# mantasu/face-crop-plus

Measured on AMD Instinct MI355X. Metric: faces/sec end-to-end (detect+align+crop), higher is better.
Workload: dtype f16x3; 1 GPU; RetinaFace detect + 5-pt align/crop, batch=32/GPU synthetic 1024x1024 RGB, strategy=largest, det_threshold=0.6, output 256x256, detector on 2 HIP streams x 16 images; global_batch=32, image_size=1024, parallelism=dp1

## Files before the change

face-crop-plus_amd/_native.py:

```python
from __future__ import annotations

import ctypes as C
import os

_HERE = os.path.dirname(os.path.abspath(__file__))
LIB_PATH = os.path.join(_HERE, "csrc", "libfcp_hip.so")
ABI_VERSION = 15

c_f32p = C.c_void_p
_lib = None


class ConvDesc(C.Structure):
    _fields_ = [
        ("in_", C.c_void_p), ("w", C.c_void_p), ("bias", C.c_void_p), ("out", C.c_void_p),
        ("res1", C.c_void_p), ("res2", C.c_void_p), ("wscale", C.c_void_p), ("in2", C.c_void_p),
        ("n", C.c_int32), ("in_h", C.c_int32), ("in_w", C.c_int32),
        ("cin", C.c_int32), ("in_ld", C.c_int32), ("in_up2", C.c_int32),
        ("cout", C.c_int32), ("kh", C.c_int32), ("kw", C.c_int32),
        ("stride", C.c_int32), ("pad", C.c_int32),
        ("out_h", C.c_int32), ("out_w", C.c_int32), ("out_ld", C.c_int32),
        ("tile_n", C.c_int32), ("cin4", C.c_int32),
        ("act_slope", C.c_float), ("alpha", C.c_float), ("alpha2", C.c_float),
        ("res1_pre", C.c_int32), ("res1_ld", C.c_int32), ("res1_h", C.c_int32),
        ("res1_w", C.c_int32), ("res2_ld", C.c_int32), ("precision", C.c_int32),
        ("in_fmt", C.c_int32), ("out_fmt", C.c_int32), ("res1_fmt", C.c_int32), ("res2_fmt", C.c_int32),
        ("tile_m", C.c_int32), ("cin2", C.c_int32), ("in2_ld", C.c_int32), ("in2_h", C.c_int32),
        ("in2_w", C.c_int32), ("in2_stride", C.c_int32), ("flags", C.c_int32), ("cu_budget", C.c_int32),
        ("band_top", C.c_int32), ("band_bottom", C.c_int32),
    ]


CONV_FLAT_ADDR = 1
CONV_BALANCE_TAIL = 2
CHAIN_OUT_EVEN_ONLY = 1


class ChainDesc(C.Structure):
    _fields_ = [(k, C.c_void_p) for k in ("t1", "w2", "ws2", "b2", "w3", "ws3", "b3", "res", "out", "w1n", "ws1n",
                                          "b1n", "t1n", "t1b")] + \
               [(k, C.c_int32) for k in ("n", "h", "w", "c", "cn", "t1_ld", "res_ld", "out_ld", "t1n_ld", "nout", "tile_m", "flags",
                                         "cb", "t1b_ld", "t1b_h", "t1b_w", "t1b_stride")]


_P, _I, _F, _L = C.c_void_p, C.c_int, C.c_float, C.c_int64
SIGNATURES = {
    "fcp_conv2d_nhwc_f32": [C.POINTER(ConvDesc), _P],
    "fcp_bottleneck_chain_f16x3": [C.POINTER(ChainDesc), _P],
    "fcp_u8_to_nhwc4_f32": [_P, _P, _L, C.POINTER(C.c_float), _F, _P],
    "fcp_f32nchw_to_nhwc4_f32": [_P, _P, _I, _I, _I, C.POINTER(C.c_float), _F, _P],
    "fcp_maxpool3x3s2_nhwc_f32": [_P, _P, _I, _I, _I, _I, _I, _I, _I, _P],
    "fcp_maxpool3x3s2_split32": [_P, _P, _I, _I, _I, _I, _I, _I, _I, _P],
    "fcp_stem7x7s2_relu_pool_u8": [_P, _I, _I, _I, C.POINTER(C.c_int32), _P, _P, _P, _P, _I, _I, _P],
    "fcp_stem7x7s2_relu_pool_conv1_u8": [_P, _I, _I, _I, C.POINTER(C.c_int32), _P, _P, _P, _P, _I, _I, _P, _P, _P, _P, _I, _P],
    "fcp_stem7x7s2_relu_pool_f32": [_P, _I, _I, _I, _P, _P, _P, _P, _I, _I, _P],
    "fcp_f32_to_split32": [_P, _P, _L, _I, _P],
    "fcp_split32_to_f32": [_P, _P, _L, _I, _P],
    "fcp_absmax_nhwc": [_P, _L, _I, _I, _I, _P, _P],
    "fcp_retina_decode": [_P, _P, _P, _I, _I, _I, _F, _F, _F, _P, _P, _P, _P, _P, _P, _P, _P, _P],
    "fcp_retina_nms_select": [_P, _P, _P, _I, _I, _F, _I, _P, _P, _P, _P, _P, _P],
    "fcp_retina_gather_faces": [_P, _P, _P, _I, _I, _P, _I, _P, _P, _P, _P],
    "fcp_estimate_transform": [_P, _P, _I, _I, _I, _P, _P, _P],
    "fcp_estimate_transform_counted": [_P, _P, _I, _I, _I, _P, _P, _P, _P, _P],
    "fcp_bise_preprocess_u8": [_P, _I, _I, _I, _P, _I, _I, C.POINTER(C.c_float), C.POINTER(C.c_float), _P],
    "fcp_avgpool_nhwc_f32": [_P, _I, _I, _I, _I, _P, _P],
    "fcp_fc_f32": [_P, _P, _P, _P, _I, _I, _I, _I, _P, _P],
    "fcp_scale_add_nhwc_f32": [_P, _I, _P, _P, _P, _I, _I, _I, _I, _P, _I, _P],
    "fcp_parse_tail": [_P, _I, _I, _I, _I, _I, _I, _I, _I, _I, _P, _P, _P],
    "fcp_label_mask_u8": [_P, _L, C.c_uint32, _P, _P],
    "fcp_bicubic_down4_u8": [_P, _I, _I, _I, _P, _P],
    "fcp_warp_affine_u8": [_P, _I, _I, _I, _P, _P, _P, _P, _I, _I, _I, _I, _P, _P],
    "fcp_warp_affine_u8_float": [_P, _I, _I, _I, _P, _P, _P, _P, _I, _I, _I, _I, _P, _P],
    "fcp_build_batch_u8": [_P, _L, _P, _P, _I, _I, _I, _I, _P, _P],
    "fcp_warp_affine_u8_ragged": [_P, _L, _P, _P, _P, _P, _I, _I, _I, _I, _P, _P],
    "fcp_warp_affine_u8_float_ragged": [_P, _L, _P, _P, _P, _P, _I, _I, _I, _I, _P, _P],
    "fcp_resize_area_ragged_u8": [_P, _L, _P, _P, _I, _P, _L, _P],
    "fcp_warp_affine_u8_interp": [_P, _I, _I, _I, _P, _P, _P, _P, _I, _I, _I, _I, _I, _P, _P],
    "fcp_warp_affine_u8_interp_ragged": [_P, _L, _P, _P, _P, _P, _I, _I, _I, _I, _I, _P, _P],
    "fcp_warp_interp_weights": [_I, _P],
    "fcp_crop_sharpness_u8": [_P, _I, _I, _I, _P, _P, _P],
    "fcp_jpeg_encode_u8": [_P, _I, _I, _I, _I, _I, _I, _P, _L, _L, _P, _P, _L, _P],
    "fcp_jpeg_encode_ex_u8": [_P, _I, _I, _I, _I, _I, _I, _I, _P, _L, _L, _P, _P, _P, _L, _P],
    "fcp_jpeg_huffman_tables": [_P, _I, _P, _P, _P],
    "fcp_png_encode_u8": [_P, _I, _I, _I, _I, _P, _L, _L, _P, _P, _L, _P],
    "fcp_png_huffman_lengths": [_P, _I, _P, _P, _P],
    "fcp_matte_u8": [_P, _P, _I, _I, _I, C.c_uint32, _I, _I, _I, _I, _P, _P, _P],
    "fcp_clahe_u8": [_P, _I, _I, _I, _I, C.c_double, _P, _P, _P],
    "fcp_matte_blur_u8": [_P, _P, _I, _I, _I, C.c_uint32, _I, _P, _I, _P, _P, _P, _L, _P],
    "fcp_matte_refine_u8": [_P, _P, _I, _I, _I, C.c_uint32, _I, _I, _P, _P, _L, _P],
    "fcp_matte_alpha_u8": [_P, _P, _I, _I, _I, _I, _I, _I, _P, _P],
    "fcp_matte_blur_alpha_u8": [_P, _P, _P, _I, _I, _I, C.c_uint32, _P, _I, _P, _P, _L, _P],
    "fcp_subject_mask_u8": [_P, _I, _I, _I, C.c_uint32, _I, _I, _P, _P, _L, _P],
    "fcp_feather_alpha_u8": [_P, _I, _I, _I, C.c_uint32, _I, _P, _P],
    "fcp_cutout_u8": [_P, _P, _I, _I, _I, _I, _I, _I, _I, _P, _I, _P, _P, _L, _P],
    "fcp_mask_shift_u8": [_P, _I, _I, _I, C.c_uint32, _I, _P, _P],
    "fcp_nlm_denoise_u8": [_P, _I, _I, _I, _P, _I, _I, _P, _P],
}
EXPORTS = ["fcp_abi_version", "fcp_last_error", "fcp_retina_nms_workspace_bytes", "fcp_jpeg_workspace_bytes",
           "fcp_jpeg_workspace_bytes_ex", "fcp_matte_blur_workspace_bytes", "fcp_matte_refine_workspace_bytes",
           "fcp_subject_mask_workspace_bytes", "fcp_png_workspace_bytes", "fcp_cutout_workspace_bytes"] + list(SIGNATURES)


def lib():
    global _lib
    if _lib is not None:
        return _lib
    if not os.path.isfile(LIB_PATH):
        raise RuntimeError(
            f"HIP extension not built: {LIB_PATH} is missing. Run "
            f"`python face-crop-plus_amd/build_native.py` (needs hipcc). There is no CPU fallback.")
    l = C.CDLL(LIB_PATH)
    l.fcp_abi_version.restype = C.c_int
    l.fcp_last_error.restype = C.c_char_p
    if l.fcp_abi_version() != ABI_VERSION:
        raise RuntimeError(f"libfcp_hip.so ABI {l.fcp_abi_version()} != expected {ABI_VERSION}; rebuild")
    l.fcp_retina_nms_workspace_bytes.argtypes = [C.c_int, C.c_int]
    l.fcp_retina_nms_workspace_bytes.restype = C.c_int64
    l.fcp_jpeg_workspace_bytes.argtypes = [C.c_int, C.c_int, C.c_int, C.c_int]
    l.fcp_jpeg_workspace_bytes.restype = C.c_int64
    l.fcp_jpeg_workspace_bytes_ex.argtypes = [C.c_int] * 6
    l.fcp_jpeg_workspace_bytes_ex.restype = C.c_int64
    l.fcp_png_workspace_bytes.argtypes = [C.c_int, C.c_int, C.c_int, C.c_int]
    l.fcp_png_workspace_bytes.restype = C.c_int64
    l.fcp_matte_blur_workspace_bytes.argtypes = [C.c_int, C.c_int, C.c_int]
    l.fcp_matte_blur_workspace_bytes.restype = C.c_int64
    l.fcp_matte_refine_workspace_bytes.argtypes = [C.c_int, C.c_int, C.c_int]
    l.fcp_matte_refine_workspace_bytes.restype = C.c_int64
    l.fcp_subject_mask_workspace_bytes.argtypes = [C.c_int, C.c_int, C.c_int]
    l.fcp_subject_mask_workspace_bytes.restype = C.c_int64
    l.fcp_cutout_workspace_bytes.argtypes = [C.c_int, C.c_int, C.c_int]
    l.fcp_cutout_workspace_bytes.restype = C.c_int64
    for name, args in SIGNATURES.items():
        fn = getattr(l, name)
        fn.argtypes = args
        fn.restype = C.c_int
    _lib = l
    return l


def check(rc: int, what: str = ""):
    if rc != 0:
        msg = lib().fcp_last_error().decode(errors="replace")
        raise RuntimeError(f"{what or 'fcp_hip'} failed ({rc}): {msg}")


def stream_ptr():
    import torch
    return C.c_void_p(torch.cuda.current_stream().cuda_stream)


def ptr(t, byte_offset: int = 0):
    if t is None:
        return C.c_void_p(0)
    return C.c_void_p(t.data_ptr() + byte_offset)


def encode_slots(who: str, entry: str, pixels_dev, out, op, workspace_bytes, call):
    import torch
    assert pixels_dev.dtype == torch.uint8 and pixels_dev.is_contiguous() and pixels_dev.dim() in (3, 4)
    assert out.dtype == torch.uint8 and out.dim() == 2 and out.shape[0] == pixels_dev.shape[0]
    if op is not None:
        return op()
    f, h, w = pixels_dev.shape[:3]
    c = pixels_dev.shape[3] if pixels_dev.dim() == 4 else 1
    capacity = out.shape[1]
    if capacity and out.stride(1) != 1:
        raise RuntimeError(f"{who}: the bytes of a row of out must be contiguous")
    lengths = torch.empty((f,), dtype=torch.int32, device=pixels_dev.device)
    need = workspace_bytes(f, h, w, c)
    check(-1 if need < 0 else 0, entry)
    work = torch.empty((need,), dtype=torch.uint8, device=pixels_dev.device)
    check(call((f, h, w, c), (ptr(out) if capacity else None, out.stride(0) if f > 1 else capacity, capacity, ptr(lengths)),
               (ptr(work), need, stream_ptr())), entry)
    return lengths
```

face-crop-plus_amd/csrc/fcp_conv.hip:

```cpp
#include "fcp_conv_common.h"

#include <cstdlib>

using namespace fcp_conv;

namespace {

constexpr int LDK = 32;


template <int BN, bool CIN4, bool BUF>
__global__ void __launch_bounds__(256, (BN == 128 ? 2 : (BN == 64 ? 3 : 4))) conv_igemm_f32(const ConvK p) {
  constexpr int WAVES_N = (BN == 32) ? 1 : 2;
  constexpr int WAVES_M = 4 / WAVES_N;
  constexpr int WTM = BM / WAVES_M;
  constexpr int WTN = BN / WAVES_N;
  constexpr int TM = WTM / 32, TN = WTN / 32;
  constexpr int A_LD = BM / 32;
  constexpr int B_LD = BN / 32;

  extern __shared__ __attribute__((aligned(16))) float smem[];
  float* As = smem;
  float* Bs = smem + 2 * BM * LDK;

  const int logical = xcd_tile_order(gridDim.x, blockIdx.x);
  const int tile_n = logical % p.grid_n;
  const int tile_m = logical / p.grid_n;

  const int tid = threadIdx.x;
  const int lane = tid & 63;
  const int wave = tid >> 6;
  const int wm = wave / WAVES_N, wn = wave % WAVES_N;
  const int chunk = tid & 7;
  const int lrow = tid >> 3;

  long nbase[A_LD];
  RowPiece pc[A_LD];
  const int hw = p.out_h * p.out_w;
#pragma unroll
  for (int i = 0; i < A_LD; ++i) {
    const ConvRow r = conv_row(p, tile_m * BM + lrow + 32 * i, p.M, hw, 0u);
    nbase[i] = (long)r.ni * p.ph * p.pw;
    pc[i] = make_row_piece<CIN4>(p, r, chunk, (unsigned)(chunk * 4));
  }
  const float* wbase = p.w + (long)(tile_n * BN + lrow) * p.wrow + chunk * 4;

  __amdgpu_buffer_rsrc_t rs_in, rs_w;
  unsigned rowoff[A_LD];
  unsigned woff[B_LD];
  if (BUF) {
    rs_in = __builtin_amdgcn_make_buffer_rsrc(const_cast<float*>(p.in), 0, p.in_bytes, 0x00020000);
    rs_w = __builtin_amdgcn_make_buffer_rsrc(const_cast<float*>(p.w), 0, p.w_bytes, 0x00020000);
#pragma unroll
    for (int i = 0; i < B_LD; ++i)
      woff[i] = (unsigned)(((tile_n * BN + lrow + 32 * i) * p.wrow + chunk * 4) * 4);
  }

  f32x4 ra0[A_LD], rb0[B_LD], ra1[A_LD], rb1[B_LD];

  auto load_slice = [&](f32x4 (&ra)[A_LD], f32x4 (&rb)[B_LD], int kt, int kh_i, int kw_i, int c0) {
    if (BUF) {
#pragma unroll
      for (int i = 0; i < A_LD; ++i) {
        const unsigned vo = rowoff[i] == 0xFFFFFFFFu ? 0xFFFFFFFFu : rowoff[i] + (unsigned)(c0 * 4);
        ra[i] = buf_load16(rs_in, vo);
      }
#pragma unroll
      for (int i = 0; i < B_LD; ++i) rb[i] = buf_load16(rs_w, woff[i] + (unsigned)(kt * BK * 4));
    } else {
#pragma unroll
      for (int i = 0; i < A_LD; ++i) {
        int hi = pc[i].hi0 + kh_i;
        int wi = pc[i].wi0 + (CIN4 ? chunk : kw_i);
        const bool ok = (unsigned)hi < (unsigned)p.in_h && (unsigned)wi < (unsigned)p.in_w;
        if (p.in_up2) { hi >>= 1; wi >>= 1; }
        const long pix = nbase[i] + (long)hi * p.pw + wi;
        const float* src = CIN4 ? p.in + pix * p.in_ld : p.in + pix * p.in_ld + c0 + chunk * 4;
        ra[i] = ok ? *reinterpret_cast<const f32x4*>(src) : f32x4{0.f, 0.f, 0.f, 0.f};
      }
#pragma unroll
      for (int i = 0; i < B_LD; ++i)
        rb[i] = *reinterpret_cast<const f32x4*>(wbase + (long)(32 * i) * p.wrow + kt * BK);
    }
  };
  const int schunk = chunk ^ ((lrow >> 1) & 7);
  auto store_slice = [&](const f32x4 (&ra)[A_LD], const f32x4 (&rb)[B_LD], int buf) {
    float* a = As + buf * BM * LDK + lrow * LDK + schunk * 4;
    float* b = Bs + buf * BN * LDK + lrow * LDK + schunk * 4;
#pragma unroll
    for (int i = 0; i < A_LD; ++i) *reinterpret_cast<f32x4*>(a + 32 * i * LDK) = ra[i];
#pragma unroll
    for (int i = 0; i < B_LD; ++i) *reinterpret_cast<f32x4*>(b + 32 * i * LDK) = rb[i];
  };

  f32x16 acc[TM][TN];
  clear_acc(acc);

  TapWalk tw;
  auto advance = [&]() {
    if (BUF) next_tap<CIN4, true>(p, tw, pc, rowoff);
    else tw.advance<CIN4>(p);
  };

  const int aoff = (wm * WTM + (lane & 31)) * LDK;
  const int boff = (wn * WTN + (lane & 31)) * LDK;
  const int rsw = ((lane & 31) >> 1) & 7;
  int koff[4];
#pragma unroll
  for (int pp = 0; pp < 4; ++pp) koff[pp] = (((2 * pp + (lane >> 5)) ^ rsw)) * 4;

  auto compute = [&](int buf) {
    const float* Ab = As + buf * BM * LDK + aoff;
    const float* Bb = Bs + buf * BN * LDK + boff;
#pragma unroll
    for (int pp = 0; pp < 4; ++pp) {
      f32x4 a[TM], b[TN];
#pragma unroll
      for (int i = 0; i < TM; ++i) a[i] = *reinterpret_cast<const f32x4*>(Ab + (i * 32 * LDK + koff[pp]));
#pragma unroll
      for (int j = 0; j < TN; ++j) b[j] = *reinterpret_cast<const f32x4*>(Bb + (j * 32 * LDK + koff[pp]));
#pragma unroll
      for (int e = 0; e < 4; ++e)
#pragma unroll
        for (int i = 0; i < TM; ++i)
#pragma unroll
          for (int j = 0; j < TN; ++j)
            acc[i][j] = __builtin_amdgcn_mfma_f32_32x32x2f32(a[i][e], b[j][e], acc[i][j], 0, 0, 0);
    }
  };
  auto step = [&](int kt, f32x4 (&ra_ld)[A_LD], f32x4 (&rb_ld)[B_LD], const f32x4 (&ra_st)[A_LD],
                  const f32x4 (&rb_st)[B_LD]) {
    if (kt + 2 < p.ktiles) {
      advance();
      load_slice(ra_ld, rb_ld, kt + 2, tw.kh_i, tw.kw_i, tw.c0);
    }
    compute(kt & 1);
    if (kt + 1 < p.ktiles) store_slice(ra_st, rb_st, (kt + 1) & 1);
    __syncthreads();
  };

  if (BUF) set_tap<CIN4, true>(p, tw, pc, rowoff);
  load_slice(ra0, rb0, 0, tw.kh_i, tw.kw_i, tw.c0);
  store_slice(ra0, rb0, 0);
  if (p.ktiles > 1) {
    advance();
    load_slice(ra1, rb1, 1, tw.kh_i, tw.kw_i, tw.c0);
  }
  __syncthreads();
  for (int kt = 0; kt < p.ktiles; kt += 2) {
    step(kt, ra0, rb0, ra1, rb1);
    if (kt + 1 < p.ktiles) step(kt + 1, ra1, rb1, ra0, rb0);
  }

  conv_epilogue<BN, TM, TN, WTM, WTN>(p, acc, smem, tile_m, tile_n, tid, lane, wm, wn, hw);
}

template <int BN, bool CIN4, bool BUF>
int launch(const ConvK& k, hipStream_t s) {
  const size_t lds = (size_t)2 * (BM + BN) * LDK * sizeof(float);
  FCP_LDS_OPT_IN((&conv_igemm_f32<BN, CIN4, BUF>), lds);
  const int blocks = k.grid_m * k.grid_n;
  hipLaunchKernelGGL((conv_igemm_f32<BN, CIN4, BUF>), dim3(blocks), dim3(256), lds, s, k);
  FCP_LAUNCH_OK();
  return 0;
}

}

extern "C" int fcp_conv2d_nhwc_f32(const fcp_conv_desc* d, fcp_stream_t stream) {
  FCP_REQUIRE(d != nullptr, "conv: null descriptor");
  FCP_REQUIRE(d->in && d->w && d->out, "conv: null tensor pointer");
  FCP_REQUIRE(d->n > 0 && d->in_h > 0 && d->in_w > 0 && d->cout > 0, "conv: bad sizes");
  const bool big = d->tile_m == 256, halo = d->tile_m == 1;
  FCP_REQUIRE(d->tile_m == 0 || d->tile_m == 128 || big || halo, "conv: tile_m must be 0/128/256 (or 1: halo-tile 3x3)");
  const bool halo_wide = halo && d->tile_n != 32;
  if (halo)
    FCP_REQUIRE(d->precision == 1 && d->in_fmt == 1 && !d->cin4 && d->kh == 3 && d->kw == 3 && d->stride == 1 &&
                d->pad == 1 && d->cout <= 64 && d->cout % 8 == 0 && d->cin >= 64 && !d->in2 &&
                (!d->res1 || (d->res1_h == d->out_h && d->res1_w == d->out_w)) || halo_wide,
                "conv: the halo-tile kernel needs a 3x3 / stride 1 / pad 1 conv with cin >= 64, cout <= 64 (cout %% 8 == 0) on the "
                "fp16x3 path with a split32 input, no second source, no resized residual");
  if (halo_wide)
    FCP_REQUIRE(d->precision == 1 && d->in_fmt == 1 && !d->cin4 && d->kh == 3 && d->kw == 3 && d->stride == 1 &&
                d->pad == 1 && d->cout % 8 == 0 && d->cin >= 64 && d->cin % 64 == 0 && !d->in2 &&
                ((d->tile_n == 64 && d->cout <= 64 && (!d->res1 || (d->res1_h == d->out_h && d->res1_w == d->out_w))) ||
                 (d->tile_n == 128 && d->cout <= 128 && !d->res1 && !d->res2)),
                "conv: the wide halo-tile kernel (tile_m 1, tile_n 64 / 128) needs a 3x3 / stride 1 / pad 1 conv with cin %% 64 == 0, "
                "cout <= tile_n (cout %% 8 == 0; no residuals above 64 filters) on the fp16x3 path with a split32 input");
  FCP_REQUIRE(d->tile_n == 32 || d->tile_n == 64 || d->tile_n == 128 || (big && (d->tile_n == 256 || d->tile_n == 192)),
              "conv: tile_n must be 32/64/128 (or 192 / 256 with tile_m 256)");
  if (big)
    FCP_REQUIRE(d->precision == 1 && d->in_fmt == 1 && !d->cin4 && !d->in_up2 && d->cout % 8 == 0 && d->tile_n >= 128,
                "conv: 256-row tiles need the fp16x3 path on a split32 input (no cin4 / in_up2), cout %% 8 == 0, tile_n 128/256");
  FCP_REQUIRE(d->kh >= 1 && d->kw >= 1 && d->stride >= 1 && d->pad >= 0, "conv: bad filter geometry");
  FCP_REQUIRE(d->kh * d->kw <= 32 || d->cin4, "conv: at most 32 filter taps (kh*kw) outside cin4 mode");
  FCP_REQUIRE(d->in_ld % 4 == 0 && ((uintptr_t)d->in & 15) == 0, "conv: input must be 16-byte aligned, in_ld %% 4 == 0");
  FCP_REQUIRE(((uintptr_t)d->w & 15) == 0, "conv: filter must be 16-byte aligned");
  if (d->cin4) {
    FCP_REQUIRE(d->cin <= 4 && d->in_ld == 4 && d->kw <= 8, "conv: cin4 mode needs cin<=4, in_ld==4, kw<=8");
  } else {
    FCP_REQUIRE(d->cin % 32 == 0 && d->cin > 0, "conv: cin must be a multiple of 32 (got %d)", d->cin);
  }
  FCP_REQUIRE(d->band_top >= 0 && d->band_bottom >= 0 && d->band_top <= d->pad && d->band_bottom <= d->pad &&
              ((d->band_top | d->band_bottom) == 0 || (d->stride == 1 && !d->in2)),
              "conv: band_top / band_bottom must lie in 0..pad (stride-1 convs without a second source only)");
  const int eh = (d->in_h - d->band_top - d->band_bottom + 2 * d->pad - d->kh) / d->stride + 1;
  const int ew = (d->in_w + 2 * d->pad - d->kw) / d->stride + 1;
  FCP_REQUIRE(eh == d->out_h && ew == d->out_w, "conv: output size %dx%d does not match geometry %dx%d",
              d->out_h, d->out_w, eh, ew);
  if (d->in_up2) FCP_REQUIRE(d->in_h % 2 == 0 && d->in_w % 2 == 0, "conv: in_up2 needs even logical size");
  const long M = (long)d->n * d->out_h * d->out_w;
  FCP_REQUIRE(M < (1L << 31), "conv: too many output pixels");

  ConvK k;
  k.in = d->in; k.w = reinterpret_cast<const float*>(d->w); k.bias = d->bias; k.wscale = d->wscale; k.out = d->out; k.res1 = d->res1; k.res2 = d->res2;
  k.n = d->n; k.in_h = d->in_h; k.in_w = d->in_w;
  k.ph = d->in_up2 ? d->in_h / 2 : d->in_h;
  k.pw = d->in_up2 ? d->in_w / 2 : d->in_w;
  k.cin = d->cin; k.in_ld = d->in_ld; k.in_up2 = d->in_up2;
  k.cout = d->cout; k.kh = d->kh; k.kw = d->kw; k.stride = d->stride; k.pad = d->pad; k.pad_h = d->pad - d->band_top;
  k.out_h = d->out_h; k.out_w = d->out_w; k.out_ld = d->out_ld;
  k.M = (int)M;
  if (d->cin4) {
    k.ktiles = d->kh; k.ctiles = 1; k.wrow = d->kh * 32;
  } else {
    k.ctiles = d->cin / 32; k.ktiles = d->kh * d->kw * k.ctiles; k.wrow = d->kh * d->kw * d->cin;
  }
  k.act_slope = d->act_slope; k.alpha = d->alpha; k.alpha2 = d->alpha2;
  k.res1_pre = d->res1_pre; k.res1_ld = d->res1_ld; k.res2_ld = d->res2_ld;
  k.res1_h = d->res1_h; k.res1_w = d->res1_w;
  k.res1_resize = 0; k.res1_sh = 1.f; k.res1_sw = 1.f;
  k.in_fmt = d->in_fmt; k.out_fmt = d->out_fmt; k.res1_fmt = d->res1 ? d->res1_fmt : 0; k.res2_fmt = d->res2 ? d->res2_fmt : 0;
  const int any_split = k.in_fmt | k.out_fmt | k.res1_fmt | k.res2_fmt;
  FCP_REQUIRE((unsigned)any_split <= 1u, "conv: tensor formats must be 0 (fp32) or 1 (split32)");
  if (any_split) {
    FCP_REQUIRE(d->precision == 1, "conv: split32 tensors need precision 1 (fp16x3 kernel)");
    FCP_REQUIRE(d->cout % 8 == 0, "conv: split32 epilogue needs cout %% 8 == 0");
    FCP_REQUIRE(!k.in_fmt || (!d->cin4 && d->in_ld % 32 == 0 && ((uintptr_t)d->in & 127) == 0),
                "conv: split32 input must be a 32-channel-group aligned view (in_ld %% 32 == 0), not cin4");
    FCP_REQUIRE(!k.out_fmt || (d->out_ld % 32 == 0 && ((uintptr_t)d->out & 127) == 0 && d->cout % 32 == 0),
                "conv: split32 output must be a 32-channel-group aligned view with cout %% 32 == 0");
    FCP_REQUIRE(!k.res1_fmt || (d->res1_ld % 32 == 0 && ((uintptr_t)d->res1 & 127) == 0), "conv: misaligned split32 res1");
    FCP_REQUIRE(!k.res2_fmt || (d->res2_ld % 32 == 0 && ((uintptr_t)d->res2 & 127) == 0), "conv: misaligned split32 res2");
    FCP_REQUIRE(((uintptr_t)d->out & 15) == 0 && d->out_ld % 4 == 0 && (!d->res1 || (((uintptr_t)d->res1 & 15) == 0 && d->res1_ld % 4 == 0)) &&
                (!d->res2 || (((uintptr_t)d->res2 & 15) == 0 && d->res2_ld % 4 == 0)), "conv: 8-channel epilogue needs 16-byte aligned tensors");
  }
  if (d->res1) {
    FCP_REQUIRE(d->res1_h > 0 && d->res1_w > 0 && d->res1_ld > 0, "conv: res1 geometry missing");
    if (d->res1_h != d->out_h || d->res1_w != d->out_w) {
      k.res1_resize = 1;
      k.res1_sh = (float)d->res1_h / (float)d->out_h;
      k.res1_sw = (float)d->res1_w / (float)d->out_w;
    }
  }
  if (d->res2) FCP_REQUIRE(d->res2_ld > 0, "conv: res2_ld missing");
  k.vec_ok = (d->out_ld % 4 == 0) && (((uintptr_t)d->out & 15) == 0);
  if (d->res1) k.vec_ok = k.vec_ok && (d->res1_ld % 4 == 0) && (((uintptr_t)d->res1 & 15) == 0);
  if (d->res2) k.vec_ok = k.vec_ok && (d->res2_ld % 4 == 0) && (((uintptr_t)d->res2 & 15) == 0);
  static const int nt_env = getenv("FCP_NT_STORE") ? atoi(getenv("FCP_NT_STORE")) : 1;
  k.nt_store = nt_env;
  k.balance = (d->flags & FCP_CONV_BALANCE_TAIL) ? 1 : 0;
  k.cu_budget = d->cu_budget;
  k.mfull = 0; k.tail_rows = 0; k.round_size = 0;
  k.in2 = nullptr; k.in2_bytes = 0; k.csplit = d->cin; k.in2_ld = 0; k.ph2 = 0; k.pw2 = 0; k.stride2 = 1;
  if (d->in2) {
    FCP_REQUIRE(d->precision == 1 && d->in_fmt == 1 && !d->cin4 && !d->in_up2 && d->kh == 1 && d->kw == 1 && d->pad == 0,
                "conv: a second source needs a 1x1 / pad 0 conv on the fp16x3 path with split32 inputs");
    FCP_REQUIRE(d->cin2 > 0 && d->cin2 < d->cin && d->cin2 % 32 == 0 && d->in2_ld % 32 == 0 && d->in2_ld >= d->cin2 &&
                ((uintptr_t)d->in2 & 127) == 0, "conv: in2 must be a 32-channel-group aligned split32 view, 0 < cin2 < cin");
    FCP_REQUIRE(d->in2_stride >= 1 && d->in2_h > 0 && d->in2_w > 0 && (long)(d->out_h - 1) * d->in2_stride < d->in2_h &&
                (long)(d->out_w - 1) * d->in2_stride < d->in2_w, "conv: in2 geometry does not cover the output grid");
    const unsigned long in2_bytes = (unsigned long)d->n * d->in2_h * d->in2_w * d->in2_ld * 4ul;
    FCP_REQUIRE(in2_bytes < 0xFFFFFFF0ul, "conv: in2 must be below 4 GiB");
    k.in2 = d->in2; k.in2_bytes = (unsigned)in2_bytes; k.csplit = d->cin - d->cin2; k.in2_ld = d->in2_ld;
    k.ph2 = d->in2_h; k.pw2 = d->in2_w; k.stride2 = d->in2_stride;
  }
  k.grid_m = fcp_cdiv(M, BM);
  k.grid_n = fcp_cdiv(d->cout, d->tile_n);
  hipStream_t s = (hipStream_t)stream;
  const unsigned long in_bytes = (unsigned long)d->n * k.ph * k.pw * d->in_ld * 4ul;
  const unsigned long w_bytes = (unsigned long)(k.grid_n * d->tile_n) * k.wrow * 4ul;
  FCP_REQUIRE(!(d->flags & FCP_CONV_FLAT_ADDR) || d->precision == 0, "conv: FCP_CONV_FLAT_ADDR is a precision-0 (fp32 kernel) option");
  const bool buf = in_bytes < 0xFFFFFFF0ul && w_bytes < 0xFFFFFFF0ul && !(d->flags & FCP_CONV_FLAT_ADDR);
  FCP_REQUIRE(d->precision == 0 || d->precision == 1, "conv: precision must be 0 (fp32) or 1 (fp16x3)");
  if (d->precision == 1) {
    FCP_REQUIRE(buf, "conv: the fp16x3 path needs tensors below 4 GiB (pack this layer with precision 0)");
    FCP_REQUIRE(d->wscale != nullptr, "conv: precision 1 needs wscale");
    k.in_bytes = (unsigned)in_bytes;
    k.w_bytes = (unsigned)w_bytes;
    if (halo) {
      k.grid_n = 1;
      const unsigned long out_bytes = (unsigned long)M * d->out_ld * 4ul;
      FCP_REQUIRE(out_bytes < 0xFFFFFFF0ul, "conv(halo): the output view must span less than 4 GiB");
      FCP_REQUIRE(d->wscale != nullptr && ((uintptr_t)d->wscale & 15) == 0 && ((uintptr_t)d->bias & 15) == 0,
                  "conv(halo): wscale / bias must be 16-byte aligned");
      k.in2_bytes = (unsigned)out_bytes;
      k.w_bytes = (unsigned)((unsigned long)fcp_cdiv(d->cout, 128) * 128ul * k.wrow * 4ul);
      return halo_wide ? launch_f16x3_halo_wide(k, s) : launch_f16x3_halo(k, s);
    }
    if (big) {
      k.w_bytes = (unsigned)((unsigned long)fcp_cdiv(d->cout, 128) * 128ul * k.wrow * 4ul);
      return launch_f16x3_big(k, d->tile_n, s);
    }
    if (k.in_fmt == 1 && !d->cin4) return launch_f16x3_dma(k, d->tile_n, s);
    return launch_f16x3(k, d->tile_n, d->cin4 != 0, s);
  }
  k.in_bytes = buf ? (unsigned)in_bytes : 0u;
  k.w_bytes = buf ? (unsigned)w_bytes : 0u;
#define FCP_DISPATCH(BN_)                                                             \
  do {                                                                                \
    if (d->cin4) return buf ? launch<BN_, true, true>(k, s) : launch<BN_, true, false>(k, s); \
    return buf ? launch<BN_, false, true>(k, s) : launch<BN_, false, false>(k, s);   \
  } while (0)
  switch (d->tile_n) {
    case 32: FCP_DISPATCH(32);
    case 64: FCP_DISPATCH(64);
    default: FCP_DISPATCH(128);
  }
#undef FCP_DISPATCH
}
```

face-crop-plus_amd/csrc/fcp_conv_common.h:

```cpp
#pragma once
#include <type_traits>
#include "fcp_common.h"
#include "fcp_hip.h"

typedef float f32x16 __attribute__((ext_vector_type(16)));
typedef float f32x4 __attribute__((ext_vector_type(4)));


constexpr int FCP_AUX_A = 0;
constexpr int FCP_AUX_B = 0;

namespace fcp_conv {

constexpr int BM = 128;
constexpr int BK = 32;

struct ConvK {
  const float* in;
  const float* w;
  const float* bias;
  float* out;
  const float* res1;
  const float* res2;
  int n, in_h, in_w, ph, pw, cin, in_ld, in_up2;
// ... 271 lines not shown
  if (fmt == 1) {
    pack8(v, 1, a, b);
    store8(base, pix, ld, c, 1, nt, a, b);
  } else {
    pack8(v, 0, a, b);
    store8(base, pix, ld, c, 0, 0, a, b);
  }
}

__device__ __forceinline__ float conv_scale_bias(float acc, float ws, float b) { return acc * ws + b; }

struct ConvEpi {
  bool res1, res1_pre, res2;
  float act_slope, alpha, alpha2;
};
template <typename E>
__device__ __forceinline__ float conv_finish(const E e, float x, float r1, float r2) {
  if (e.res1 && e.res1_pre) x += r1;
  x = x >= 0.f ? x : x * e.act_slope;
  x = x * e.alpha;
  if (e.res1 && !e.res1_pre) x += r1;
  if (e.res2) x = x * e.alpha2 + r2;
  return x;
}
template <typename E>
__device__ __forceinline__ float conv_value(const E& e, float acc, float ws, float b, float r1, float r2) {
  return conv_finish(e, conv_scale_bias(acc, ws, b), r1, r2);
}
__device__ __forceinline__ float conv_finish_relu(float x) { return conv_finish(ConvEpi{false, false, false, 0.f, 1.f, 1.f}, x, 0.f, 0.f); }
__device__ __forceinline__ float conv_finish_relu(float x, float r1) { return conv_finish(ConvEpi{true, true, false, 0.f, 1.f, 1.f}, x, r1, 0.f); }
__device__ __forceinline__ float conv_value_relu(float acc, float ws, float b) { return conv_finish_relu(conv_scale_bias(acc, ws, b)); }

__device__ __forceinline__ long res1_pixel(const ConvK& p, long m, int hw) {
  int ni, ho, wo;
  conv_out_pixel(p, m, hw, ni, ho, wo);
  int sh = (int)floorf(ho * p.res1_sh);
  int sw = (int)floorf(wo * p.res1_sw);
  sh = sh < p.res1_h - 1 ? sh : p.res1_h - 1;
  sw = sw < p.res1_w - 1 ? sw : p.res1_w - 1;
  return ((long)ni * p.res1_h + sh) * p.res1_w + sw;
}

__device__ __forceinline__ constexpr int mfma_c_row(int rr, int half) { return (rr & 3) + 8 * (rr >> 2) + 4 * half; }

template <int BN, int TM, int TN, int WTM, int WTN>
__device__ __forceinline__ void stage_acc_tile(const f32x16 (&acc)[TM][TN], float* Cs, int lane, int wm, int wn) {
  const int half = lane >> 5;
#pragma unroll
  for (int i = 0; i < TM; ++i)
#pragma unroll
    for (int j = 0; j < TN; ++j)
#pragma unroll
      for (int rr = 0; rr < 16; ++rr) {
        const int row = wm * WTM + i * 32 + mfma_c_row(rr, half);
        Cs[row * BN + wn * WTN + j * 32 + (lane & 31)] = acc[i][j][rr];
      }
  __syncthreads();
}

template <int BN, int TM, int TN, int WTM, int WTN>
__device__ __forceinline__ void conv_epilogue(const ConvK& p, f32x16 (&acc)[TM][TN], float* smem, int tile_m,
                                              int tile_n, int tid, int lane, int wm, int wn, int hw) {
  constexpr int CPR = BN / 4;
  constexpr int RPP = 256 / CPR;
  constexpr int PASSES = BM / RPP;
  float* Cs = smem;
  const int ccol = (tid % CPR) * 4;
  const int crow = tid / CPR;
  const int co = tile_n * BN + ccol;
  const bool vec = p.vec_ok && (co + 3 < p.cout);
  const long m0 = (long)tile_m * BM + crow;

  const bool pre1 = p.res1 != nullptr && !p.res1_resize && vec;
  const bool pre2 = p.res2 != nullptr && vec;
  stage_acc_tile<BN, TM, TN, WTM, WTN>(acc, Cs, lane, wm, wn);

  f32x4 bias4 = {0.f, 0.f, 0.f, 0.f}, ws4 = {1.f, 1.f, 1.f, 1.f};
  if (p.bias != nullptr) {
#pragma unroll
    for (int e = 0; e < 4; ++e)
      if (co + e < p.cout) bias4[e] = p.bias[co + e];
  }
  if (p.wscale != nullptr) {
#pragma unroll
    for (int e = 0; e < 4; ++e)
      if (co + e < p.cout) ws4[e] = p.wscale[co + e];
  }
  constexpr int EPC = PASSES < 4 ? PASSES : 4;
#pragma unroll 1
  for (int g = 0; g < PASSES; g += EPC) {
    f32x4 r1v[EPC], r2v[EPC];
    if (pre1) {
#pragma unroll
      for (int i = 0; i < EPC; ++i) {
        const long m = m0 + (long)(g + i) * RPP;
        r1v[i] = m < p.M ? *reinterpret_cast<const f32x4*>(p.res1 + m * p.res1_ld + co) : f32x4{0.f, 0.f, 0.f, 0.f};
      }
    }
    if (pre2) {
#pragma unroll
      for (int i = 0; i < EPC; ++i) {
        const long m = m0 + (long)(g + i) * RPP;
        r2v[i] = m < p.M ? *reinterpret_cast<const f32x4*>(p.res2 + m * p.res2_ld + co) : f32x4{0.f, 0.f, 0.f, 0.f};
      }
    }
#pragma unroll
    for (int i = 0; i < EPC; ++i) {
      const int row = crow + (g + i) * RPP;
      const long m = m0 + (long)(g + i) * RPP;
      if (m >= p.M || co >= p.cout) continue;
      f32x4 v = *reinterpret_cast<const f32x4*>(Cs + row * BN + ccol);
      f32x4 r1 = {0.f, 0.f, 0.f, 0.f}, r2 = {0.f, 0.f, 0.f, 0.f};
      if (pre1) {
        r1 = r1v[i];
      } else if (p.res1 != nullptr) {
        const long roff = (p.res1_resize ? res1_pixel(p, m, hw) : m) * p.res1_ld + co;
        if (vec) {
          r1 = *reinterpret_cast<const f32x4*>(p.res1 + roff);
        } else {
#pragma unroll
          for (int e = 0; e < 4; ++e)
            if (co + e < p.cout) r1[e] = p.res1[roff + e];
        }
      }
      if (pre2) {
        r2 = r2v[i];
      } else if (p.res2 != nullptr) {
#pragma unroll
        for (int e = 0; e < 4; ++e)
          if (co + e < p.cout) r2[e] = p.res2[m * p.res2_ld + co + e];
      }
#pragma unroll
      for (int e = 0; e < 4; ++e) v[e] = conv_value(p, v[e], ws4[e], bias4[e], r1[e], r2[e]);
      float* dst = p.out + m * p.out_ld + co;
      if (vec) {
        *reinterpret_cast<f32x4*>(dst) = v;
      } else {
#pragma unroll
        for (int e = 0; e < 4; ++e)
          if (co + e < p.cout) dst[e] = v[e];
      }
    }
  }
}


template <int I, int N, typename F>
__device__ __forceinline__ void fcp_static_for(F&& f) {
  if constexpr (I < N) {
    f(std::integral_constant<int, I>{});
    fcp_static_for<I + 1, N>(f);
  }
}

template <int TM, int TN, int WTM, int WTN>
__device__ __forceinline__ void conv_epilogue_regs(const ConvK& p, f32x16 (&acc)[TM][TN], int m_start, int m_end, int tm_act, int co_tile,
                                                   int co_end, int wm, int wn, int lane, int hw) {
    const int lp = lane & 15, lg = lane >> 4;
  auto swap32 = [](float& x, float& y) {
    const auto r = __builtin_amdgcn_permlane32_swap(__float_as_uint(x), __float_as_uint(y), false, false);
    const unsigned r0 = r[0], r1 = r[1];
    x = __uint_as_float(r0); y = __uint_as_float(r1);
  };
  auto swap16 = [](float& x, float& y) {
    const auto r = __builtin_amdgcn_permlane16_swap(__float_as_uint(x), __float_as_uint(y), false, false);
    const unsigned r0 = r[0], r1 = r[1];
    x = __uint_as_float(r0); y = __uint_as_float(r1);
  };
  constexpr int GI = TM < 2 ? TM : 2;
  constexpr int NGI = (TM + GI - 1) / GI;
  constexpr int NG = TN * NGI;
  u32x4_t pend_a[GI][2], pend_b[GI][2];
  auto row_of = [&](int i, int set) { return m_start + wm * WTM + i * 32 + 16 * set + lp; };
  auto chan_of = [&](int jj) { return co_tile + wn * WTN + jj * 32 + 8 * lg; };
  auto flush = [&](auto gc) {
    constexpr int g = decltype(gc)::value, jj = g / NGI, i0 = (g % NGI) * GI;
    const int co = chan_of(jj);
    fcp_static_for<0, GI>([&](auto ic) {
      constexpr int i = i0 + decltype(ic)::value;
      if constexpr (i < TM) {
        fcp_static_for<0, 2>([&](auto sc) {
          constexpr int set = decltype(sc)::value;
          const int mi = row_of(i, set);
          if (i < tm_act && mi < m_end && co < co_end) store8(p.out, mi, p.out_ld, co, p.out_fmt, 0, pend_a[i - i0][set], pend_b[i - i0][set]);
        });
      }
    });
  };
  fcp_static_for<0, NG>([&](auto gc) {
    constexpr int g = decltype(gc)::value, j = g / NGI, i0 = (g % NGI) * GI;
    const int co = chan_of(j);
    const bool cok = co < co_end;
    const int cc = cok ? co : co_tile;
    u32x4_t r1a[GI][2], r1b[GI][2];
    if (p.res1 != nullptr) {
      fcp_static_for<0, GI>([&](auto ic) {
        constexpr int i = i0 + decltype(ic)::value;
        if constexpr (i < TM) {
          fcp_static_for<0, 2>([&](auto sc) {
            constexpr int set = decltype(sc)::value;
            const int mi = row_of(i, set);
            const long m = (i < tm_act && mi < m_end && cok) ? (long)mi : (long)m_start;
            const long rpix = p.res1_resize ? res1_pixel(p, m, hw) : m;
            if (p.res1_fmt == 1) {
              const char* pb = reinterpret_cast<const char*>(p.res1) + rpix * p.res1_ld * 4 + split_chan_off(cc);
              r1a[i - i0][set] = *reinterpret_cast<const u32x4_t*>(pb);
              r1b[i - i0][set] = *reinterpret_cast<const u32x4_t*>(pb + 64);
            } else {
              r1a[i - i0][set] = *reinterpret_cast<const u32x4_t*>(p.res1 + rpix * p.res1_ld + cc);
              r1b[i - i0][set] = *reinterpret_cast<const u32x4_t*>(p.res1 + rpix * p.res1_ld + cc + 4);
            }
          });
        }
      });
    }
    __builtin_amdgcn_sched_barrier(0);
    if constexpr (g > 0) flush(std::integral_constant<int, g - 1>{});
    __builtin_amdgcn_sched_barrier(0);
    float bias8[8], ws8[8];
    {
      const f32x4 w0 = *reinterpret_cast<const f32x4*>(p.wscale + cc), w1 = *reinterpret_cast<const f32x4*>(p.wscale + cc + 4);
      f32x4 b0 = {0.f, 0.f, 0.f, 0.f}, b1 = b0;
      if (p.bias != nullptr) { b0 = *reinterpret_cast<const f32x4*>(p.bias + cc); b1 = *reinterpret_cast<const f32x4*>(p.bias + cc + 4); }
#pragma unroll
      for (int e = 0; e < 4; ++e) { ws8[e] = w0[e]; ws8[4 + e] = w1[e]; bias8[e] = b0[e]; bias8[4 + e] = b1[e]; }
    }
    fcp_static_for<0, GI>([&](auto ic) {
      constexpr int i = i0 + decltype(ic)::value;
      if constexpr (i < TM) {
        float va[8], vb[8];
        fcp_static_for<0, 4>([&](auto ec) {
          constexpr int e = decltype(ec)::value;
          float q0 = acc[i][j][e], q1 = acc[i][j][4 + e], q2 = acc[i][j][8 + e], q3 = acc[i][j][12 + e];
          swap32(q0, q1);
          swap32(q2, q3);
          swap32(q0, q2); swap16(q0, q2);
          swap32(q1, q3); swap16(q1, q3);
          va[e] = q0; va[4 + e] = q1; vb[e] = q2; vb[4 + e] = q3;
        });
        fcp_static_for<0, 2>([&](auto sc) {
          constexpr int set = decltype(sc)::value;
          float (&v)[8] = set == 0 ? va : vb;
          float r1[8], r2[8];
          if (p.res1 != nullptr) {
            if (p.res1_fmt == 1) {
              join8(r1a[i - i0][set], r1b[i - i0][set], r1);
            } else {
              const f32x4 fa = __builtin_bit_cast(f32x4, r1a[i - i0][set]), fb = __builtin_bit_cast(f32x4, r1b[i - i0][set]);
              r1[0] = fa[0]; r1[1] = fa[1]; r1[2] = fa[2]; r1[3] = fa[3]; r1[4] = fb[0]; r1[5] = fb[1]; r1[6] = fb[2]; r1[7] = fb[3];
            }
          }
          if (p.res2 != nullptr) {
            const int mi = row_of(i, set);
            load8(p.res2, (i < tm_act && mi < m_end && cok) ? (long)mi : (long)m_start, p.res2_ld, cc, p.res2_fmt, r2);
          }
#pragma unroll
          for (int e = 0; e < 8; ++e) v[e] = conv_value(p, v[e], ws8[e], bias8[e], r1[e], r2[e]);
          pack8(v, p.out_fmt, pend_a[i - i0][set], pend_b[i - i0][set]);
        });
      }
    });
  });
  flush(std::integral_constant<int, NG - 1>{});
}

template <int BN, int TM, int TN, int WTM, int WTN>
__device__ __forceinline__ void conv_epilogue8(const ConvK& p, f32x16 (&acc)[TM][TN], float* smem, int tile_m,
                                               int tile_n, int tid, int lane, int wm, int wn, int hw) {
  constexpr int CPR = BN / 8;
  constexpr int RPP = 256 / CPR;
  constexpr int PASSES = BM / RPP;
  float* Cs = smem;
  const int ccol = (tid % CPR) * 8;
  const int crow = tid / CPR;
  const int co = tile_n * BN + ccol;
  const long m0 = (long)tile_m * BM + crow;
  stage_acc_tile<BN, TM, TN, WTM, WTN>(acc, Cs, lane, wm, wn);
  if (co >= p.cout) return;
  float bias8[8], ws8[8];
#pragma unroll
  for (int e = 0; e < 8; ++e) {
    bias8[e] = p.bias != nullptr ? p.bias[co + e] : 0.f;
    ws8[e] = p.wscale != nullptr ? p.wscale[co + e] : 1.f;
  }
#pragma unroll
  for (int g = 0; g < PASSES; ++g) {
    const int row = crow + g * RPP;
    const long m = m0 + (long)g * RPP;
    if (m >= p.M) continue;
    float v[8], r1[8], r2[8];
    {
      const f32x4 a = *reinterpret_cast<const f32x4*>(Cs + row * BN + ccol);
      const f32x4 b = *reinterpret_cast<const f32x4*>(Cs + row * BN + ccol + 4);
      v[0] = a[0]; v[1] = a[1]; v[2] = a[2]; v[3] = a[3]; v[4] = b[0]; v[5] = b[1]; v[6] = b[2]; v[7] = b[3];
    }
    if (p.res1 != nullptr) load8(p.res1, p.res1_resize ? res1_pixel(p, m, hw) : m, p.res1_ld, co, p.res1_fmt, r1);
    if (p.res2 != nullptr) load8(p.res2, m, p.res2_ld, co, p.res2_fmt, r2);
#pragma unroll
    for (int e = 0; e < 8; ++e) v[e] = conv_value(p, v[e], ws8[e], bias8[e], r1[e], r2[e]);
    pack_store8(p.out, m, p.out_ld, co, p.out_fmt, p.nt_store, v);
  }
}

int launch_f16x3(const ConvK& k, int tile_n, bool cin4, hipStream_t s);
int launch_f16x3_dma(const ConvK& k, int tile_n, hipStream_t s);
int launch_f16x3_halo(const ConvK& k, hipStream_t s);
int launch_f16x3_halo_wide(const ConvK& k, hipStream_t s);
int launch_f16x3_big(const ConvK& k, int tile_n, hipStream_t s);

}
```

face-crop-plus_amd/csrc/fcp_conv_f16x3_big.hip:

```cpp
#include "fcp_conv_common.h"

#include <type_traits>

using namespace fcp_conv;

namespace {

constexpr int BMB = 256;
constexpr int NT = 512;
constexpr int ROWB = 128;
constexpr int STAGE = 1 << 16;

template <int BN>
__global__ void __launch_bounds__(NT, 1) conv_igemm_f16x3_big(const ConvK p) {
  constexpr int WAVES_N = BN == 256 ? 4 : 2;
  constexpr int WAVES_M = 8 / WAVES_N;
  constexpr int WTM = BMB / WAVES_M, WTN = BN / WAVES_N;
  constexpr int TM = WTM / 32, TN = WTN / 32;
  constexpr int A_LD = BMB / 64, B_LD = BN / 64;

  extern __shared__ __attribute__((aligned(16))) float smem[];
  char* lds = reinterpret_cast<char*>(smem);

  const int nb = p.big_tiles;
  int vb = blockIdx.x;
  int tile_n = 0, m_start = 0, m_end = 0;
  auto decode = [&](int bid) {
    const int rbase = (bid / p.round_size) * p.round_size;
    const int nr = nb - rbase < p.round_size ? nb - rbase : p.round_size;
    const int bi = bid - rbase;
    const int logical = rbase + xcd_tile_order(nr, bi);
    tile_n = logical % p.grid_n;
    const int tile_m = logical / p.grid_n;
    m_start = tile_m < p.mfull ? tile_m * BMB : p.mfull * BMB + (tile_m - p.mfull) * p.tail_rows;
    const int m_rows = tile_m < p.mfull ? BMB : p.tail_rows;
    m_end = m_start + m_rows < p.M ? m_start + m_rows : p.M;
  };
  decode(vb);

  const int tid = threadIdx.x;
  const int lane = tid & 63;
  const int wave_u = __builtin_amdgcn_readfirstlane(tid >> 6);
  const int wm = wave_u / WAVES_N, wn = wave_u % WAVES_N;
  const int lrow = tid >> 3;
  const int csrc = (tid & 7) ^ (((lrow >> 1) & 7) ^ ((lrow & 1) << 2));

  const int hw = p.out_h * p.out_w;
  RowPiece pc[A_LD];
  unsigned base2[A_LD];
  unsigned rowoff[A_LD], woff[B_LD];
  auto setup_tile = [&]() {
#pragma unroll
    for (int i = 0; i < A_LD; ++i) {
      const int m = m_start + lrow + 64 * i;
      unsigned pbase = 0;
      int hi0 = -(1 << 28), wi0 = 0;
      base2[i] = 0xFFFFFFFFu;
      if (m < m_end) {
        int ni, ho, wo;
        conv_out_pixel(p, m, hw, ni, ho, wo);
        pbase = (unsigned)(ni * p.ph * p.pw);
        hi0 = ho * p.stride - p.pad_h;
        wi0 = wo * p.stride - p.pad;
        if (p.in2 != nullptr)
          base2[i] = (((unsigned)(ni * p.ph2 + ho * p.stride2) * (unsigned)p.pw2 + (unsigned)(wo * p.stride2)) * (unsigned)p.in2_ld +
                      (unsigned)(csrc * 4)) * 4u;
      }
      pc[i].tp = make_tap_piece<false>(p, pbase, hi0, wi0, (unsigned)(csrc * 4));
    }
#pragma unroll
    for (int i = 0; i < B_LD; ++i) woff[i] = (unsigned)(((tile_n * BN + lrow + 64 * i) * p.wrow + csrc * 4) * 4);
  };
  setup_tile();
  __amdgpu_buffer_rsrc_t rs_in2 = __builtin_amdgcn_make_buffer_rsrc(const_cast<float*>(p.in2 ? p.in2 : p.in), 0, p.in2_bytes, 0x00020000);
  __amdgpu_buffer_rsrc_t rs_in = __builtin_amdgcn_make_buffer_rsrc(const_cast<float*>(p.in), 0, p.in_bytes, 0x00020000);
  __amdgpu_buffer_rsrc_t rs_w = __builtin_amdgcn_make_buffer_rsrc(const_cast<float*>(p.w), 0, p.w_bytes, 0x00020000);
  TapWalk tw;
  auto advance = [&]() { next_tap<false, false>(p, tw, pc, rowoff); };
  auto dma = [&](int kt, int stage) {
    char* a = lds + stage * STAGE + wave_u * 8 * ROWB;
    dma_slice<64>(p, rs_in, rs_in2, rs_w, a, a + BMB * ROWB, rowoff, base2, woff, tw.c0, kt);
  };

  f32x16 acc[TM][TN];

  const unsigned lds0 = (unsigned)(size_t)(__attribute__((address_space(3))) char*)lds;
  int offH[2], offL[2];
  frag_offsets(lane, offH, offL);
  const unsigned arow = lds0 + (unsigned)((wm * WTM + (lane & 31)) * ROWB);
  const unsigned brow = lds0 + (unsigned)((BMB + wn * WTN + (lane & 31)) * ROWB);
  unsigned aH[2], aL[2], bH[2], bL[2];
#pragma unroll
  for (int s = 0; s < 2; ++s) {
    aH[s] = arow + (unsigned)offH[s]; aL[s] = arow + (unsigned)offL[s];
    bH[s] = brow + (unsigned)offH[s]; bL[s] = brow + (unsigned)offL[s];
  }

  auto prefetch_tile = [&]() {
    tw = TapWalk();
    set_tap<false, false>(p, tw, pc, rowoff);
    dma(0, 0);
    if (p.ktiles > 1) {
      advance();
      dma(1, 1);
    }
  };
  prefetch_tile();
  int tm_act = 0;
  auto main_loop = [&](auto tma_c) {
    constexpr int TMA = decltype(tma_c)::value;
    f16x8 fah[2][TMA > 0 ? TMA : 1], fal[2][TMA > 0 ? TMA : 1], fbh[2][TN], fbl[2][TN];
  auto read_frags = [&](auto set_c, unsigned stage_xor) {
    constexpr int set = decltype(set_c)::value;
    fcp_static_for<0, TMA>([&](auto ic) {
      constexpr int i = decltype(ic)::value;
      fah[set][i] = lds_read128i<i * 32 * ROWB>(aH[set] ^ stage_xor);
      fal[set][i] = lds_read128i<i * 32 * ROWB>(aL[set] ^ stage_xor);
    });
    fcp_static_for<0, TN>([&](auto jc) {
      constexpr int j = decltype(jc)::value;
      fbh[set][j] = lds_read128i<j * 32 * ROWB>(bH[set] ^ stage_xor);
      fbl[set][j] = lds_read128i<j * 32 * ROWB>(bL[set] ^ stage_xor);
    });
  };
  constexpr std::integral_constant<int, 0> SET0{};
  constexpr std::integral_constant<int, 1> SET1{};
  auto mfmas_reads = [&](auto cs_c, auto ls_c, unsigned stage_xor) {
    constexpr int cs = decltype(cs_c)::value, ls = decltype(ls_c)::value;
    constexpr int NM = 3 * TMA * TN, NR = 2 * TMA + 2 * TN;
    fcp_static_for<0, NM>([&](auto mc) {
      constexpr int m = decltype(mc)::value;
      constexpr int g = m / (TMA * TN), i = (m % (TMA * TN)) / TN, j = m % TN;
      if constexpr (g == 0) acc[i][j] = __builtin_amdgcn_mfma_f32_32x32x16_f16(fbh[cs][j], fal[cs][i], acc[i][j], 0, 0, 0);
      else if constexpr (g == 1) acc[i][j] = __builtin_amdgcn_mfma_f32_32x32x16_f16(fbl[cs][j], fah[cs][i], acc[i][j], 0, 0, 0);
      else acc[i][j] = __builtin_amdgcn_mfma_f32_32x32x16_f16(fbh[cs][j], fah[cs][i], acc[i][j], 0, 0, 0);
      __builtin_amdgcn_sched_barrier(0);
      fcp_static_for<0, NR>([&](auto rc) {
        constexpr int r = decltype(rc)::value;
        if constexpr (((r + 1) * NM) / NR - 1 == m
        ) {
          if constexpr (r < 2 * TMA) {
            constexpr int ii = r / 2;
            if constexpr (r % 2 == 0) fah[ls][ii] = lds_read128i<ii * 32 * ROWB>(aH[ls] ^ stage_xor);
            else fal[ls][ii] = lds_read128i<ii * 32 * ROWB>(aL[ls] ^ stage_xor);
          } else {
            constexpr int jj = (r - 2 * TMA) / 2;
            if constexpr (r % 2 == 0) fbh[ls][jj] = lds_read128i<jj * 32 * ROWB>(bH[ls] ^ stage_xor);
            else fbl[ls][jj] = lds_read128i<jj * 32 * ROWB>(bL[ls] ^ stage_xor);
          }
          __builtin_amdgcn_sched_barrier(0);
        }
      });
    });
  };

  read_frags(SET0, 0u);
  asm volatile("s_waitcnt lgkmcnt(0)" ::: "memory");
  __builtin_amdgcn_sched_barrier(0);

  unsigned sx = 0u;
  for (int kt = 0; kt < p.ktiles; ++kt) {
    mfmas_reads(SET0, SET1, sx);
    __builtin_amdgcn_sched_barrier(0);
    asm volatile("s_waitcnt lgkmcnt(0)" ::: "memory");
    asm volatile("s_waitcnt vmcnt(0)" ::: "memory");
    __builtin_amdgcn_s_barrier();
    __builtin_amdgcn_sched_barrier(0);
    const bool dma_first = wave_u >= 4;
    if (dma_first && kt + 2 < p.ktiles) {
      advance();
      dma(kt + 2, kt & 1);
    }
    __builtin_amdgcn_sched_barrier(0);
    mfmas_reads(SET1, SET0, sx ^ (unsigned)STAGE);
    __builtin_amdgcn_sched_barrier(0);
    if (!dma_first && kt + 2 < p.ktiles) {
      advance();
      dma(kt + 2, kt & 1);
    }
    __builtin_amdgcn_sched_barrier(0);
    asm volatile("s_waitcnt lgkmcnt(0)" ::: "memory");
    __builtin_amdgcn_sched_barrier(0);
    sx ^= (unsigned)STAGE;
  }
  };
  for (;;) {
  asm volatile("s_waitcnt vmcnt(0)" ::: "memory");
  __builtin_amdgcn_s_barrier();
  __builtin_amdgcn_sched_barrier(0);
  tm_act = (m_end - m_start - wm * WTM + 31) >> 5;
  tm_act = __builtin_amdgcn_readfirstlane(tm_act < 0 ? 0 : (tm_act > TM ? TM : tm_act));
  clear_acc(acc);
  fcp_static_for<0, TM + 1>([&](auto tc) {
    if (tm_act == decltype(tc)::value) main_loop(tc);
  });
  asm volatile("s_waitcnt vmcnt(0)" ::: "memory");
  __builtin_amdgcn_s_barrier();

  const int e_tile_n = tile_n, e_m_start = m_start, e_m_end = m_end, e_tm_act = tm_act;
  const bool more = p.big_persist && vb + p.round_size < nb;
  if (more) {
    vb += p.round_size;
    decode(vb);
    setup_tile();
    prefetch_tile();
  }
  conv_epilogue_regs<TM, TN, WTM, WTN>(p, acc, e_m_start, e_m_end, e_tm_act, e_tile_n * BN,
                                       (e_tile_n + 1) * BN < p.cout ? (e_tile_n + 1) * BN : p.cout, wm, wn, lane, hw);
  if (!more) break;
  }
}

template <int BN>
int launch(ConvK k, hipStream_t s) {
  const size_t lds = 2 * (size_t)STAGE;
  FCP_LDS_OPT_IN((&conv_igemm_f16x3_big<BN>), lds);
  k.grid_n = fcp_cdiv(k.cout, BN);
  int cus = k.cu_budget > 0 ? k.cu_budget : fcp_cu_count();
  cus = cus < 8 ? 8 : (cus & ~7);
  k.round_size = cus;
  const int mt = fcp_cdiv(k.M, BMB);
  k.mfull = mt;
  k.tail_rows = BMB;
  k.grid_m = mt;
  if (k.balance) {
    const long tiles = (long)mt * k.grid_n;
    const long full_rounds = tiles / cus;
    const int mfull = (int)((full_rounds * cus) / k.grid_n);
    const long rem = (long)k.M - (long)mfull * BMB;
    if (rem > 0) {
      const long slots = cus / k.grid_n > 0 ? cus / k.grid_n : 1;
      long r = ((rem + slots - 1) / slots + 31) / 32 * 32;
      r = r < 32 ? 32 : r;
      if (r < BMB) {
        k.mfull = mfull;
        k.tail_rows = (int)r;
        k.grid_m = mfull + (int)((rem + r - 1) / r);
      }
    }
  }
  k.big_tiles = k.grid_m * k.grid_n;
  static const int persist_env = getenv("FCP_BIG_PERSIST") ? atoi(getenv("FCP_BIG_PERSIST")) : -1;
  k.big_persist = persist_env < 0 ? (k.cu_budget == 0) : (persist_env != 0);
  hipLaunchKernelGGL((conv_igemm_f16x3_big<BN>), dim3(k.big_persist && k.big_tiles > k.round_size ? k.round_size : k.big_tiles), dim3(NT), lds, s, k);
  FCP_LAUNCH_OK();
  return 0;
}

}

namespace fcp_conv {

int launch_f16x3_big(const ConvK& k, int tile_n, hipStream_t s) {
  return tile_n == 256 ? launch<256>(k, s) : tile_n == 192 ? launch<192>(k, s) : launch<128>(k, s);
}

}
```

face-crop-plus_amd/csrc/fcp_conv_f16x3_dma.hip:

```cpp
#include "fcp_conv_common.h"

using namespace fcp_conv;

namespace {

constexpr int NST = 2;

template <int BN, bool EP8>
__global__ void __launch_bounds__(256, (BN == 128 ? 2 : 3)) conv_igemm_f16x3_dma(const ConvK p) {
  constexpr int WAVES_N = (BN == 32) ? 1 : 2;
  constexpr int WAVES_M = 4 / WAVES_N;
  constexpr int WTM = BM / WAVES_M;
  constexpr int WTN = BN / WAVES_N;
  constexpr int TM = WTM / 32, TN = WTN / 32;
  constexpr int A_LD = BM / 32;
  constexpr int B_LD = BN / 32;
  constexpr int ROWB = 128;
  constexpr int STAGE = (BM + BN) * ROWB;

  extern __shared__ __attribute__((aligned(16))) float smem[];
  char* lds = reinterpret_cast<char*>(smem);

  const int logical = xcd_tile_order(gridDim.x, blockIdx.x);
  const int tile_n = logical % p.grid_n;
  const int tile_m = logical / p.grid_n;

  const int tid = threadIdx.x;
  const int lane = tid & 63;
  const int wave = tid >> 6;
  const int wave_u = __builtin_amdgcn_readfirstlane(wave);
  const int wm = wave / WAVES_N, wn = wave % WAVES_N;
  const int lrow = tid >> 3;
  const int csrc = (tid & 7) ^ (((lrow >> 1) & 7) ^ ((lrow & 1) << 2));

  const int hw = p.out_h * p.out_w;
  __amdgpu_buffer_rsrc_t rs_in = __builtin_amdgcn_make_buffer_rsrc(const_cast<float*>(p.in), 0, p.in_bytes, 0x00020000);
  __amdgpu_buffer_rsrc_t rs_w = __builtin_amdgcn_make_buffer_rsrc(const_cast<float*>(p.w), 0, p.w_bytes, 0x00020000);
  __amdgpu_buffer_rsrc_t rs_in2 = __builtin_amdgcn_make_buffer_rsrc(const_cast<float*>(p.in2 ? p.in2 : p.in), 0, p.in2_bytes, 0x00020000);
  RowPiece pc[A_LD];
  unsigned base2[A_LD], rowoff[A_LD], woff[B_LD];
#pragma unroll
  for (int i = 0; i < A_LD; ++i) {
    const ConvRow r = conv_row(p, tile_m * BM + lrow + 32 * i, p.M, hw, (unsigned)(csrc * 4));
    pc[i] = make_row_piece<false>(p, r, 0, (unsigned)(csrc * 4));
    base2[i] = r.base2;
  }
#pragma unroll
  for (int i = 0; i < B_LD; ++i) woff[i] = (unsigned)(((tile_n * BN + lrow + 32 * i) * p.wrow + csrc * 4) * 4);
  TapWalk tw;
  auto dma = [&](int kt, int stage) {
    char* a = lds + stage * STAGE + wave_u * 8 * ROWB;
    dma_slice<32>(p, rs_in, rs_in2, rs_w, a, a + BM * ROWB, rowoff, base2, woff, tw.c0, kt);
  };

  f32x16 acc[TM][TN];
  clear_acc(acc);

  const int aoff = (wm * WTM + (lane & 31)) * ROWB;
  const int boff = BM * ROWB + (wn * WTN + (lane & 31)) * ROWB;
  int offH[2], offL[2];
  frag_offsets(lane, offH, offL);

  set_tap<false, true>(p, tw, pc, rowoff);
  dma(0, 0);
  asm volatile("s_waitcnt vmcnt(0)" ::: "memory");
  __builtin_amdgcn_s_barrier();

  int stage = 0;
  const int kt_end = p.ktiles;
  for (int kt = 0; kt < kt_end; ++kt) {
    const char* Ab = lds + stage * STAGE + aoff;
    const char* Bb = lds + stage * STAGE + boff;
    f16x8 ah[2][TM], al[2][TM], bh[2][TN], bl[2][TN];
#pragma unroll
    for (int s = 0; s < 2; ++s) {
#pragma unroll
      for (int i = 0; i < TM; ++i) {
        ah[s][i] = *reinterpret_cast<const f16x8*>(Ab + i * 32 * ROWB + offH[s]);
        al[s][i] = *reinterpret_cast<const f16x8*>(Ab + i * 32 * ROWB + offL[s]);
      }
#pragma unroll
      for (int j = 0; j < TN; ++j) {
        bh[s][j] = *reinterpret_cast<const f16x8*>(Bb + j * 32 * ROWB + offH[s]);
        bl[s][j] = *reinterpret_cast<const f16x8*>(Bb + j * 32 * ROWB + offL[s]);
      }
    }
    asm volatile("s_waitcnt lgkmcnt(0)" ::: "memory");
    __builtin_amdgcn_sched_barrier(0);
    const int ahead = kt + NST - 1;
    const bool issue = ahead < p.ktiles;
    if (issue) {
      next_tap<false, true>(p, tw, pc, rowoff);
      int st = stage + NST - 1;
      if (st >= NST) st -= NST;
      dma(ahead, st);
    }
    __builtin_amdgcn_sched_barrier(0);
#pragma unroll
    for (int s = 0; s < 2; ++s)
#pragma unroll
      for (int i = 0; i < TM; ++i)
#pragma unroll
        for (int j = 0; j < TN; ++j) {
          if constexpr (EP8) {
            acc[i][j] = __builtin_amdgcn_mfma_f32_32x32x16_f16(bh[s][j], al[s][i], acc[i][j], 0, 0, 0);
            acc[i][j] = __builtin_amdgcn_mfma_f32_32x32x16_f16(bl[s][j], ah[s][i], acc[i][j], 0, 0, 0);
            acc[i][j] = __builtin_amdgcn_mfma_f32_32x32x16_f16(bh[s][j], ah[s][i], acc[i][j], 0, 0, 0);
          } else {
            acc[i][j] = __builtin_amdgcn_mfma_f32_32x32x16_f16(al[s][i], bh[s][j], acc[i][j], 0, 0, 0);
            acc[i][j] = __builtin_amdgcn_mfma_f32_32x32x16_f16(ah[s][i], bl[s][j], acc[i][j], 0, 0, 0);
            acc[i][j] = __builtin_amdgcn_mfma_f32_32x32x16_f16(ah[s][i], bh[s][j], acc[i][j], 0, 0, 0);
          }
        }
    __builtin_amdgcn_sched_barrier(0);
    asm volatile("s_waitcnt vmcnt(0)" ::: "memory");
    __builtin_amdgcn_s_barrier();
    __builtin_amdgcn_sched_barrier(0);
    if (++stage >= NST) stage = 0;
  }

  if constexpr (EP8) {
    const int m_end = (tile_m + 1) * BM < p.M ? (tile_m + 1) * BM : p.M;
    conv_epilogue_regs<TM, TN, WTM, WTN>(p, acc, tile_m * BM, m_end, TM, tile_n * BN, (tile_n + 1) * BN < p.cout ? (tile_n + 1) * BN : p.cout,
                                         wm, wn, lane, hw);
  } else {
    conv_epilogue<BN, TM, TN, WTM, WTN>(p, acc, smem, tile_m, tile_n, tid, lane, wm, wn, hw);
  }
}

template <int BN, bool EP8>
int launch_ep(const ConvK& k, hipStream_t s) {
  size_t lds = (size_t)NST * (BM + BN) * 128;
  const size_t epi = EP8 ? 0 : (size_t)BM * BN * 4;
  if (lds < epi) lds = epi;
  FCP_LDS_OPT_IN((&conv_igemm_f16x3_dma<BN, EP8>), lds);
  hipLaunchKernelGGL((conv_igemm_f16x3_dma<BN, EP8>), dim3(k.grid_m * k.grid_n), dim3(256), lds, s, k);
  FCP_LAUNCH_OK();
  return 0;
}
template <int BN>
int launch(const ConvK& k, hipStream_t s) {
  const bool ep8 = (k.out_fmt | k.res1_fmt | k.res2_fmt) != 0;
  return ep8 ? launch_ep<BN, true>(k, s) : launch_ep<BN, false>(k, s);
}

}

namespace fcp_conv {

int launch_f16x3_dma(const ConvK& k, int tile_n, hipStream_t s) {
  switch (tile_n) {
    case 32: return launch<32>(k, s);
    case 64: return launch<64>(k, s);
    default: return launch<128>(k, s);
  }
}

}
```

face-crop-plus_amd/csrc/fcp_conv_f16x3_halo.hip:

```cpp
#include "fcp_conv_common.h"

#include <type_traits>

using namespace fcp_conv;

namespace {

constexpr int TH = 8, TW = 32;
constexpr int HW_ = TW + 2;
constexpr int HROWS = 344;
constexpr int ROWB = 128;
constexpr int A_BYTES = HROWS * ROWB;
constexpr int B_BYTES = 9 * 32 * ROWB;
constexpr int B_OFF = 2 * A_BYTES;
constexpr int LDS_TOTAL = 2 * A_BYTES + 2 * B_BYTES;
constexpr int A_LD = 11;
constexpr int HALO_I = A_LD - 1;

__device__ __forceinline__ void lds_write32(unsigned addr, float v) { asm volatile("ds_write_b32 %0, %1" ::"v"(addr), "v"(v) : "memory"); }
__device__ __forceinline__ f32x4 lds_read128f(unsigned addr) {
  f32x4 v;
  asm volatile("ds_read_b128 %0, %1" : "=v"(v) : "v"(addr));
  return v;
}


struct HaloTiles {
  int tiles_x, tiles_y, ntiles, per_x, xcd, slot, slots;
  struct Next { int nit, ntile; bool more; };
  __device__ __forceinline__ HaloTiles(const ConvK& p, int nb, int bid)
      : tiles_x((p.out_w + TW - 1) / TW), tiles_y((p.out_h + TH - 1) / TH), ntiles(p.n * tiles_x * tiles_y), per_x((ntiles + 7) / 8),
        xcd(bid & 7), slot(bid >> 3), slots((nb + 7 - xcd) / 8) {}
  __device__ __forceinline__ int tile(int it) const { return xcd * per_x + it; }
  __device__ __forceinline__ bool has(int it) const { return it < per_x && tile(it) < ntiles; }
  __device__ __forceinline__ Next next(int it) const { return {it + slots, tile(it + slots), has(it + slots)}; }
  __device__ __forceinline__ void coords(int tile, int& ni, int& y0, int& x0) const {
    const int tx = tile % tiles_x;
    const int ty = (tile / tiles_x) % tiles_y;
    ni = tile / (tiles_x * tiles_y);
    y0 = ty * TH; x0 = tx * TW;
  }
};

__device__ __forceinline__ void halo_frag_addrs(unsigned (&aaddr)[4][3], unsigned lds0, int wave_u, int xl, int half) {
#pragma unroll
  for (int d = 0; d < 4; ++d)
#pragma unroll
    for (int kw = 0; kw < 3; ++kw) {
      const int hr = (2 * wave_u + d) * HW_ + xl + kw;
      aaddr[d][kw] = lds0 + (unsigned)(hr * ROWB + ((half ^ swz(hr)) << 4));
    }
}

__device__ __forceinline__ void halo_epi_consts(const ConvK& p, int ccol, bool cvalid, f32x4 (&b8)[2], f32x4 (&w8)[2]) {
  b8[0] = b8[1] = w8[0] = w8[1] = f32x4{0.f, 0.f, 0.f, 0.f};
  if (cvalid) {
    if (p.bias != nullptr) { b8[0] = *reinterpret_cast<const f32x4*>(p.bias + ccol); b8[1] = *reinterpret_cast<const f32x4*>(p.bias + ccol + 4); }
    w8[0] = *reinterpret_cast<const f32x4*>(p.wscale + ccol); w8[1] = *reinterpret_cast<const f32x4*>(p.wscale + ccol + 4);
  }
}

template <int TN>
__global__ void __launch_bounds__(512, 1) conv3x3_halo_f16x3(const ConvK p) {
  extern __shared__ __attribute__((aligned(16))) float smem[];
  char* lds = reinterpret_cast<char*>(smem);
  const unsigned lds0 = (unsigned)(size_t)(__attribute__((address_space(3))) char*)lds;

  const HaloTiles ts(p, gridDim.x, blockIdx.x);

  const int lane = threadIdx.x & 63;
  const int wave8 = __builtin_amdgcn_readfirstlane(threadIdx.x >> 6);
  const bool loader = wave8 >= 4;
  const int wave_u = wave8 & 3;
  const int tid = threadIdx.x & 255;
  const int nslices = p.ctiles;
  const int nblocks = nslices * TN;

  int it = ts.slot;
  if (!ts.has(it)) return;

  if (loader) {
    const int lrow = tid >> 3;
    const int csrc = (tid & 7) ^ swz(lrow);
    __amdgpu_buffer_rsrc_t rs_in = __builtin_amdgcn_make_buffer_rsrc(const_cast<float*>(p.in), 0, p.in_bytes, 0x00020000);
    __amdgpu_buffer_rsrc_t rs_w = __builtin_amdgcn_make_buffer_rsrc(const_cast<float*>(p.w), 0, p.w_bytes, 0x00020000);
    const unsigned wbase = (unsigned)((lrow * p.wrow) * 4 + csrc * 16);
    unsigned abase[A_LD];
    int hyx[A_LD];
#pragma unroll
    for (int i = 0; i < A_LD; ++i) {
      const int hr = lrow + 32 * i;
      const int hy = hr / HW_, hx = hr - hy * HW_;
      hyx[i] = hr < (TH + 2) * HW_ ? (hy << 8 | hx) : -1;
    }
    auto tile_setup = [&](int tile) {
      int ni, y0, x0;
      ts.coords(tile, ni, y0, x0);
#pragma unroll
      for (int i = 0; i < A_LD; ++i) {
        const int y = y0 - p.pad_h + (hyx[i] >> 8), x = x0 - 1 + (hyx[i] & 255);
        const bool ok = hyx[i] >= 0 && (unsigned)y < (unsigned)p.in_h && (unsigned)x < (unsigned)p.in_w;
        const int yp = p.in_up2 ? y >> 1 : y, xp = p.in_up2 ? x >> 1 : x;
        abase[i] = ok ? ((unsigned)((ni * p.ph + yp) * p.pw + xp) * (unsigned)p.in_ld + (unsigned)(csrc * 4)) * 4u : 0xFFFFFFFFu;
      }
    };
    auto dma_halo = [&](int cs, int stage) {
      char* a = lds + stage * A_BYTES + wave_u * 8 * ROWB;
#pragma unroll
      for (int i = 0; i < A_LD - 1; ++i) {
        const unsigned ro = abase[i];
        __builtin_amdgcn_raw_ptr_buffer_load_lds(rs_in, (__attribute__((address_space(3))) void*)(a + 32 * i * ROWB), 16,
                                                 (int)(ro == 0xFFFFFFFFu ? 0xFFFFFFFFu : ro + (unsigned)(cs * 128)), 0, 0, 0);
      }
      if (wave_u < 3) {
        const unsigned ro = abase[A_LD - 1];
        __builtin_amdgcn_raw_ptr_buffer_load_lds(rs_in, (__attribute__((address_space(3))) void*)(a + 32 * (A_LD - 1) * ROWB), 16,
                                                 (int)(ro == 0xFFFFFFFFu ? 0xFFFFFFFFu : ro + (unsigned)(cs * 128)), 0, 0, 0);
      }
    };
    auto dma_filter = [&](int blk, int buf) {
      const int cs = blk / TN, pass = blk - cs * TN;
      char* b = (lds + wave_u * 8 * ROWB) + B_OFF + buf * B_BYTES;
      const unsigned wo = wbase + (unsigned)(pass * 32 * p.wrow * 4 + cs * 9 * 128);
#pragma unroll
      for (int t = 0; t < 9; ++t)
        __builtin_amdgcn_raw_ptr_buffer_load_lds(rs_w, (__attribute__((address_space(3))) void*)(b + 32 * t * ROWB), 16,
                                                 (int)(wo + (unsigned)(t * 128)), 0, 0, 0);
    };

    tile_setup(ts.tile(it));
    dma_halo(0, 0);
    dma_filter(0, 0);
    dma_halo(1, 1);
    dma_filter(1, 1);
    int blk = 0;
    unsigned bbuf = 0, astage = 0;
    asm volatile("s_waitcnt vmcnt(0)" ::: "memory");
    __builtin_amdgcn_s_barrier();
    for (;;) {
      const bool new_slice = TN == 1 || (blk & 1) != 0;
      const int cs = blk / TN;
      const bool last_of_tile = blk == nblocks - 1;
      const HaloTiles::Next nx = ts.next(it);
      asm volatile("s_waitcnt vmcnt(0)" ::: "memory");
      __builtin_amdgcn_s_barrier();
      bool halo_delayed = false;
      const int b2 = blk + 2;
      if (b2 < nblocks) dma_filter(b2, (int)bbuf);
      else if (nx.more) dma_filter(b2 - nblocks, (int)bbuf);
      if (new_slice) {
        const int s2 = cs + 2;
        if (s2 < nslices) dma_halo(s2, (int)astage);
        else if (nx.more) {
          if (s2 == nslices) {
            tile_setup(nx.ntile);
            dma_halo(0, (int)astage);
          } else {
            halo_delayed = true;
          }
        }
      }
      const unsigned freed = astage;
      bbuf ^= 1u;
      if (new_slice) astage ^= 1u;
      ++blk;
      if (new_slice && last_of_tile) {
        __builtin_amdgcn_s_barrier();
        if (!nx.more) return;
        if (halo_delayed) dma_halo(1, (int)freed);
        it = nx.nit;
        blk = 0;
      }
    }
  }

  const int xl = lane & 31, half = lane >> 5;
  unsigned aaddr[4][3];
  halo_frag_addrs(aaddr, lds0, wave_u, xl, half);
  const unsigned baddr0 = lds0 + (unsigned)(B_OFF + xl * ROWB + ((half ^ swz(xl)) << 4));

  f16x8 fah[2][2], fal[2][2], fbh[2], fbl[2];

  auto read_one = [&](auto tap_c, auto idx_c, unsigned aoff, unsigned boff) {
    constexpr int tap = decltype(tap_c)::value, idx = decltype(idx_c)::value;
    constexpr int kh = tap / 3, kw = tap % 3;
    constexpr int s = idx / 6, r = idx % 6;
    if constexpr (r == 0) fbh[s] = lds_read128i<tap * 4096>((baddr0 + boff) ^ (unsigned)(s ? 0x20 : 0));
    else if constexpr (r == 3) fbl[s] = lds_read128i<tap * 4096>((baddr0 + boff) ^ (unsigned)(s ? 0x60 : 0x40));
    else {
      constexpr int i = (r == 1 || r == 4) ? 0 : 1;
      constexpr bool lo = r < 3;
      const unsigned a = (aaddr[i + kh][kw] + aoff) ^ (unsigned)((lo ? 0x40 : 0) | (s ? 0x20 : 0));
      if constexpr (lo) fal[i][s] = lds_read128i<0>(a);
      else fah[i][s] = lds_read128i<0>(a);
    }
  };

  __amdgpu_buffer_rsrc_t rs_out = __builtin_amdgcn_make_buffer_rsrc(p.out, 0, p.in2_bytes, 0x00020000);

  int e_ni = 0, e_y0 = 0, e_x0 = 0;
  ts.coords(ts.tile(it), e_ni, e_y0, e_x0);

  f32x16 acc[TN][2];
  clear_acc(acc);

  __builtin_amdgcn_s_barrier();
  __builtin_amdgcn_sched_barrier(0);

  fcp_static_for<0, 12>([&](auto ic) { read_one(std::integral_constant<int, 0>{}, ic, 0u, 0u); });

  auto tap_step = [&](auto tap_c, auto pass_c, unsigned aoff_n, unsigned boff_n) {
    constexpr int tap = decltype(tap_c)::value, pass = decltype(pass_c)::value;
    constexpr int ntap = (tap + 1) % 9;
    fcp_static_for<0, 2>([&](auto sc) {
      constexpr int s = decltype(sc)::value;
      asm volatile("s_waitcnt lgkmcnt(6)" ::: "memory");
      __builtin_amdgcn_sched_barrier(0);
      auto rd = [&](auto rc) {
        read_one(std::integral_constant<int, ntap>{}, std::integral_constant<int, 6 * s + decltype(rc)::value>{}, aoff_n, boff_n);
        __builtin_amdgcn_sched_barrier(0);
      };
      auto mm = [&](int i, const f16x8& a, const f16x8& b) {
        acc[pass][i] = __builtin_amdgcn_mfma_f32_32x32x16_f16(a, b, acc[pass][i], 0, 0, 0);
        __builtin_amdgcn_sched_barrier(0);
      };
      mm(0, fal[0][s], fbh[s]); rd(std::integral_constant<int, 1>{});
      mm(1, fal[1][s], fbh[s]); rd(std::integral_constant<int, 2>{});
      mm(0, fah[0][s], fbl[s]);
      mm(1, fah[1][s], fbl[s]); rd(std::integral_constant<int, 3>{});
      mm(0, fah[0][s], fbh[s]); rd(std::integral_constant<int, 4>{});
      mm(1, fah[1][s], fbh[s]); rd(std::integral_constant<int, 5>{}); rd(std::integral_constant<int, 0>{});
    });
  };

  auto epilogue = [&](int stage) {
    const unsigned cs0 = lds0 + (unsigned)(stage * A_BYTES + wave_u * 64 * 128);
    const int eq = lane & 3, er = lane >> 2;
#pragma unroll
    for (int n = 0; n < TN; ++n) {
      const int ccol = n * 32 + eq * 8;
      const bool cvalid = ccol < p.cout;
      f32x4 b8[2], w8[2];
      halo_epi_consts(p, ccol, cvalid, b8, w8);
#pragma unroll
      for (int i = 0; i < 2; ++i)
#pragma unroll
        for (int rr = 0; rr < 16; ++rr) {
          const int row = i * 32 + mfma_c_row(rr, half);
          lds_write32(cs0 + (unsigned)((row * 32 + xl) * 4), acc[n][i][rr]);
        }
      __builtin_amdgcn_sched_barrier(0);
#pragma unroll
      for (int gp = 0; gp < 2; ++gp) {
        f32x4 va[2], vb[2];
#pragma unroll
        for (int g = 0; g < 2; ++g) {
          const unsigned ra = cs0 + (unsigned)(((er + 16 * (2 * gp + g)) * 32 + eq * 8) * 4);
          va[g] = lds_read128f(ra);
          vb[g] = lds_read128f(ra + 16);
        }
        asm volatile("s_waitcnt lgkmcnt(0)" ::: "memory");
        __builtin_amdgcn_sched_barrier(0);
#pragma unroll
        for (int g = 0; g < 2; ++g) {
          const int row = wave_u * 64 + er + 16 * (2 * gp + g);
          const int y = e_y0 + (row >> 5), x = e_x0 + (row & 31);
          const bool ok = cvalid && y < p.out_h && x < p.out_w;
          const long m = ok ? ((long)e_ni * p.out_h + y) * p.out_w + x : 0;
          float v[8] = {va[g][0], va[g][1], va[g][2], va[g][3], vb[g][0], vb[g][1], vb[g][2], vb[g][3]};
          float r1[8], r2[8];
          if (p.res1 != nullptr) load8(p.res1, m, p.res1_ld, cvalid ? ccol : 0, p.res1_fmt, r1);
          if (p.res2 != nullptr) load8(p.res2, m, p.res2_ld, cvalid ? ccol : 0, p.res2_fmt, r2);
#pragma unroll
          for (int e = 0; e < 8; ++e) v[e] = conv_value(p, v[e], w8[e >> 2][e & 3], b8[e >> 2][e & 3], r1[e], r2[e]);
          u32x4_t s0, s1;
          unsigned o0, o1;
          if (p.out_fmt == 1) {
            pack8(v, 1, s0, s1);
            o0 = (unsigned)(m * p.out_ld * 4 + split_chan_off(ccol));
            o1 = o0 + 64u;
          } else {
            pack8(v, 0, s0, s1);
            o0 = (unsigned)((m * p.out_ld + ccol) * 4);
            o1 = o0 + 16u;
          }
          __builtin_amdgcn_raw_buffer_store_b128(s0, rs_out, ok ? o0 : 0xFFFFFFFFu, 0, 0);
          __builtin_amdgcn_raw_buffer_store_b128(s1, rs_out, ok ? o1 : 0xFFFFFFFFu, 0, 0);
        }
      }
      __builtin_amdgcn_sched_barrier(0);
    }
    __builtin_amdgcn_s_barrier();
    __builtin_amdgcn_sched_barrier(0);
  };

  int blk = 0;
  unsigned bbuf = 0, astage = 0;
  auto run_block = [&](auto pass_c) -> bool {
    constexpr int pass = decltype(pass_c)::value;
    constexpr bool new_slice = pass == TN - 1;
    const unsigned aoff = astage * (unsigned)A_BYTES, boff = bbuf * (unsigned)B_BYTES;
    const bool last_of_tile = blk == nblocks - 1;
    const HaloTiles::Next nx = ts.next(it);
    fcp_static_for<0, 8>([&](auto tc) { tap_step(tc, pass_c, aoff, boff); });
    asm volatile("s_waitcnt lgkmcnt(0)" ::: "memory");
    __builtin_amdgcn_s_barrier();
    __builtin_amdgcn_sched_barrier(0);
    const unsigned aoff_next = new_slice ? (astage ^ 1u) * (unsigned)A_BYTES : aoff;
    const unsigned boff_next = (bbuf ^ 1u) * (unsigned)B_BYTES;
    tap_step(std::integral_constant<int, 8>{}, pass_c, aoff_next, boff_next);
    const unsigned freed = astage;
    bbuf ^= 1u;
    if constexpr (new_slice) astage ^= 1u;
    ++blk;
    if constexpr (new_slice) {
      if (last_of_tile) {
        __builtin_amdgcn_sched_barrier(0);
        epilogue((int)freed);
        if (!nx.more) return true;
        it = nx.nit;
        blk = 0;
        ts.coords(nx.ntile, e_ni, e_y0, e_x0);
        clear_acc(acc);
      }
    }
    return false;
  };
  for (;;) {
    if constexpr (TN == 2) {
      if (run_block(std::integral_constant<int, 0>{})) break;
      if (run_block(std::integral_constant<int, 1>{})) break;
    } else {
      if (run_block(std::integral_constant<int, 0>{})) break;
    }
  }
}


template <int TN, bool RES, int BT, int RS>
__global__ void __launch_bounds__(512, 1) conv3x3_halo_wide_f16x3(const ConvK p) {
  constexpr int TAPB = TN * 32 * ROWB;
  constexpr int PRE = RS - BT;
  constexpr bool SLACK2 = (RS - BT - 1) / BT >= 2;
  static_assert(18 % BT == 0 && 18 % RS == 2 && (RS & (RS - 1)) == 0 && PRE >= BT + 1, "block / ring geometry");
  extern __shared__ __attribute__((aligned(16))) float smem[];
  char* lds = reinterpret_cast<char*>(smem);
  const unsigned lds0 = (unsigned)(size_t)(__attribute__((address_space(3))) char*)lds;

  const HaloTiles ts(p, gridDim.x, blockIdx.x);

  const int lane = threadIdx.x & 63;
  const int wave8 = __builtin_amdgcn_readfirstlane(threadIdx.x >> 6);
  const bool loader = wave8 >= 4;
  const int wave_u = wave8 & 3;
  const int tid = threadIdx.x & 255;
  const int nslices = p.ctiles;
  const int T = 9 * nslices;

  int it = ts.slot;
  if (!ts.has(it)) return;

  if (loader) {
    const int lrow = tid >> 3;
    const int csrc = (tid & 7) ^ swz(lrow);
    __amdgpu_buffer_rsrc_t rs_in = __builtin_amdgcn_make_buffer_rsrc(const_cast<float*>(p.in), 0, p.in_bytes, 0x00020000);
    __amdgpu_buffer_rsrc_t rs_w = __builtin_amdgcn_make_buffer_rsrc(const_cast<float*>(p.w), 0, p.w_bytes, 0x00020000);
    const unsigned wbase = (unsigned)((lrow * p.wrow) * 4 + csrc * 16);
    unsigned abase[A_LD];
    int hyx[A_LD];
#pragma unroll
    for (int i = 0; i < A_LD; ++i) {
      const int hr = lrow + 32 * i;
      const int hy = hr / HW_, hx = hr - hy * HW_;
      hyx[i] = hr < (TH + 2) * HW_ ? (hy << 8 | hx) : -1;
    }
    auto tile_setup = [&](int tile) {
      int ni, y0, x0;
      ts.coords(tile, ni, y0, x0);
#pragma unroll
      for (int i = 0; i < A_LD; ++i) {
        const int y = y0 - p.pad_h + (hyx[i] >> 8), x = x0 - 1 + (hyx[i] & 255);
        const bool ok = hyx[i] >= 0 && (unsigned)y < (unsigned)p.in_h && (unsigned)x < (unsigned)p.in_w;
        const int yp = p.in_up2 ? y >> 1 : y, xp = p.in_up2 ? x >> 1 : x;
        abase[i] = ok ? ((unsigned)((ni * p.ph + yp) * p.pw + xp) * (unsigned)p.in_ld + (unsigned)(csrc * 4)) * 4u : 0xFFFFFFFFu;
      }
    };
    auto dma_halo = [&](int cs, int stage) {
      char* a = lds + stage * A_BYTES + wave_u * 8 * ROWB;
#pragma unroll
      for (int i = 0; i < A_LD - 1; ++i) {
        const unsigned ro = abase[i];
        __builtin_amdgcn_raw_ptr_buffer_load_lds(rs_in, (__attribute__((address_space(3))) void*)(a + 32 * i * ROWB), 16,
                                                 (int)(ro == 0xFFFFFFFFu ? 0xFFFFFFFFu : ro + (unsigned)(cs * 128)), 0, 0, 0);
      }
      if (wave_u < 3) {
        const unsigned ro = abase[A_LD - 1];
        __builtin_amdgcn_raw_ptr_buffer_load_lds(rs_in, (__attribute__((address_space(3))) void*)(a + 32 * (A_LD - 1) * ROWB), 16,
                                                 (int)(ro == 0xFFFFFFFFu ? 0xFFFFFFFFu : ro + (unsigned)(cs * 128)), 0, 0, 0);
      }
    };
    auto dma_tap = [&](int gt, int rs) {
      const int cs = gt / 9, tap = gt - cs * 9;
      char* b = (lds + wave_u * 8 * ROWB) + B_OFF + rs * TAPB;
      const unsigned wo = wbase + (unsigned)(cs * 9 * 128 + tap * 128);
#pragma unroll
      for (int k = 0; k < TN; ++k)
        __builtin_amdgcn_raw_ptr_buffer_load_lds(rs_w, (__attribute__((address_space(3))) void*)(b + 32 * k * ROWB), 16,
                                                 (int)(wo + (unsigned)(k * 32 * p.wrow * 4)), 0, 0, 0);
    };

    tile_setup(ts.tile(it));
    dma_halo(0, 0);
    dma_halo(1, 1);
#pragma unroll
    for (int e = 0; e < PRE; ++e) dma_tap(e, e);
    int g = 0;
    unsigned G = 0;
    int pend = 0;
    asm volatile("s_waitcnt vmcnt(0)" ::: "memory");
    __builtin_amdgcn_s_barrier();
    for (;;) {
      const HaloTiles::Next nx = ts.next(it);
      if constexpr (SLACK2) {
        if (pend >= BT * TN + HALO_I) asm volatile("s_waitcnt vmcnt(%0)" ::"n"(BT * TN + HALO_I) : "memory");
        else if (pend >= BT * TN) asm volatile("s_waitcnt vmcnt(%0)" ::"n"(BT * TN) : "memory");
        else asm volatile("s_waitcnt vmcnt(0)" ::: "memory");
      } else {
        asm volatile("s_waitcnt vmcnt(0)" ::: "memory");
      }
      __builtin_amdgcn_s_barrier();
      pend = 0;
#pragma unroll
      for (int e = 0; e < BT; ++e) {
        const int ta = g + PRE + e;
        if (ta < T) { dma_tap(ta, (int)((G + (unsigned)(PRE + e)) & (unsigned)(RS - 1))); pend += TN; }
        else if (nx.more) { dma_tap(ta - T, (int)((G + (unsigned)(PRE + e)) & (unsigned)(RS - 1))); pend += TN; }
      }
      const int t8 = (g / 9) * 9 - 1;
      if (t8 >= 0 && t8 >= g - BT) {
        const int died = t8 / 9, s2 = died + 2, stage = died & 1;
        if (s2 < nslices) { dma_halo(s2, stage); pend += HALO_I; }
        else if (nx.more) {
          tile_setup(nx.ntile);
          dma_halo(0, stage);
          pend += HALO_I;
        }
      }
      g += BT; G += (unsigned)BT;
      if (g == T) {
        __builtin_amdgcn_s_barrier();
        if (!nx.more) return;
        dma_halo(1, 1);
        pend += HALO_I;
        it = nx.nit;
        g = 0;
      }
    }
  }

  const int xl = lane & 31, half = lane >> 5;
  unsigned aaddr[4][3];
  auto make_aaddr = [&]() {
    int xo = xl;
    asm volatile("" : "+v"(xo));
    halo_frag_addrs(aaddr, lds0, wave_u, xo, half);
  };
  make_aaddr();
  unsigned bslot[RS];
#pragma unroll
  for (int k = 0; k < RS; ++k) bslot[k] = lds0 + (unsigned)(B_OFF + k * TAPB + xl * ROWB + ((half ^ swz(xl)) << 4));

  f16x8 fah[2][2], fal[2][2], fbh[2], fbl[2];

  auto read_a = [&](auto tap_c, auto s_c, auto i_c, auto lo_c, auto aoff_c) {
    constexpr int tap = decltype(tap_c)::value, sk = decltype(s_c)::value, i = decltype(i_c)::value;
    constexpr bool lo = decltype(lo_c)::value != 0;
    constexpr int kh = tap / 3, kw = tap % 3;
    const unsigned a = aaddr[i + kh][kw] ^ (unsigned)((lo ? 0x40 : 0) | (sk ? 0x20 : 0));
    if constexpr (lo) fal[sk][i] = lds_read128i<decltype(aoff_c)::value>(a);
    else fah[sk][i] = lds_read128i<decltype(aoff_c)::value>(a);
  };
  auto read_b = [&](unsigned base, auto j_c, auto s_c, auto lo_c, auto set_c) {
    constexpr int j = decltype(j_c)::value, sk = decltype(s_c)::value, set = decltype(set_c)::value;
    constexpr bool lo = decltype(lo_c)::value != 0;
    const unsigned b = base ^ (unsigned)((lo ? 0x40 : 0) | (sk ? 0x20 : 0));
    if constexpr (lo) fbl[set] = lds_read128i<j * 4096>(b);
    else fbh[set] = lds_read128i<j * 4096>(b);
  };

  __amdgpu_buffer_rsrc_t rs_out = __builtin_amdgcn_make_buffer_rsrc(p.out, 0, p.in2_bytes, 0x00020000);

  f32x16 acc[TN][2];
  clear_acc(acc);

  __builtin_amdgcn_s_barrier();
  __builtin_amdgcn_sched_barrier(0);

  using I0 = std::integral_constant<int, 0>;
  using I1 = std::integral_constant<int, 1>;
  auto first_frags = [&]() {
    read_a(I0{}, I0{}, I0{}, I1{}, I0{}); read_a(I0{}, I0{}, I1{}, I1{}, I0{});
    read_a(I0{}, I0{}, I0{}, I0{}, I0{}); read_a(I0{}, I0{}, I1{}, I0{}, I0{});
    read_b(bslot[0], I0{}, I0{}, I0{}, I0{}); read_b(bslot[0], I0{}, I0{}, I1{}, I0{});
  };
  first_frags();

  auto tap_step = [&](auto first_c, auto tap_c, auto aoff_x, unsigned bx, auto ntap_c, auto aoff_n, unsigned bn) {
    if constexpr (decltype(first_c)::value != 0) {
      __builtin_amdgcn_s_barrier();
      __builtin_amdgcn_sched_barrier(0);
    }
    fcp_static_for<0, 2>([&](auto sc) {
      constexpr int s = decltype(sc)::value;
      fcp_static_for<0, TN>([&](auto jc) {
        constexpr int j = decltype(jc)::value;
        constexpr int gi = s * TN + j, set = gi & 1, nset = set ^ 1;
        if constexpr (j == 1 || (j == 2 && TN == 4)) asm volatile("s_waitcnt lgkmcnt(2)" ::: "memory");
        else asm volatile("s_waitcnt lgkmcnt(0)" ::: "memory");
        __builtin_amdgcn_sched_barrier(0);
        auto mm = [&](int i, const f16x8& a, const f16x8& b) {
          acc[j][i] = __builtin_amdgcn_mfma_f32_32x32x16_f16(a, b, acc[j][i], 0, 0, 0);
          __builtin_amdgcn_sched_barrier(0);
        };
        auto rd_b = [&](auto lo_c) {
          if constexpr (j + 1 < TN) read_b(bx, std::integral_constant<int, j + 1>{}, sc, lo_c, std::integral_constant<int, nset>{});
          else if constexpr (s == 0) read_b(bx, I0{}, I1{}, lo_c, std::integral_constant<int, nset>{});
          else read_b(bn, I0{}, I0{}, lo_c, std::integral_constant<int, nset>{});
          __builtin_amdgcn_sched_barrier(0);
        };
        auto rd_a = [&](auto idx_c) {
          constexpr int idx = decltype(idx_c)::value;
          if constexpr (idx < 4) {
            using IC = std::integral_constant<int, idx & 1>;
            using LO = std::integral_constant<int, idx < 2 ? 1 : 0>;
            if constexpr (s == 0) read_a(tap_c, I1{}, IC{}, LO{}, aoff_x);
            else read_a(ntap_c, I0{}, IC{}, LO{}, aoff_n);
            __builtin_amdgcn_sched_barrier(0);
          }
        };
        mm(0, fal[s][0], fbh[set]); rd_b(I0{});
        mm(1, fal[s][1], fbh[set]); rd_b(I1{});
        mm(0, fah[s][0], fbl[set]); rd_a(std::integral_constant<int, j < 2 ? 2 * j : 4>{});
        mm(1, fah[s][1], fbl[set]); rd_a(std::integral_constant<int, j < 2 ? 2 * j + 1 : 4>{});
        mm(0, fah[s][0], fbh[set]);
        mm(1, fah[s][1], fbh[set]);
      });
    });
  };

  auto epilogue = [&]() {
    int e_ni, e_y0, e_x0;
    ts.coords(ts.tile(it), e_ni, e_y0, e_x0);
    const unsigned cs0 = lds0 + (unsigned)(A_BYTES + wave_u * 64 * 128);
    const int eq = lane & 3, er = lane >> 2;
    asm volatile("s_waitcnt lgkmcnt(0)" ::: "memory");
#pragma unroll
    for (int n = 0; n < TN; ++n) {
      asm volatile("" ::: "memory");
      __builtin_amdgcn_sched_barrier(0);
      const int ccol = n * 32 + eq * 8;
      const bool cvalid = ccol < p.cout;
      f32x4 b8[2], w8[2];
      halo_epi_consts(p, ccol, cvalid, b8, w8);
#pragma unroll
      for (int i = 0; i < 2; ++i)
#pragma unroll
        for (int rr = 0; rr < 16; ++rr) {
          const int row = i * 32 + mfma_c_row(rr, half);
          lds_write32(cs0 + (unsigned)((row * 32 + xl) * 4), acc[n][i][rr]);
        }
      __builtin_amdgcn_sched_barrier(0);
#pragma unroll
      for (int gp = 0; gp < (RES ? 2 : 4); ++gp) {
        constexpr int GN = RES ? 2 : 1;
        f32x4 va[GN], vb[GN];
#pragma unroll
        for (int g = 0; g < GN; ++g) {
          const unsigned ra = cs0 + (unsigned)(((er + 16 * (GN * gp + g)) * 32 + eq * 8) * 4);
          va[g] = lds_read128f(ra);
          vb[g] = lds_read128f(ra + 16);
        }
        asm volatile("s_waitcnt lgkmcnt(0)" ::: "memory");
        __builtin_amdgcn_sched_barrier(0);
#pragma unroll
        for (int g = 0; g < GN; ++g) {
          const int row = wave_u * 64 + er + 16 * (GN * gp + g);
          const int y = e_y0 + (row >> 5), x = e_x0 + (row & 31);
          const bool ok = cvalid && y < p.out_h && x < p.out_w;
          const long m = ok ? ((long)e_ni * p.out_h + y) * p.out_w + x : 0;
          float v[8] = {va[g][0], va[g][1], va[g][2], va[g][3], vb[g][0], vb[g][1], vb[g][2], vb[g][3]};
          if constexpr (RES) {
            float r1[8], r2[8];
            if (p.res1 != nullptr) load8(p.res1, m, p.res1_ld, cvalid ? ccol : 0, p.res1_fmt, r1);
            if (p.res2 != nullptr) load8(p.res2, m, p.res2_ld, cvalid ? ccol : 0, p.res2_fmt, r2);
#pragma unroll
            for (int e = 0; e < 8; ++e) v[e] = conv_value(p, v[e], w8[e >> 2][e & 3], b8[e >> 2][e & 3], r1[e], r2[e]);
          } else {
            const ConvEpi plain{false, false, false, p.act_slope, p.alpha, 1.f};
#pragma unroll
            for (int e = 0; e < 8; ++e) v[e] = conv_value(plain, v[e], w8[e >> 2][e & 3], b8[e >> 2][e & 3], 0.f, 0.f);
          }
          u32x4_t s0, s1;
          unsigned o0, o1;
          if (p.out_fmt == 1) {
            pack8(v, 1, s0, s1);
            o0 = (unsigned)(m * p.out_ld * 4 + split_chan_off(ccol));
            o1 = o0 + 64u;
          } else {
            pack8(v, 0, s0, s1);
            o0 = (unsigned)((m * p.out_ld + ccol) * 4);
            o1 = o0 + 16u;
          }
          __builtin_amdgcn_raw_buffer_store_b128(s0, rs_out, ok ? o0 : 0xFFFFFFFFu, 0, 0);
          __builtin_amdgcn_raw_buffer_store_b128(s1, rs_out, ok ? o1 : 0xFFFFFFFFu, 0, 0);
        }
      }
      __builtin_amdgcn_sched_barrier(0);
    }
    __builtin_amdgcn_s_barrier();
    __builtin_amdgcn_sched_barrier(0);
  };

  int unit = 0;
  const int nunits = nslices / 2;
  for (;;) {
    if (unit != 0 || it != ts.slot) make_aaddr();
    fcp_static_for<0, 18>([&](auto tc) {
      constexpr int t = decltype(tc)::value, tn = (t + 1) % 18;
      using OX = std::integral_constant<int, (t / 9) * A_BYTES>;
      using ON = std::integral_constant<int, (tn / 9) * A_BYTES>;
      tap_step(std::integral_constant<int, t % BT == 0 ? 1 : 0>{}, std::integral_constant<int, t % 9>{}, OX{}, bslot[t % RS],
               std::integral_constant<int, tn % 9>{}, ON{}, bslot[(t + 1) % RS]);
    });
    {
      const unsigned b0 = bslot[0], b1 = bslot[1];
      fcp_static_for<0, RS - 2>([&](auto kc) { bslot[decltype(kc)::value] = bslot[decltype(kc)::value + 2]; });
      bslot[RS - 2] = b0; bslot[RS - 1] = b1;
    }
    if (++unit == nunits) {
      const HaloTiles::Next nx = ts.next(it);
      __builtin_amdgcn_sched_barrier(0);
      epilogue();
      if (!nx.more) break;
      it = nx.nit;
      unit = 0;
      clear_acc(acc);
      first_frags();
    }
  }
}

}

namespace fcp_conv {

static int halo_grid(const ConvK& k, unsigned* grid) {
  const long tiles = (long)k.n * ((k.out_h + TH - 1) / TH) * ((k.out_w + TW - 1) / TW);
  FCP_REQUIRE(tiles < (1L << 31), "conv(halo): too many tiles");
  const int cus = fcp_cu_count();
  *grid = (unsigned)(tiles < cus ? tiles : cus);
  return 0;
}

int launch_f16x3_halo(const ConvK& k, hipStream_t s) {
  const size_t lds = (size_t)LDS_TOTAL;
  unsigned grid = 0;
  if (const int e = halo_grid(k, &grid)) return e;
  if (k.cout <= 32) {
    FCP_LDS_OPT_IN(&conv3x3_halo_f16x3<1>, lds);
    hipLaunchKernelGGL(conv3x3_halo_f16x3<1>, dim3(grid), dim3(512), lds, s, k);
  } else {
    FCP_LDS_OPT_IN(&conv3x3_halo_f16x3<2>, lds);
    hipLaunchKernelGGL(conv3x3_halo_f16x3<2>, dim3(grid), dim3(512), lds, s, k);
  }
  FCP_LAUNCH_OK();
  return 0;
}

constexpr int WIDE2_BT = 2;

int launch_f16x3_halo_wide(const ConvK& k, hipStream_t s) {
  const int tn = k.cout <= 64 ? 2 : 4;
  const size_t lds = (size_t)(2 * A_BYTES + (tn == 2 ? 8 : 4) * tn * 32 * ROWB);
  unsigned grid = 0;
  if (const int e = halo_grid(k, &grid)) return e;
  FCP_REQUIRE(k.ctiles >= 2 && k.ctiles % 2 == 0 && k.cout <= 128, "conv(halo, wide): cin must be a multiple of 64, cout <= 128");
  FCP_REQUIRE(tn == 2 || (k.res1 == nullptr && k.res2 == nullptr), "conv(halo, wide): no residual inputs with more than 64 filters");
  if (tn == 2) {
    FCP_LDS_OPT_IN((&conv3x3_halo_wide_f16x3<2, true, WIDE2_BT, 8>), lds);
    hipLaunchKernelGGL((conv3x3_halo_wide_f16x3<2, true, WIDE2_BT, 8>), dim3(grid), dim3(512), lds, s, k);
  } else {
    FCP_LDS_OPT_IN((&conv3x3_halo_wide_f16x3<4, false, 1, 4>), lds);
    hipLaunchKernelGGL((conv3x3_halo_wide_f16x3<4, false, 1, 4>), dim3(grid), dim3(512), lds, s, k);
  }
  FCP_LAUNCH_OK();
  return 0;
}

}
```

face-crop-plus_amd/engine.py:

```python
from __future__ import annotations

import contextlib
import ctypes as C
import os
import threading
from dataclasses import dataclass

import numpy as np
import torch

from . import _native as N
from . import torch_ops as T

BN_EPS = 1e-5
COUT_PAD = 128


class Act:
    __slots__ = ("buf", "c0", "c", "fmt")

    def __init__(self, buf: torch.Tensor, c0: int = 0, c: int | None = None, fmt: int = 0):
        assert buf.dim() == 4 and buf.dtype == torch.float32 and buf.is_contiguous()
        self.buf, self.c0, self.fmt = buf, c0, fmt
        self.c = buf.shape[3] - c0 if c is None else c
        assert 0 <= c0 and c0 + self.c <= buf.shape[3]
        if fmt == 1:
            assert c0 % 32 == 0 and self.c % 32 == 0 and buf.shape[3] % 32 == 0, "split32 views are 32-channel aligned"

    @staticmethod
    def empty(n, h, w, c, device, fmt: int = 0):
        return Act(torch.empty((n, h, w, c), dtype=torch.float32, device=device), fmt=fmt)

    @property
    def n(self): return self.buf.shape[0]
    @property
    def h(self): return self.buf.shape[1]
    @property
    def w(self): return self.buf.shape[2]
    @property
    def ld(self): return self.buf.shape[3]

    def slice(self, c0, c):
        return Act(self.buf, self.c0 + c0, c, self.fmt)

    def ptr(self):
        return N.ptr(self.buf, 4 * self.c0)

    def nchw(self) -> torch.Tensor:
        v = self.buf[..., self.c0:self.c0 + self.c].contiguous()
        if self.fmt == 1:
            v = split32_to_f32(Act(v, fmt=1)).buf
        return v.permute(0, 3, 1, 2).contiguous()


@dataclass
class PackedConv:
    w: torch.Tensor
    bias: torch.Tensor | None
    cin: int
    cout: int
    kh: int
    kw: int
    stride: int
    pad: int
    cin4: bool
    flops_per_pixel: int
    precision: int = 0
    wscale: torch.Tensor | None = None


def fold_bn(weight: np.ndarray, bn: dict | None, bias: np.ndarray | None):
    w = np.asarray(weight, dtype=np.float32)
    if bn is None:
        return w, (None if bias is None else np.asarray(bias, np.float32))
    f = np.float32
    alpha = (bn["weight"].astype(f) / np.sqrt(bn["running_var"].astype(f) + f(BN_EPS))).astype(f)
    beta = (bn["bias"].astype(f) - bn["running_mean"].astype(f) * alpha).astype(f)
    if bias is not None:
        beta = (beta + np.asarray(bias, f) * alpha).astype(f)
    return (w * alpha[:, None, None, None]).astype(f), beta


PRECISIONS = {"f32": 0, "fp32": 0, "exact": 0, 0: 0, "f16x3": 1, "fp16x3": 1, 1: 1}
DEFAULT_PRECISION = PRECISIONS[os.environ.get("FCP_PRECISION", "f16x3")]


def resolve_precision(p):
    if p is None:
        return DEFAULT_PRECISION
    if p not in PRECISIONS:
        raise ValueError(f"unknown precision {p!r}: use 'f32' (exact fp32 MFMA) or 'f16x3' (split fp16 MFMA)")
    return PRECISIONS[p]


@contextlib.contextmanager
def default_precision(p):
    global DEFAULT_PRECISION
    prev, DEFAULT_PRECISION = DEFAULT_PRECISION, resolve_precision(p)
    try:
        yield
    finally:
        DEFAULT_PRECISION = prev



def split_f16x3(packed: np.ndarray):
    rows = packed.reshape(packed.shape[0], -1).astype(np.float32)
    amax = np.abs(rows).max(1)
    e = np.where(amax > 0, np.floor(np.log2(np.maximum(amax, 1e-38))), 0.0)
    scale = np.exp2(e).astype(np.float32)
    ws = rows / scale[:, None]
    hi = ws.astype(np.float16)
    lo = (ws - hi.astype(np.float32)).astype(np.float16)
    k = rows.shape[1]
    assert k % 32 == 0
    img = np.empty((rows.shape[0], k // 32, 2, 32), np.float16)
    img[:, :, 0] = hi.reshape(rows.shape[0], k // 32, 32)
    img[:, :, 1] = lo.reshape(rows.shape[0], k // 32, 32)
    return img.reshape(rows.shape[0], k * 2).view(np.uint16), scale


def pack_conv(weight, bias=None, bn=None, stride=1, pad=0, device="cuda", cin_perm=None,
              precision: int | None = None) -> PackedConv:
    precision = resolve_precision(precision)
    if isinstance(weight, torch.Tensor):
        weight = weight.detach().cpu().numpy()
    if isinstance(bias, torch.Tensor):
        bias = bias.detach().cpu().numpy()
    if bn is not None:
        bn = {k: (v.detach().cpu().numpy() if isinstance(v, torch.Tensor) else np.asarray(v)) for k, v in bn.items()}
    w, b = fold_bn(weight, bn, bias)
    if cin_perm is not None:
        w = w[:, cin_perm]
    cout, cin, kh, kw = w.shape
    cout_pad = -(-cout // COUT_PAD) * COUT_PAD
    cin4 = cin <= 4
    if cin4:
        assert kw <= 8
        packed = np.zeros((cout_pad, kh, 8, 4), np.float32)
        packed[:cout, :, :kw, :cin] = w.transpose(0, 2, 3, 1)
    else:
        assert cin % 32 == 0, f"cin={cin} must be a multiple of 32"
        packed = np.zeros((cout_pad, cin // 32, kh, kw, 32), np.float32)
        packed[:cout] = w.transpose(0, 2, 3, 1).reshape(cout, kh, kw, cin // 32, 32).transpose(0, 3, 1, 2, 4)
    wsc = None
    if precision == 1:
        img, scale = split_f16x3(packed)
        wd = torch.from_numpy(np.ascontiguousarray(img.view(np.int16))).to(device)
        wsc = torch.from_numpy(scale).to(device)
    else:
        wd = torch.from_numpy(np.ascontiguousarray(packed)).to(device)
    bd = None if b is None else torch.from_numpy(np.ascontiguousarray(b)).to(device)
    return PackedConv(wd, bd, 4 if cin4 else cin, cout, kh, kw, stride, pad, cin4,
                      2 * cout * cin * kh * kw, precision, wsc)


def bn_of(sd, prefix):
    return {k: sd[f"{prefix}.{k}"] for k in ("weight", "bias", "running_mean", "running_var")}


def _pick_tile_n(cout: int, m: int) -> int:
    if cout <= 32:
        return 32
    gm = -(-m // 128)
    if cout % 128 == 0 and gm * (cout // 128) >= 512:
        return 128
    return 64


_props_lock = threading.Lock()
_props: dict = {}


def device_props(dev=None):
    idx = torch.cuda.current_device() if dev is None else (torch.device(dev).index if torch.device(dev).index is not None
                                                           else torch.cuda.current_device())
    got = _props.get(idx)
    if got is None:
        with _props_lock:
            got = _props.get(idx)
            if got is None:
                got = _props[idx] = torch.cuda.get_device_properties(idx)
    return got


class _StreamClaim:

    def __init__(self, dev_index, slot):
        self.dev_index, self.slot = dev_index, slot

    def __del__(self):
        try:
            with _stream_lock:
                _stream_free.setdefault(self.dev_index, set()).add(self.slot)
        except Exception:
            pass


_stream_lock = threading.RLock()
_stream_sets: dict = {}
_stream_free: dict = {}
_stream_tls = threading.local()


def thread_streams(dev) -> dict:
    dev = torch.device(dev)
    idx = dev.index if dev.index is not None else torch.cuda.current_device()
    claims = _stream_tls.__dict__.setdefault("claims", {})
    claim = claims.get(idx)
    with _stream_lock:
        sets = _stream_sets.setdefault(idx, [])
        if claim is None:
            free = _stream_free.setdefault(idx, set())
            slot = min(free) if free else len(sets)
            free.discard(slot)
            if slot == len(sets):
                sets.append({"main": None, "side": {}})
            claim = claims[idx] = _StreamClaim(idx, slot)
        return sets[claim.slot]


STREAM_PROBE = os.environ.get("FCP_STREAM_PROBE", "1") != "0"
_stream_rejects: list = []


def _streams_overlap(a, b, cycles: int = 1_500_000) -> bool:
    import time

    def timed(streams):
        for s_ in streams:
            s_.synchronize()
        t = time.perf_counter()
        for s_ in streams:
            with torch.cuda.stream(s_):
                torch.cuda._sleep(cycles)
        for s_ in streams:
            s_.synchronize()
        return time.perf_counter() - t
    timed([a])
    timed([b])
    one = min(timed([a]), timed([b]))
    return min(timed([a, b]), timed([a, b])) < 1.5 * one


def _new_stream_beside(dev, others, tries: int = 6):
    with torch.cuda.device(dev):
        cand = torch.cuda.Stream(device=dev)
        if not STREAM_PROBE or not others or not hasattr(torch.cuda, "_sleep") or torch.cuda.is_current_stream_capturing():
            return cand
        for _ in range(tries):
            try:
                if all(_streams_overlap(o, cand) for o in others):
                    return cand
            except Exception:
                return cand
            _stream_rejects.append(cand)
            cand = torch.cuda.Stream(device=dev)
        return cand


def thread_side_streams(dev, k: int, with_main: bool = False):
    st = thread_streams(dev)
    key = (k, bool(with_main))
    if key not in st["side"]:
        base = [thread_main_stream(dev)] if with_main else []
        with _stream_lock:
            side = list(base)
            while len(side) < k:
                side.append(_new_stream_beside(dev, side))
        st["side"][key] = side
    return st["side"][key]


def thread_main_stream(dev):
    st = thread_streams(dev)
    if st["main"] is None:
        with torch.cuda.device(dev):
            st["main"] = torch.cuda.Stream(device=dev)
    return st["main"]


_budget = threading.local()


@contextlib.contextmanager
def cu_budget(cus: int):
    prev = getattr(_budget, "cus", 0)
    _budget.cus = int(cus)
    try:
        yield
    finally:
        _budget.cus = prev


class Autotune:
    enabled = os.environ.get("FCP_AUTOTUNE", "1") != "0"
    use_tables = os.environ.get("FCP_TUNE_TABLES", "1") != "0"
    cache: dict = {}
    _lock = threading.Lock()
    TABLE_VERSION = 13
    _disk_loaded = False
    _disk_section = None
    _disk_dirty = False

    @classmethod
    def _user_path(cls):
        p = os.environ.get("FCP_TUNE_CACHE")
        if p == "0":
            return None
        return p or os.path.join(os.path.expanduser("~"), ".cache", "face_crop_plus_amd", "autotune.json")

    @classmethod
    def section(cls):
        if cls._disk_section is None:
            prop = device_props()
            arch = getattr(prop, "gcnArchName", prop.name).split(":")[0]
            cls._disk_section = f"{arch}|{prop.multi_processor_count}|abi{cls.TABLE_VERSION}"
        return cls._disk_section

    @classmethod
    def ensure_loaded(cls):
        if cls._disk_loaded or not cls.use_tables:
            return
        with cls._lock:
            if cls._disk_loaded:
                return
            cls._disk_loaded = True
            if os.environ.get("FCP_TUNE_CACHE") == "0":
                return
            import ast
            import json
            shipped = os.path.join(os.path.dirname(os.path.abspath(__file__)), "tuned")
            files = sorted(os.path.join(shipped, f) for f in os.listdir(shipped) if f.endswith(".json")) if os.path.isdir(shipped) else []
            if cls._user_path() and os.path.isfile(cls._user_path()):
                files.append(cls._user_path())
            try:
                sec = cls.section()
            except Exception:
                return
            for path in files:
                try:
                    with open(path) as f:
                        table = json.load(f).get(sec, {})
                    for k, v in table.items():
                        cls.cache.setdefault(ast.literal_eval(k), tuple(v))
                except Exception as e:
                    import warnings
                    warnings.warn(f"autotune table {path} ignored: {type(e).__name__}: {e}")

    @classmethod
    def save(cls, path: str | None = None):
        path = path or cls._user_path()
        if path is None:
            return None
        import json
        with cls._lock:
            table = {}
            try:
                with open(path) as f:
                    table = json.load(f)
            except Exception:
                pass
            sec = table.setdefault(cls.section(), {})
            for k, v in list(cls.cache.items()):
                sec[repr(k)] = list(v)
            os.makedirs(os.path.dirname(os.path.abspath(path)), exist_ok=True)
            tmp = f"{path}.{os.getpid()}.tmp"
            with open(tmp, "w") as f:
                json.dump(table, f, indent=0, sort_keys=True)
            os.replace(tmp, path)
            cls._disk_dirty = False
        return path

    @classmethod
    def choose(cls, key, candidates, trial_desc):
        cls.ensure_loaded()
        if not (cls.enabled or cls.cache):
            return None
        best = cls.cache.get(key)
        if best is not None and tuple(best) not in candidates:
            with cls._lock:
                cls.cache.pop(key, None)
            best = None
        if best is None and cls.enabled:
            d = trial_desc()
            base_flags = d.flags

            def trial(t):
                d.tile_m, d.tile_n, d.flags = t[0], t[1], base_flags | (t[2] if len(t) > 2 else 0)
                _c_launch("fcp_conv2d_nhwc_f32", C.byref(d))
            best = cls.pick(key, candidates, trial)
        return best

    @classmethod
    def pick(cls, key, candidates, launch):
        best = cls.cache.get(key)
        if best is not None:
            return best
        with cls._lock:
            best = cls.cache.get(key)
            if best is not None:
                return best
            times = []
            for t in candidates:
                launch(t)
                best_t = float("inf")
                for _ in range(3):
                    e0, e1 = torch.cuda.Event(enable_timing=True), torch.cuda.Event(enable_timing=True)
                    e0.record()
                    for _ in range(2):
                        launch(t)
                    e1.record()
                    e1.synchronize()
                    best_t = min(best_t, e0.elapsed_time(e1) / 2)
                times.append(best_t)
            tmin = min(times)
            best = next(c for c, t in zip(candidates, times) if t <= 1.02 * tmin)
            if os.environ.get("FCP_AUTOTUNE_LOG"):
                print("autotune", key, {str(c): round(t * 1e3, 1) for c, t in zip(candidates, times)}, "->", best, flush=True)
            cls.cache[key] = best
            cls._disk_dirty = True
        if os.environ.get("FCP_TUNE_CACHE") != "0":
            cls._save_soon()
        return best

    _last_save = 0.0
    _atexit = False

    @classmethod
    def _save_soon(cls):
        import time
        if not cls._atexit:
            import atexit
            cls._atexit = True
            atexit.register(cls._save_quietly)
        if time.monotonic() - cls._last_save >= 2.0:
            cls._save_quietly()

    @classmethod
    def _save_quietly(cls):
        import time
        if not cls._disk_dirty or os.environ.get("FCP_TUNE_CACHE") == "0":
            return
        try:
            cls.save()
        except Exception:
            pass
        cls._last_save = time.monotonic()


class ConvStats:
    timing = None
    replay = None


class RangeMonitor:
    active = None
    LIMIT = 32768.0

    def __init__(self):
        self.rows = []

    def __enter__(self):
        assert RangeMonitor.active is None, "RangeMonitor is not re-entrant"
        RangeMonitor.active = self
        return self

    def __exit__(self, *exc):
        RangeMonitor.active = None

    def see(self, label: str, t: Act):
        m = torch.zeros((), dtype=torch.float32, device=t.buf.device)
        N.check(N.lib().fcp_absmax_nhwc(t.ptr(), t.n * t.h * t.w, t.c, t.ld, t.fmt, N.ptr(m), N.stream_ptr()), "fcp_absmax_nhwc")
        self.rows.append((label, m))

    def report(self):
        return [(label, float(m.item())) for label, m in self.rows]

    def check(self, what: str):
        rep = self.report()
        bad = [(label, v) for label, v in rep if not v < self.LIMIT]
        if bad:
            worst = max(bad, key=lambda r: r[1])
            raise FloatingPointError(
                f"{what}: activations leave the range of the fp16x3 (split binary16) conv path: |x| reaches {worst[1]:.4g} "
                f"after '{worst[0]}' ({len(bad)} of {len(rep)} launches at or above 2^15 = {self.LIMIT:.0f}; binary16 "
                f"saturates at 65504).  Load the model with precision='f32' (exact fp32 MFMA path) for these weights.")
        return rep


def selfcheck_mode(weights) -> bool:
    mode = os.environ.get("FCP_SELFCHECK", "auto")
    from_checkpoint = weights is None or (isinstance(weights, str) and weights != "generated")
    return mode == "1" or (mode == "auto" and from_checkpoint)


SELFCHECK_HARD_TOL = 1e-2


def selfcheck_compare(what: str, got: torch.Tensor, ref: torch.Tensor, rel_tol: float) -> float:
    scale = float(ref.abs().max().item())
    diff = float((got - ref).abs().max().item()) / max(scale, 1e-30)
    if not diff <= rel_tol:
        msg = (f"{what}: the fp16x3 path and the exact-fp32 path disagree by {diff:.3g} of the output's "
               f"largest value (tolerance {rel_tol:g}, hard limit {SELFCHECK_HARD_TOL:g}) with these weights; load with precision='f32'.")
        if os.environ.get("FCP_SELFCHECK", "auto") == "1" or not diff <= SELFCHECK_HARD_TOL:
            raise FloatingPointError(msg)
        import warnings
        warnings.warn(msg)
    return diff


def selfcheck_at_load(model, sd, weights, precision, repack_f32):
    if model.precision != 1 or not selfcheck_mode(weights):
        return
    try:
        model.selfcheck(sd)
    except FloatingPointError as e:
        if precision is not None or os.environ.get("FCP_SELFCHECK", "auto") == "1":
            raise
        import warnings
        warnings.warn(f"{e}  Falling back to precision='f32' for this model.", RuntimeWarning)
        repack_f32()
        model.selfcheck_report = {"fallback": "f32", "reason": str(e)}


def _c_launch(fn: str, *args):
    N.check(getattr(N.lib(), fn)(*args, N.stream_ptr()), fn)


def _filter(pc: PackedConv | None):
    return (None, None, None) if pc is None else (pc.w, pc.wscale, pc.bias)


def _alias_safe_out(out: Act, *ins: Act | None) -> Act:
    st = out.buf.untyped_storage().data_ptr()
    if any(t is not None and t.buf.untyped_storage().data_ptr() == st and t.c0 < out.c0 + out.c and out.c0 < t.c0 + t.c
           for t in ins):
        return Act.empty(out.n, out.h, out.w, out.c, out.buf.device, out.fmt)
    return out


def _accounted(go, describe, relaunch):
    timing, replay = ConvStats.timing, ConvStats.replay
    if timing is not None:
        e0, e1 = torch.cuda.Event(enable_timing=True), torch.cuda.Event(enable_timing=True)
        e0.record()
    outs = go()
    if timing is None and replay is None and RangeMonitor.active is None:
        return outs
    label, mon_label, flops, byts = describe()
    if timing is not None:
        e1.record()
        timing.append((e0, e1, flops, label, byts))
    if replay is not None:
        fn, args, keep = relaunch(*outs)
        replay.append((label, flops, byts, lambda keep=keep: _c_launch(fn, *args)))
    mon = RangeMonitor.active
    if mon is not None:
        for i, t in enumerate(outs):
            if t is not None and t.c % 8 == 0:
                mon.see(mon_label if i == 0 else f"{mon_label} [output {i}]", t)
    return outs


def _conv_desc(pc: PackedConv, x: Act, out: Act, x2, x2_stride, res1, res1_pre, res2, alpha, alpha2, act_slope, in_up2, band,
               tile_m, tile_n, flags, cu_budget) -> N.ConvDesc:
    in_h, in_w = (x.h * 2, x.w * 2) if in_up2 else (x.h, x.w)
    d = N.ConvDesc()
    d.in_, d.w, d.out = x.ptr(), N.ptr(pc.w), out.ptr()
    if x2 is not None:
        d.in2, d.cin2, d.in2_ld, d.in2_h, d.in2_w, d.in2_stride = x2.ptr(), x2.c, x2.ld, x2.h, x2.w, x2_stride
    d.bias = N.ptr(pc.bias)
    d.wscale = N.ptr(pc.wscale)
    d.precision = pc.precision
    d.in_fmt, d.out_fmt = x.fmt, out.fmt
    d.res1_fmt = res1.fmt if res1 is not None else 0
    d.res2_fmt = res2.fmt if res2 is not None else 0
    d.res1 = res1.ptr() if res1 is not None else None
    d.res2 = res2.ptr() if res2 is not None else None
    d.n, d.in_h, d.in_w = x.n, in_h, in_w
    d.cin, d.in_ld, d.in_up2 = pc.cin, x.ld, int(in_up2)
    d.cout, d.kh, d.kw, d.stride, d.pad = pc.cout, pc.kh, pc.kw, pc.stride, pc.pad
    d.out_h, d.out_w, d.out_ld = out.h, out.w, out.ld
    d.tile_m, d.tile_n = tile_m, tile_n
    d.cin4 = int(pc.cin4)
    d.act_slope, d.alpha, d.alpha2 = act_slope, alpha, alpha2
    d.res1_pre = int(res1_pre)
    d.flags = flags
    d.cu_budget = cu_budget
    d.band_top, d.band_bottom = band
    if res1 is not None:
        d.res1_ld, d.res1_h, d.res1_w = res1.ld, res1.h, res1.w
    if res2 is not None:
        d.res2_ld = res2.ld
    return d


def conv(pc: PackedConv, x: Act, out: Act | None = None, *, act_slope: float = 1.0,
         alpha: float = 1.0, res1: Act | None = None, res1_pre: bool = True,
         res2: Act | None = None, alpha2: float = 1.0, in_up2: bool = False,
         tile_n: int | None = None, out_fmt: int = 0, tile_m: int | None = None,
         x2: Act | None = None, x2_stride: int = 1, flat: bool = False, balance_tail: bool = False,
         band: tuple[int, int] = (0, 0)) -> Act:
    assert x.c + (x2.c if x2 is not None else 0) == pc.cin, f"conv expects {pc.cin} input channels, got {x.c}"
    in_h, in_w = (x.h * 2, x.w * 2) if in_up2 else (x.h, x.w)
    oh = (in_h - band[0] - band[1] + 2 * pc.pad - pc.kh) // pc.stride + 1
    ow = (in_w + 2 * pc.pad - pc.kw) // pc.stride + 1
    if out is None:
        out = Act.empty(x.n, oh, ow, pc.cout, x.buf.device, out_fmt)
    assert (out.n, out.h, out.w, out.c) == (x.n, oh, ow, pc.cout), "conv: bad output view"
    if (x.fmt or out.fmt or (res1 is not None and res1.fmt) or (res2 is not None and res2.fmt)) and pc.precision != 1:
        raise ValueError("split32 tensors can only be used with filters packed for the fp16x3 path")
    assert x2 is None or (x2.fmt == 1 and x.fmt == 1 and x2.n == x.n), "two-source convs take split32 tensors"
    assert res1 is None or (res1.c == pc.cout and res1.n == x.n)
    assert res2 is None or (res2.n, res2.h, res2.w, res2.c) == (x.n, oh, ow, pc.cout)
    m = x.n * oh * ow
    tm, tn = tile_m or 128, tile_n or _pick_tile_n(pc.cout, m)
    flags = (N.CONV_FLAT_ADDR if flat else 0) | (N.CONV_BALANCE_TAIL if balance_tail else 0)
    cu = getattr(_budget, "cus", 0)
    desc = lambda o: _conv_desc(pc, x, o, x2, x2_stride, res1, res1_pre, res2, alpha, alpha2, act_slope, in_up2, band,
                                tm, tn, flags, cu)
    big_ok = (pc.precision == 1 and x.fmt == 1 and not pc.cin4 and not in_up2 and pc.cout % 8 == 0
              and pc.cout >= 128 and m >= 256 * 64)
    halo_ok = (pc.precision == 1 and x.fmt == 1 and not pc.cin4 and (pc.kh, pc.kw, pc.stride, pc.pad) == (3, 3, 1, 1)
               and pc.cout <= 64 and pc.cout % 8 == 0 and pc.cin >= 64 and x2 is None and (res1 is None or (res1.h, res1.w) == (oh, ow)))
    wide_ok = (pc.precision == 1 and x.fmt == 1 and not pc.cin4 and (pc.kh, pc.kw, pc.stride, pc.pad) == (3, 3, 1, 1)
               and pc.cout % 8 == 0 and pc.cin % 64 == 0 and x2 is None and 64 < pc.cout <= 128 and res1 is None and res2 is None)
    if tile_n is None and tile_m is None and (pc.cout > 64 or halo_ok):
        key = (pc.cin, pc.cout, pc.kh, pc.kw, pc.stride, m, int(in_up2), res1 is not None, res2 is not None,
               pc.precision, x.fmt, out.fmt, None if x2 is None else (x2.c, x2_stride), cu)
        best = Autotune.choose(key, tile_candidates(pc.cout, halo_ok, wide_ok, big_ok),
                               lambda: desc(_alias_safe_out(out, x, x2, res1, res2)))
        if best is not None:
            tm, tn = best[0], best[1]
            flags |= best[2] if len(best) > 2 else 0

    def go():
        if T.ENABLED:
            T.load().conv2d_out(x.buf, x.c0, pc.cin, pc.w, pc.bias, pc.wscale, None if res1 is None else res1.buf,
                                0 if res1 is None else res1.c0, None if res2 is None else res2.buf, 0 if res2 is None else res2.c0,
                                out.buf, out.c0, pc.cout, pc.kh, pc.kw, pc.stride, pc.pad, float(act_slope), float(alpha),
                                float(alpha2), bool(res1_pre), pc.precision, x.fmt, out.fmt, 0 if res1 is None else res1.fmt,
                                0 if res2 is None else res2.fmt, bool(in_up2), bool(pc.cin4), int(tm), int(tn),
                                None if x2 is None else x2.buf, 0 if x2 is None else x2.c0, 0 if x2 is None else x2.c,
                                int(x2_stride), int(flags), int(cu), int(band[0]), int(band[1]))
        else:
            _c_launch("fcp_conv2d_nhwc_f32", C.byref(desc(out)))
        return (out,)

    def describe():
        byts = 4 * (m * (pc.cout + (pc.cout if res1 is not None else 0) + (pc.cout if res2 is not None else 0))
                    + x.n * in_h * in_w * x.c // (4 if in_up2 else 1) + (m * x2.c if x2 is not None else 0)
                    + pc.cout * pc.cin * pc.kh * pc.kw)
        head = f"conv {pc.kh}x{pc.kw} s{pc.stride} {pc.cin}->{pc.cout} @{oh}x{ow}"
        return (f"{head} tile {tm}x{tn}{' bal' if flags & N.CONV_BALANCE_TAIL else ''}{' +res' if res1 is not None else ''}",
                head, pc.flops_per_pixel * m, byts)

    def relaunch(o):
        o = _alias_safe_out(o, x, x2, res1, res2)
        return "fcp_conv2d_nhwc_f32", (C.byref(desc(o)),), (pc, x, x2, res1, res2, o)
    return _accounted(go, describe, relaunch)[0]


def tile_candidates(cout: int, halo_ok: bool, wide_ok: bool, big_ok: bool):
    cands = [(128, 128), (128, 64)]
    if halo_ok:
        cands = ([(128, 32)] if cout <= 32 else []) + [(128, 64), (1, 32)]
    if wide_ok:
        cands = cands + [(1, 128)]
    if big_ok:
        big = [(256, 128)] + ([(256, 256)] if cout >= 256 else []) + ([(256, 192)] if 128 < cout <= 192 else [])
        cands += big
        cands += [(tm, tn, N.CONV_BALANCE_TAIL) for tm, tn in big]
    return cands


def chain_supported(pc2: PackedConv | None, pc3: PackedConv, pc1n: PackedConv | None, residual: bool = True, cb: int = 0) -> bool:
    convs = [pc for pc in (pc2, pc3, pc1n) if pc is not None]
    if not all(pc.precision == 1 and pc.bias is not None and not pc.cin4 for pc in convs):
        return False
    one = lambda pc, cin, cout: (pc.cin, pc.cout, pc.kh, pc.kw, pc.stride, pc.pad) == (cin, cout, 1, 1, 1, 0)
    if pc1n is None:
        return pc2 is None and residual and not cb and one(pc3, 256, 1024)
    if cb:
        return pc2 is None and not residual and cb == 256 and one(pc3, 384, 512) and one(pc1n, 512, 128)
    if pc2 is not None:
        return ((pc2.cin, pc2.cout, pc2.kh, pc2.kw, pc2.stride, pc2.pad) == (64, 64, 3, 3, 1, 1) and residual
                and one(pc3, 64, 256) and (one(pc1n, 256, 64) or one(pc1n, 256, 128)))
    if residual:
        return ((one(pc3, 128, 512) and (one(pc1n, 512, 128) or one(pc1n, 512, 256)))
                or (one(pc3, 256, 1024) and one(pc1n, 1024, 256)))
    return one(pc3, 128, 256) and one(pc1n, 256, 64)



def _chain_desc(pc2, pc3, pc1n, t1, res, out, t1n, tile_m, flags, t1b, t1b_stride) -> N.ChainDesc:
    d = N.ChainDesc()
    d.t1, d.res, d.out = t1.ptr(), (res.ptr() if res is not None else None), out.ptr()
    d.t1n = t1n.ptr() if t1n is not None else None
    d.w2, d.ws2, d.b2 = map(N.ptr, _filter(pc2))
    d.w3, d.ws3, d.b3 = map(N.ptr, _filter(pc3))
    d.w1n, d.ws1n, d.b1n = map(N.ptr, _filter(pc1n))
    d.n, d.h, d.w, d.c, d.nout = t1.n, t1.h, t1.w, pc3.cin, pc3.cout
    d.cn = pc1n.cout if pc1n is not None else 0
    d.t1_ld, d.res_ld, d.out_ld = t1.ld, (res.ld if res is not None else 0), out.ld
    d.t1n_ld = t1n.ld if t1n is not None else 0
    d.tile_m, d.flags = tile_m, flags
    if t1b is not None:
        d.t1b, d.cb, d.t1b_ld, d.t1b_h, d.t1b_w, d.t1b_stride = t1b.ptr(), t1b.c, t1b.ld, t1b.h, t1b.w, t1b_stride
    return d


def bottleneck_chain(pc2: PackedConv | None, pc3: PackedConv, pc1n: PackedConv, t1: Act, res: Act | None,
                     out: Act | None = None, t1n: Act | None = None, tile_m: int = 0, out_even_only: bool = False,
                     t1b: Act | None = None, t1b_stride: int = 1):
    cb = t1b.c if t1b is not None else 0
    assert chain_supported(pc2, pc3, pc1n, res is not None, cb), "bottleneck_chain: unsupported shapes"
    assert t1.fmt == 1 and t1.c + cb == pc3.cin and (res is None or (res.fmt == 1 and res.c == pc3.cout))
    assert t1b is None or (t1b.fmt == 1 and t1b.n == t1.n and (t1.h - 1) * t1b_stride < t1b.h and (t1.w - 1) * t1b_stride < t1b.w)
    assert res is None or (t1.n, t1.h, t1.w) == (res.n, res.h, res.w)
    c, nout, cn = pc3.cin, pc3.cout, (pc1n.cout if pc1n is not None else 0)
    flags = N.CHAIN_OUT_EVEN_ONLY if (out_even_only and pc2 is not None and RangeMonitor.active is None) else 0
    via_op = T.ENABLED and out is None and t1n is None
    if not via_op:
        if out is None:
            out = Act.empty(t1.n, t1.h, t1.w, nout, t1.buf.device, 1)
        if t1n is None and pc1n is not None:
            t1n = Act.empty(t1.n, t1.h, t1.w, cn, t1.buf.device, 1)
        assert out.fmt == 1 and (out.n, out.h, out.w, out.c) == (t1.n, t1.h, t1.w, nout)
        assert pc1n is None or (t1n.fmt == 1 and (t1n.n, t1n.h, t1n.w, t1n.c) == (t1.n, t1.h, t1.w, cn))
    desc = lambda o, o1n: _chain_desc(pc2, pc3, pc1n, t1, res, o, o1n, tile_m, flags, t1b, t1b_stride)

    def go():
        if not via_op:
            _c_launch("fcp_bottleneck_chain_f16x3", C.byref(desc(out, t1n)))
            return out, t1n
        o, t = T.load().bottleneck_chain(t1.buf, t1.c0, None if res is None else res.buf, 0 if res is None else res.c0,
                                         *_filter(pc2), *_filter(pc3), *_filter(pc1n), c, nout, cn, tile_m, flags,
                                         None if t1b is None else t1b.buf, 0 if t1b is None else t1b.c0, cb, int(t1b_stride))
        return Act(o, fmt=1), (Act(t, fmt=1) if pc1n is not None else None)

    def describe():
        m = t1.n * t1.h * t1.w
        flops = ((pc2.flops_per_pixel if pc2 is not None else 0) + pc3.flops_per_pixel
                 + (pc1n.flops_per_pixel if pc1n is not None else 0)) * m
        byts = 4 * (m * (c + (nout if not flags else nout // 4) + (nout if res is not None else 0) + cn) + (0 if pc2 is None else 9 * c * c)
                    + c * nout + nout * cn)
        if pc1n is None:
            head = f"expand {c}->{nout} @{t1.h}x{t1.w}"
            return f"{head} +res", head, flops, byts
        head = f"chain {'3x3 ' if pc2 is not None else ''}{c}->{nout}->{cn} @{t1.h}x{t1.w}"
        return (f"{head}{' +res' if res is not None else ''}{' out@even' if flags else ''}{' two-source' if t1b is not None else ''}",
                head, flops, byts)

    def relaunch(o, o1n):
        o = _alias_safe_out(o, t1, res, t1b)
        o1n = o1n if o1n is None else _alias_safe_out(o1n, t1, res, t1b)
        return "fcp_bottleneck_chain_f16x3", (C.byref(desc(o, o1n)),), (pc2, pc3, pc1n, t1, res, o, o1n, t1b)
    return _accounted(go, describe, relaunch)


def u8_to_nhwc4(images_u8: torch.Tensor, sub=(0.0, 0.0, 0.0), div: float = 1.0) -> Act:
    assert images_u8.dtype == torch.uint8 and images_u8.dim() == 4 and images_u8.shape[3] == 3
    assert images_u8.is_contiguous()
    n, h, w, _ = images_u8.shape
    out = Act.empty(n, h, w, 4, images_u8.device)
    sub_arr = (C.c_float * 3)(*[float(s) for s in sub])
    N.check(N.lib().fcp_u8_to_nhwc4_f32(N.ptr(images_u8), out.ptr(), n * h * w, sub_arr, float(div),
                                        N.stream_ptr()), "fcp_u8_to_nhwc4_f32")
    return out


@dataclass
class PackedStem:
    wfrag: torch.Tensor
    bias: torch.Tensor
    wscale: torch.Tensor
    flops_per_pixel: int


def pack_stem_fused(weight, bn, device, cin_perm=None) -> PackedStem:
    if isinstance(weight, torch.Tensor):
        weight = weight.detach().cpu().numpy()
    bn = {k: (v.detach().cpu().numpy() if isinstance(v, torch.Tensor) else np.asarray(v)) for k, v in bn.items()}
    w, b = fold_bn(weight, bn, None)
    if cin_perm is not None:
        w = w[:, cin_perm]
    assert w.shape == (64, 3, 7, 7), "the fused stem is the ResNet 7x7 / 64-filter stem"
    wk = np.zeros((64, 22 * 8), np.float32)
    wk.reshape(64, 22, 8)
    for kh in range(7):
        wk[:, kh * 24:kh * 24 + 21] = w[:, :, kh, :].transpose(0, 2, 1).reshape(64, 21)
    amax = np.abs(wk).max(1)
    e = np.where(amax > 0, np.floor(np.log2(np.maximum(amax, 1e-38))), 0.0)
    scale = np.exp2(e).astype(np.float32)
    ws = wk / scale[:, None]
    hi = ws.astype(np.float16)
    lo = (ws - hi.astype(np.float32)).astype(np.float16)
    frag = np.zeros((2, 11, 2, 64, 8), np.float16)
    lane = np.arange(64)
    for ct in range(2):
        n = ct * 32 + (lane & 31)
        for q in range(11):
            ch = 2 * q + (lane >> 5)
            k = ch[:, None] * 8 + np.arange(8)[None, :]
            frag[ct, q, 0] = hi[n[:, None], k]
            frag[ct, q, 1] = lo[n[:, None], k]
    return PackedStem(torch.from_numpy(np.ascontiguousarray(frag.view(np.int16))).to(device),
                      torch.from_numpy(np.ascontiguousarray(b)).to(device), torch.from_numpy(scale).to(device),
                      2 * 64 * 3 * 49)


def stem_conv1_supported(pc1: PackedConv | None) -> bool:
    return (pc1 is not None and pc1.precision == 1 and pc1.bias is not None and not pc1.cin4
            and (pc1.cin, pc1.cout, pc1.kh, pc1.kw, pc1.stride, pc1.pad) == (64, 64, 1, 1, 1, 0))


def stem_relu_pool_u8(ps: PackedStem, images_u8: torch.Tensor, out: Act | None = None, mean_rgb=(123, 117, 104),
                      out_fmt: int = 1, conv1: PackedConv | None = None, t1: Act | None = None):
    assert images_u8.dtype == torch.uint8 and images_u8.dim() == 4 and images_u8.shape[3] == 3 and images_u8.is_contiguous()
    n, h, w, _ = images_u8.shape
    hs, ws = (h - 1) // 2 + 1, (w - 1) // 2 + 1
    hp, wp = (hs - 1) // 2 + 1, (ws - 1) // 2 + 1
    if out is None:
        out = Act.empty(n, hp, wp, 64, images_u8.device, out_fmt)
    assert (out.n, out.h, out.w, out.c) == (n, hp, wp, 64), "stem: bad output view"
    mean = (C.c_int32 * 3)(*[int(m) for m in mean_rgb])
    if conv1 is not None:
        assert stem_conv1_supported(conv1) and out.fmt == 1, "stem + conv1: 1x1 64 -> 64 fp16x3 conv on a split32 pooled map"
        if t1 is None:
            t1 = Act.empty(n, hp, wp, 64, images_u8.device, 1)
        assert t1.fmt == 1 and (t1.n, t1.h, t1.w, t1.c) == (n, hp, wp, 64)

    def args(o, o1):
        a = (N.ptr(images_u8), n, h, w, mean, N.ptr(ps.wfrag), N.ptr(ps.bias), N.ptr(ps.wscale), o.ptr(), o.ld, o.fmt)
        if conv1 is None:
            return "fcp_stem7x7s2_relu_pool_u8", a
        return "fcp_stem7x7s2_relu_pool_conv1_u8", a + (N.ptr(conv1.w), N.ptr(conv1.wscale), N.ptr(conv1.bias), o1.ptr(), o1.ld)

    def go():
        fn, a = args(out, t1)
        _c_launch(fn, *a)
        return out, t1

    def describe():
        flops = ps.flops_per_pixel * n * hs * ws + (conv1.flops_per_pixel * n * hp * wp if conv1 is not None else 0)
        byts = n * h * w * 3 + 4 * n * hp * wp * 64 * (2 if conv1 is not None else 1)
        return (f"stem 7x7 s2 + pool{' + conv1' if conv1 is not None else ''} @{hp}x{wp}", f"stem 7x7 s2 + pool @{hp}x{wp}",
                flops, byts)
    relaunch = lambda o, o1: (*args(o, o1), (ps, images_u8, o, conv1, o1))
    _accounted(go, describe, relaunch)
    return out if conv1 is None else (out, t1)


def stem_relu_pool_f32(ps: PackedStem, x4: Act, out: Act | None = None, out_fmt: int = 1) -> Act:
    assert x4.fmt == 0 and x4.c0 == 0 and x4.c == 4 and x4.ld == 4, "the fused fp32 stem reads a dense NHWC4 tensor"
    n, h, w = x4.n, x4.h, x4.w
    hs, ws = (h - 1) // 2 + 1, (w - 1) // 2 + 1
    hp, wp = (hs - 1) // 2 + 1, (ws - 1) // 2 + 1
    if out is None:
        out = Act.empty(n, hp, wp, 64, x4.buf.device, out_fmt)
    assert (out.n, out.h, out.w, out.c) == (n, hp, wp, 64), "stem: bad output view"
    args = lambda o: (x4.ptr(), n, h, w, N.ptr(ps.wfrag), N.ptr(ps.bias), N.ptr(ps.wscale), o.ptr(), o.ld, o.fmt)

    def go():
        _c_launch("fcp_stem7x7s2_relu_pool_f32", *args(out))
        return (out,)

    def describe():
        label = f"stem(f32) 7x7 s2 + pool @{hp}x{wp}"
        return label, label, ps.flops_per_pixel * n * hs * ws, n * h * w * 16 + 4 * n * hp * wp * 64

    def relaunch(o):
        o = _alias_safe_out(o, x4)
        return "fcp_stem7x7s2_relu_pool_f32", args(o), (ps, x4, o)
    return _accounted(go, describe, relaunch)[0]


def f32nchw_to_nhwc4(images: torch.Tensor, sub=(0.0, 0.0, 0.0), div: float = 1.0) -> Act:
    assert images.dtype == torch.float32 and images.dim() == 4 and images.shape[1] == 3
    images = images.contiguous()
    n, _, h, w = images.shape
    out = Act.empty(n, h, w, 4, images.device)
    sub_arr = (C.c_float * 3)(*[float(s) for s in sub])
    N.check(N.lib().fcp_f32nchw_to_nhwc4_f32(N.ptr(images), out.ptr(), n, h, w, sub_arr, float(div),
                                             N.stream_ptr()), "fcp_f32nchw_to_nhwc4_f32")
    return out


def maxpool3x3s2(x: Act, out: Act | None = None) -> Act:
    assert x.c0 == 0 and x.c == x.ld
    oh, ow = (x.h + 2 - 3) // 2 + 1, (x.w + 2 - 3) // 2 + 1
    if out is None:
        out = Act.empty(x.n, oh, ow, x.c, x.buf.device, x.fmt)
    assert (out.n, out.h, out.w, out.c, out.fmt) == (x.n, oh, ow, x.c, x.fmt), "maxpool: bad output view"
    fn = N.lib().fcp_maxpool3x3s2_split32 if x.fmt == 1 else N.lib().fcp_maxpool3x3s2_nhwc_f32
    N.check(fn(x.ptr(), out.ptr(), x.n, x.h, x.w, x.c, out.ld, oh, ow, N.stream_ptr()), "fcp_maxpool3x3s2")
    return out


def f32_to_split32(x: Act) -> Act:
    assert x.fmt == 0 and x.c0 == 0 and x.c == x.ld and x.c % 32 == 0
    out = Act.empty(x.n, x.h, x.w, x.c, x.buf.device, 1)
    N.check(N.lib().fcp_f32_to_split32(x.ptr(), out.ptr(), x.n * x.h * x.w, x.c, N.stream_ptr()), "fcp_f32_to_split32")
    return out


def split32_to_f32(x: Act) -> Act:
    assert x.fmt == 1 and x.c0 == 0 and x.c == x.ld
    out = Act.empty(x.n, x.h, x.w, x.c, x.buf.device, 0)
    N.check(N.lib().fcp_split32_to_f32(x.ptr(), out.ptr(), x.n * x.h * x.w, x.c, N.stream_ptr()), "fcp_split32_to_f32")
    return out
```

face-crop-plus_amd/retinaface.py:

```python
from __future__ import annotations


import os
import threading

import numpy as np
import torch

from . import _native as N
from . import engine as E
from . import torch_ops as T
from .weights import load_state_dict

STRATEGIES = {"all": 0, "best": 1, "largest": 2}


class RetinaFace:
    WEIGHTS_FILENAME = "retinaface_detector.pth"

    def __init__(self, strategy: str = "all", vis: float = 0.6):
        self.strategy = strategy
        self.vis_threshold = vis
        self.nms_threshold = 0.4
        self.variance = [0.1, 0.2]
        self.device = None
        self._p = None
        self.precision = 0
        self.fused_chain = True
        self.streams = int(os.environ.get("FCP_DET_STREAMS", "2"))
        self.min_images_per_stream = 6
        self._tls = threading.local()

    def load(self, device: str | torch.device = "cuda:0", weights=None, precision=None):
        device = torch.device(device)
        if device.type != "cuda":
            raise RuntimeError("face_crop_plus_amd runs on an AMD GPU only (device must be cuda:N / hip); "
                               "there is no CPU fallback")
        N.lib()
        self.device = device
        sd = load_state_dict("retinaface", weights, device=device)
        self._repack(sd, precision)
        E.device_props(device)
        E.selfcheck_at_load(self, sd, weights, precision, lambda: self._repack(sd, "f32"))
        return self

    def _repack(self, sd, precision):
        with torch.cuda.device(self.device), E.default_precision(precision):
            self._p = self._pack(sd, self.device)
        self.precision = E.resolve_precision(precision)

    @torch.no_grad()
    def selfcheck(self, sd=None, images_u8: torch.Tensor | None = None, rel_tol: float = 1e-4):
        if self.precision != 1:
            self.selfcheck_report = {"skipped": "exact-fp32 path: nothing to guard"}
            return self.selfcheck_report
        dev = self.device
        with torch.cuda.device(dev):
            if images_u8 is None:
                g = torch.Generator(device="cpu").manual_seed(20260928)
                s = 256
                ramp = (torch.arange(s)[:, None] + torch.arange(s)[None, :]).clamp(max=255).to(torch.uint8)
                images_u8 = torch.stack([torch.randint(0, 256, (s, s, 3), generator=g, dtype=torch.uint8),
                                         torch.full((s, s, 3), 255, dtype=torch.uint8), torch.zeros((s, s, 3), dtype=torch.uint8),
                                         ramp[..., None].expand(s, s, 3).contiguous()]).to(dev)
            images_u8 = images_u8.to(dev).contiguous()
            tuning, E.Autotune.enabled = E.Autotune.enabled, False
            try:
                with E.RangeMonitor() as mon:
                    heads = self.forward_heads(None, images_u8) if "stem_fused" in self._p else \
                        self.forward_heads(E.u8_to_nhwc4(images_u8, sub=(123.0, 117.0, 104.0)))
                rep = {"launch_absmax": mon.check("RetinaFace"), "limit": E.RangeMonitor.LIMIT, "head_rel_diff": None}
                if sd is not None:
                    twin = RetinaFace(self.strategy, self.vis_threshold)
                    twin.device, twin.precision = dev, 0
                    with E.default_precision("f32"):
                        twin._p = self._pack(sd, dev)
                    ref = twin.forward_heads(E.u8_to_nhwc4(images_u8, sub=(123.0, 117.0, 104.0)))
                    rep["head_rel_diff"] = [E.selfcheck_compare("RetinaFace head maps", a.buf, b.buf, rel_tol)
                                            for a, b in zip(heads, ref)]
                    del twin, ref
                    torch.cuda.empty_cache()
            finally:
                E.Autotune.enabled = tuning
        self.selfcheck_report = rep
        return rep

    @staticmethod
    def _pack(sd, dev):
        p = {}
        pc, bn = E.pack_conv, E.bn_of
        p["stem"] = pc(sd["body.conv1.weight"], None, bn(sd, "body.bn1"), 2, 3, dev, cin_perm=[2, 1, 0])
        if E.DEFAULT_PRECISION == 1:
            p["stem_fused"] = E.pack_stem_fused(sd["body.conv1.weight"], bn(sd, "body.bn1"), dev, cin_perm=[2, 1, 0])
        blocks = []
        for li, nb in enumerate((3, 4, 6, 3), 1):
            for b in range(nb):
                pre = f"body.layer{li}.{b}"
                stride = 2 if (b == 0 and li > 1) else 1
                blk = {
                    "c1": pc(sd[pre + ".conv1.weight"], None, bn(sd, pre + ".bn1"), 1, 0, dev),
                    "c2": pc(sd[pre + ".conv2.weight"], None, bn(sd, pre + ".bn2"), stride, 1, dev),
                    "c3": pc(sd[pre + ".conv3.weight"], None, bn(sd, pre + ".bn3"), 1, 0, dev),
                    "ds": None, "feat": (b == nb - 1 and li >= 2),
                }
                if (pre + ".downsample.0.weight") in sd:
                    blk["ds"] = pc(sd[pre + ".downsample.0.weight"], None, bn(sd, pre + ".downsample.1"),
                                   stride, 0, dev)
                    if stride == 1 or E.DEFAULT_PRECISION == 1:
                        fold = lambda cw, cb: E.fold_bn(sd[pre + cw].numpy(), {q: v.numpy() for q, v in bn(sd, pre + cb).items()}, None)
                        (w3, b3), (wd, bd) = fold(".conv3.weight", ".bn3"), fold(".downsample.0.weight", ".downsample.1")
                        blk["c3ds"] = pc(np.concatenate([w3, wd], 1), b3 + bd, None, 1, 0, dev)
                blocks.append(blk)
        p["blocks"] = blocks
        for i in (1, 2, 3):
            p[f"fpn.output{i}"] = pc(sd[f"fpn.output{i}.0.weight"], None, bn(sd, f"fpn.output{i}.1"), 1, 0, dev)
        for i in (1, 2):
            p[f"fpn.merge{i}"] = pc(sd[f"fpn.merge{i}.0.weight"], None, bn(sd, f"fpn.merge{i}.1"), 1, 1, dev)
        head_perm = list(range(0, 128)) + list(range(192, 256)) + list(range(128, 192))
        for k in (1, 2, 3):
            def folded(nm):
                return E.fold_bn(sd[f"ssh{k}.{nm}.0.weight"].numpy(), {q: v.numpy() for q, v in bn(sd, f"ssh{k}.{nm}.1").items()}, None)
            w_b, b_b = folded("conv5X5_1")
            w_a, b_a = folded("conv3X3")
            p[f"ssh{k}.ab"] = pc(np.concatenate([w_b, w_a]), np.concatenate([b_b, b_a]), None, 1, 1, dev)
            w_c, b_c = folded("conv5X5_2")
            w_d, b_d = folded("conv7X7_2")
            p[f"ssh{k}.cd"] = pc(np.concatenate([w_c, w_d]), np.concatenate([b_c, b_d]), None, 1, 1, dev)
            w_e, b_e = folded("conv7x7_3")
            p[f"ssh{k}.e"] = pc(w_e, b_e, None, 1, 1, dev)
            i = k - 1
            hw = np.concatenate([sd[f"{h}.{i}.conv1x1.weight"].numpy() for h in ("ClassHead", "BboxHead", "LandmarkHead")])
            hb = np.concatenate([sd[f"{h}.{i}.conv1x1.bias"].numpy() for h in ("ClassHead", "BboxHead", "LandmarkHead")])
            p[f"head{k}"] = pc(hw, hb, None, 1, 0, dev, cin_perm=head_perm)
        return p

    def forward_heads(self, x4: E.Act | None, images_u8: torch.Tensor | None = None, heads_out=None):
        p = self._p
        f = 1 if self.precision == 1 else 0
        stem_t1 = None
        if images_u8 is not None and "stem_fused" in p:
            n, h, w, _ = images_u8.shape
            hp, wp = ((h - 1) // 2) // 2 + 1, ((w - 1) // 2) // 2 + 1
            cat = E.Act.empty(n, hp, wp, 128, images_u8.device, f)
            c1 = p["blocks"][0]["c1"]
            if f == 1 and E.stem_conv1_supported(c1):
                x, stem_t1 = E.stem_relu_pool_u8(p["stem_fused"], images_u8, cat.slice(64, 64), conv1=c1)
            else:
                x = E.stem_relu_pool_u8(p["stem_fused"], images_u8, cat.slice(64, 64))
        else:
            x = E.conv(p["stem"], x4, act_slope=0.0, out_fmt=f)
            cat = E.Act.empty(x.n, (x.h + 1) // 2, (x.w + 1) // 2, 2 * x.c, x.buf.device, f)
            x = E.maxpool3x3s2(x, cat.slice(x.c, x.c))
        feats = []
        blocks, pre = p["blocks"], stem_t1
        chain = bool(f) and self.fused_chain
        for bi, blk in enumerate(blocks):
            o = pre if pre is not None else E.conv(blk["c1"], x, act_slope=0.0, out_fmt=f)
            pre = None
            nxt = blocks[bi + 1] if bi + 1 < len(blocks) else None
            if (chain and blk["ds"] is None and not blk["feat"] and nxt is not None
                    and E.chain_supported(blk["c2"], blk["c3"], nxt["c1"])):
                sparse = "c3ds" in nxt and nxt["c2"].stride == 2 and not blk["feat"]
                x, pre = E.bottleneck_chain(blk["c2"], blk["c3"], nxt["c1"], o, x, out_even_only=sparse)
                continue
            if "c3ds" in blk and blk["c2"].stride == 1:
                E.conv(blk["c2"], o, cat.slice(0, o.c), act_slope=0.0)
                if chain and nxt is not None and E.chain_supported(None, blk["c3ds"], nxt["c1"], residual=False):
                    x, pre = E.bottleneck_chain(None, blk["c3ds"], nxt["c1"], cat, None)
                else:
                    x = E.conv(blk["c3ds"], cat, act_slope=0.0, out_fmt=f)
                del cat
                continue
            if "c3ds" in blk:
                o = E.conv(blk["c2"], o, act_slope=0.0, out_fmt=f)
                if (chain and not blk["feat"] and nxt is not None
                        and E.chain_supported(None, blk["c3ds"], nxt["c1"], residual=False, cb=x.c)):
                    x, pre = E.bottleneck_chain(None, blk["c3ds"], nxt["c1"], o, None, t1b=x, t1b_stride=blk["c2"].stride)
                    continue
                x = E.conv(blk["c3ds"], o, act_slope=0.0, out_fmt=f, x2=x, x2_stride=blk["c2"].stride)
                if blk["feat"]:
                    feats.append(x)
                continue
            o = E.conv(blk["c2"], o, act_slope=0.0, out_fmt=f)
            if (chain and blk["ds"] is None and nxt is not None and E.chain_supported(None, blk["c3"], nxt["c1"])):
                x, pre = E.bottleneck_chain(None, blk["c3"], nxt["c1"], o, x)
                if blk["feat"]:
                    feats.append(x)
                continue
            idt = x if blk["ds"] is None else E.conv(blk["ds"], x, out_fmt=f)
            x = E.conv(blk["c3"], o, act_slope=0.0, res1=idt, res1_pre=True, out_fmt=f)
            if blk["feat"]:
                feats.append(x)
        if getattr(self, "_debug_feats", None) is not None:
            self._debug_feats.extend(feats)
        o3 = E.conv(p["fpn.output3"], feats[2], act_slope=0.0, out_fmt=f)
        o2 = E.conv(p["fpn.output2"], feats[1], act_slope=0.0, res1=o3, res1_pre=False, out_fmt=f)
        o2 = E.conv(p["fpn.merge2"], o2, act_slope=0.0, out_fmt=f)
        o1 = E.conv(p["fpn.output1"], feats[0], act_slope=0.0, res1=o2, res1_pre=False, out_fmt=f)
        o1 = E.conv(p["fpn.merge1"], o1, act_slope=0.0, out_fmt=f)
        heads = []
        for k, ft in zip((1, 2, 3), (o1, o2, o3)):
            s = E.Act.empty(ft.n, ft.h, ft.w, 384, ft.buf.device, f)
            E.conv(p[f"ssh{k}.ab"], ft, s.slice(0, 192), act_slope=0.0)
            E.conv(p[f"ssh{k}.cd"], s.slice(0, 64), s.slice(256, 128), act_slope=0.0)
            E.conv(p[f"ssh{k}.e"], s.slice(320, 64), s.slice(192, 64), act_slope=0.0)
            heads.append(E.conv(p[f"head{k}"], s.slice(64, 256),
                                None if heads_out is None else heads_out[k - 1]))
        return heads

    def _side_streams(self, dev, k):
        main = E.thread_streams(dev)["main"]
        return E.thread_side_streams(dev, k, with_main=main is not None and torch.cuda.current_stream(dev) == main)

    MAX_OPERAND_BYTES = 0xFFFFFFF0

    def _images_per_launch(self, h: int, w: int) -> int | None:
        if self.precision != 1:
            return None
        hp, wp = ((h - 1) // 2) // 2 + 1, ((w - 1) // 2) // 2 + 1
        return max(1, (self.MAX_OPERAND_BYTES - 1) // (4 * 256 * hp * wp))

    def _streams_for(self, n: int) -> int:
        k = min(self.streams, n // max(1, self.min_images_per_stream))
        return 1 if k < 2 or torch.cuda.is_current_stream_capturing() else k

    def _chunked(self, n: int, h: int, w: int, dev, run, split: bool = True):
        per = self._images_per_launch(h, w)
        q = 1
        while True:
            bounds = [n * i // q for i in range(q + 1)]
            sub = lambda c: -(-c // (self._streams_for(c) if split else 1))
            if per is None or all(sub(b - a) <= per for a, b in zip(bounds[:-1], bounds[1:])):
                break
            q += 1
        if q == 1:
            return run(0, n, None)
        heads = [E.Act.empty(n, -(-h // s), -(-w // s), 32, dev) for s in (8, 16, 32)]
        for a, b in zip(bounds[:-1], bounds[1:]):
            run(a, b, [E.Act(hd.buf[a:b]) for hd in heads])
        return heads

    def _forward_heads_split(self, images_u8: torch.Tensor, heads_out=None):
        n, h, w, _ = images_u8.shape
        k = self._streams_for(n)
        if k < 2:
            return self.forward_heads(None, images_u8, heads_out)
        dev = images_u8.device
        heads = heads_out if heads_out is not None else [E.Act.empty(n, -(-h // s), -(-w // s), 32, dev) for s in (8, 16, 32)]
        cur = torch.cuda.current_stream(dev)
        bounds = [n * i // k for i in range(k + 1)]
        side = self._side_streams(dev, k)
        cus = E.device_props(dev).multi_processor_count // k
        for st, a, b in zip(side, bounds[:-1], bounds[1:]):
            tuned = len(E.Autotune.cache)
            if st != cur:
                st.wait_stream(cur)
            with torch.cuda.stream(st), E.cu_budget(cus):
                self.forward_heads(None, images_u8[a:b], [E.Act(hd.buf[a:b]) for hd in heads])
            if len(E.Autotune.cache) != tuned:
                st.synchronize()
        for st in side:
            if st != cur:
                cur.wait_stream(st)
        return heads

    def detect(self, images_u8: torch.Tensor | None = None, *, x4: E.Act | None = None,
               paddings: torch.Tensor | None = None, max_faces: int | None = None, want_dense: bool = False):
        if self.strategy not in STRATEGIES:
            raise ValueError(f"Unsupported startegy: {self.strategy}")
        fused = x4 is None and "stem_fused" in self._p
        if x4 is None and not fused:
            x4 = E.u8_to_nhwc4(images_u8, sub=(123.0, 117.0, 104.0))
        if fused:
            images_u8 = images_u8.contiguous()
            (n, h, w), dev = images_u8.shape[:3], images_u8.device
            heads = self._chunked(n, h, w, dev, lambda a, b, ho: self._forward_heads_split(images_u8[a:b], ho))
        else:
            n, h, w = x4.n, x4.h, x4.w
            dev = x4.buf.device
            heads = self._chunked(n, h, w, dev, lambda a, b, ho: self.forward_heads(x4 if (a, b) == (0, n) else E.Act(x4.buf[a:b]),
                                                                                    None, ho), split=False)
        P = sum(2 * (-(-h // s)) * (-(-w // s)) for s in (8, 16, 32))
        f32, i32 = torch.float32, torch.int32
        cand_score = torch.empty((n, P), dtype=f32, device=dev)
        cand_box = torch.empty((n, P, 4), dtype=f32, device=dev)
        cand_ldm = torch.empty((n, P, 10), dtype=f32, device=dev)
        cand_prior = torch.empty((n, P), dtype=i32, device=dev)
        cand_count = torch.empty((n,), dtype=i32, device=dev)
        dense = (None, None, None)
        if want_dense:
            dense = (torch.empty((n, P), dtype=f32, device=dev), torch.empty((n, P, 4), dtype=f32, device=dev),
                     torch.empty((n, P, 10), dtype=f32, device=dev))
        if T.ENABLED and not want_dense:
            return self._postprocess_ops(heads, n, h, w, P, paddings, max_faces)
        st = N.stream_ptr()
        lib = N.lib()
        N.check(lib.fcp_retina_decode(heads[0].ptr(), heads[1].ptr(), heads[2].ptr(), n, h, w,
                                      float(self.vis_threshold), float(self.variance[0]), float(self.variance[1]),
                                      N.ptr(cand_score), N.ptr(cand_box), N.ptr(cand_ldm), N.ptr(cand_prior),
                                      N.ptr(cand_count), N.ptr(dense[0]), N.ptr(dense[1]), N.ptr(dense[2]), st),
                "fcp_retina_decode")
        out = nms_select(cand_score, cand_box, cand_count, self.nms_threshold, self.strategy)
        if max_faces is None:
            max_faces = n if self.strategy != "all" else int(out["sel_count"].sum().item())
        max_faces = max(int(max_faces), 1)
        landmarks = torch.empty((max_faces, 5, 2), dtype=f32, device=dev)
        img_idx = torch.empty((max_faces,), dtype=i32, device=dev)
        face_offset = torch.empty((n + 1,), dtype=i32, device=dev)
        if paddings is not None:
            paddings = paddings.to(device=dev, dtype=i32).contiguous()
        N.check(lib.fcp_retina_gather_faces(N.ptr(cand_ldm), N.ptr(out["sel_pos"]), N.ptr(out["sel_count"]), n, P,
                                            N.ptr(paddings), max_faces, N.ptr(face_offset), N.ptr(landmarks),
                                            N.ptr(img_idx), st), "fcp_retina_gather_faces")
        out.update(landmarks=landmarks, img_idx=img_idx, face_offset=face_offset, cand_score=cand_score,
                   cand_box=cand_box, cand_ldm=cand_ldm, cand_prior=cand_prior, cand_count=cand_count,
                   heads=heads, dense=dense, max_faces=max_faces)
        return out

    def _postprocess_ops(self, heads, n, h, w, P, paddings, max_faces):
        ops = T.load()
        dev = heads[0].buf.device
        cand_score, cand_box, cand_ldm, cand_prior, cand_count = ops.retina_decode(
            heads[0].buf, heads[1].buf, heads[2].buf, h, w, float(self.vis_threshold), float(self.variance[0]),
            float(self.variance[1]))
        keep_pos, keep_count, sel_pos, sel_count = ops.nms_select(cand_score, cand_box, cand_count, float(self.nms_threshold),
                                                                  STRATEGIES[self.strategy])
        if max_faces is None:
            max_faces = n if self.strategy != "all" else int(sel_count.sum().item())
        max_faces = max(int(max_faces), 1)
        if paddings is not None:
            paddings = paddings.to(device=dev, dtype=torch.int32).contiguous()
        landmarks, img_idx, face_offset = ops.gather_faces(cand_ldm, sel_pos, sel_count, paddings, max_faces)
        return dict(keep_pos=keep_pos, keep_count=keep_count, sel_pos=sel_pos, sel_count=sel_count, landmarks=landmarks,
                    img_idx=img_idx, face_offset=face_offset, cand_score=cand_score, cand_box=cand_box, cand_ldm=cand_ldm,
                    cand_prior=cand_prior, cand_count=cand_count, heads=heads, dense=(None, None, None), max_faces=max_faces)

    def graphed(self, n: int, h: int, w: int, paddings: torch.Tensor | None = None):
        if self.strategy == "all":
            raise ValueError('graph capture needs a bounded face count: strategy "best" or "largest"')
        key = (n, h, w, None if paddings is None else tuple(paddings.flatten().tolist()))
        cache = self.__dict__.setdefault("_graphs", {})
        if key in cache:
            return cache[key]
        with torch.cuda.device(self.device):
            static = torch.zeros((n, h, w, 3), dtype=torch.uint8, device=self.device)
            prev, E.Autotune.enabled = E.Autotune.enabled, True
            side = torch.cuda.Stream(device=self.device)
            side.wait_stream(torch.cuda.current_stream())
            with torch.cuda.stream(side):
                for _ in range(2):
                    self.detect(static, paddings=paddings, max_faces=n)
            torch.cuda.current_stream().wait_stream(side)
            E.Autotune.enabled = False
            graph = torch.cuda.CUDAGraph()
            with torch.cuda.graph(graph):
                res = self.detect(static, paddings=paddings, max_faces=n)
            E.Autotune.enabled = prev
        cache[key] = (static, res, graph)
        return cache[key]

    @torch.no_grad()
    def predict(self, images: torch.Tensor):
        with torch.cuda.device(self.device):
            if images.dtype == torch.uint8:
                res = self.detect(images.to(self.device).contiguous())
            else:
                x4 = E.f32nchw_to_nhwc4(images.to(self.device, torch.float32), sub=(123.0, 117.0, 104.0))
                res = self.detect(x4=x4)
            nf = int(res["face_offset"][-1].item())
            nf = min(nf, res["max_faces"])
            landmarks = res["landmarks"][:nf].cpu().numpy()
            indices = res["img_idx"][:nf].cpu().numpy().astype(np.int64).tolist()
        return landmarks, indices


def nms_select(cand_score, cand_box, cand_count, nms_threshold=0.4, strategy="all"):
    if strategy not in STRATEGIES:
        raise ValueError(f"Unsupported startegy: {strategy}")
    n, cap = cand_score.shape
    dev = cand_score.device
    i32 = torch.int32
    lib = N.lib()
    ws = torch.empty((int(lib.fcp_retina_nms_workspace_bytes(n, cap)),), dtype=torch.uint8, device=dev)
    keep_pos = torch.empty((n, cap), dtype=i32, device=dev)
    keep_count = torch.empty((n,), dtype=i32, device=dev)
    sel_pos = torch.empty((n, cap), dtype=i32, device=dev)
    sel_count = torch.empty((n,), dtype=i32, device=dev)
    N.check(lib.fcp_retina_nms_select(N.ptr(cand_score), N.ptr(cand_box), N.ptr(cand_count), n, cap,
                                      float(nms_threshold), STRATEGIES[strategy], N.ptr(ws), N.ptr(keep_pos),
                                      N.ptr(keep_count), N.ptr(sel_pos), N.ptr(sel_count), N.stream_ptr()),
            "fcp_retina_nms_select")
    return dict(keep_pos=keep_pos, keep_count=keep_count, sel_pos=sel_pos, sel_count=sel_count)
```

face-crop-plus_amd/torch_ops.py:

```python
from __future__ import annotations

import os

import torch

_HERE = os.path.dirname(os.path.abspath(__file__))
LIB_PATH = os.path.join(_HERE, "csrc", "libfcp_torch.so")
_loaded = False


def _default_enabled() -> bool:
    mode = os.environ.get("FCP_BOUNDARY", "auto").lower()
    if mode == "ctypes":
        return False
    if mode == "torch":
        return True
    if os.path.isfile(LIB_PATH):
        return True
    import warnings
    warnings.warn(f"{LIB_PATH} is missing (the torch.ops.fcp veneer was not built): calling the C ABI through ctypes")
    return False


ENABLED = _default_enabled()


def load():
    global _loaded
    if not _loaded:
        if not os.path.isfile(LIB_PATH):
            raise RuntimeError(f"torch op library not built: {LIB_PATH} is missing "
                               f"(run `python face-crop-plus_amd/build_native.py`)")
        torch.ops.load_library(LIB_PATH)
        from ._native import ABI_VERSION
        built, running = torch.ops.fcp.abi_version()
        if built != ABI_VERSION or running != ABI_VERSION:
            raise RuntimeError(f"libfcp_torch.so is stale: compiled against ABI {built}, libfcp_hip.so reports {running}, "
                               f"host code expects {ABI_VERSION}; rebuild (python face-crop-plus_amd/build_native.py --force)")
        _loaded = True
    return torch.ops.fcp


OPS = ("conv2d", "conv2d_out", "bottleneck_chain", "retina_decode", "nms_select", "gather_faces", "similarity_from_5pt",
       "warp_affine_u8", "warp_affine_u8_float", "warp_affine_u8_ragged", "resize_area_u8_ragged", "bicubic_down4_round",
       "parse_argmax_hist", "warp_affine_u8_interp", "warp_affine_u8_interp_ragged", "crop_sharpness", "jpeg_encode", "matte", "clahe", "matte_blur",
       "jpeg_encode_ex", "jpeg_huffman_tables", "matte_refine", "matte_alpha", "matte_blur_alpha",
       "subject_mask", "png_encode", "png_huffman_lengths", "feather_alpha", "cutout", "mask_shift", "nlm_denoise")
```

include/fcp_hip.h:

```cpp
#ifndef FCP_HIP_H
#define FCP_HIP_H

#include <stdint.h>

#ifdef __cplusplus
extern "C" {
#endif

#define FCP_ABI_VERSION 15

typedef void* fcp_stream_t;

int fcp_abi_version(void);
const char* fcp_last_error(void);

typedef struct fcp_conv_desc {
  const float* in;
  const void* w;
  const float* bias;
  float* out;
  const float* res1;
  const float* res2;
  const float* wscale;
  const float* in2;
  int32_t n, in_h, in_w;
  int32_t cin, in_ld;
  int32_t in_up2;
  int32_t cout, kh, kw, stride, pad;
  int32_t out_h, out_w, out_ld;
  int32_t tile_n;
  int32_t cin4;
  float act_slope, alpha, alpha2;
  int32_t res1_pre, res1_ld, res1_h, res1_w, res2_ld;
  int32_t precision;
  int32_t in_fmt, out_fmt, res1_fmt, res2_fmt;
  int32_t tile_m;
  int32_t cin2, in2_ld, in2_h, in2_w, in2_stride;
  int32_t flags;
  int32_t cu_budget;
  int32_t band_top, band_bottom;
} fcp_conv_desc;

#define FCP_CONV_FLAT_ADDR 1
#define FCP_CONV_BALANCE_TAIL 2

int fcp_conv2d_nhwc_f32(const fcp_conv_desc* desc, fcp_stream_t stream);

typedef struct fcp_chain_desc {
  const float* t1;
  const void* w2;  const float* ws2;  const float* b2;
  const void* w3;  const float* ws3;  const float* b3;
  const float* res;
  float* out;
  const void* w1n; const float* ws1n; const float* b1n;
  float* t1n;
  const float* t1b;
  int32_t n, h, w, c, cn;
  int32_t t1_ld, res_ld, out_ld, t1n_ld;
  int32_t nout;
  int32_t tile_m;
  int32_t flags;
  int32_t cb, t1b_ld, t1b_h, t1b_w, t1b_stride;
} fcp_chain_desc;
#define FCP_CHAIN_OUT_EVEN_ONLY 1

int fcp_bottleneck_chain_f16x3(const fcp_chain_desc* desc, fcp_stream_t stream);

int fcp_u8_to_nhwc4_f32(const uint8_t* in, float* out, int64_t npix,
                        const float* sub_host, float div, fcp_stream_t stream);

int fcp_f32nchw_to_nhwc4_f32(const float* in, float* out, int n, int h, int w,
                             const float* sub_host, float div, fcp_stream_t stream);

int fcp_maxpool3x3s2_nhwc_f32(const float* in, float* out, int n, int h, int w, int c, int out_ld,
                              int out_h, int out_w, fcp_stream_t stream);
int fcp_maxpool3x3s2_split32(const float* in, float* out, int n, int h, int w, int c, int out_ld,
                             int out_h, int out_w, fcp_stream_t stream);
int fcp_stem7x7s2_relu_pool_u8(const uint8_t* images, int n, int h, int w, const int32_t* mean_rgb,
                               const void* wfrag, const float* bias, const float* wscale, float* out,
                               int out_ld, int out_fmt, fcp_stream_t stream);
int fcp_stem7x7s2_relu_pool_conv1_u8(const uint8_t* images, int n, int h, int w, const int32_t* mean_rgb,
                                     const void* wfrag, const float* bias, const float* wscale, float* out,
                                     int out_ld, int out_fmt, const void* w1, const float* ws1, const float* b1,
                                     float* t1, int t1_ld, fcp_stream_t stream);
int fcp_stem7x7s2_relu_pool_f32(const float* x4, int n, int h, int w, const void* wfrag, const float* bias,
                                const float* wscale, float* out, int out_ld, int out_fmt, fcp_stream_t stream);
int fcp_f32_to_split32(const float* in, float* out, int64_t npix, int c, fcp_stream_t stream);
int fcp_split32_to_f32(const float* in, float* out, int64_t npix, int c, fcp_stream_t stream);
int fcp_absmax_nhwc(const float* x, int64_t npix, int c, int ld, int fmt, float* out_max, fcp_stream_t stream);


int fcp_retina_decode(const float* head0, const float* head1, const float* head2,
                      int n, int img_h, int img_w, float vis_threshold,
                      float var0, float var1,
                      float* cand_score, float* cand_box, float* cand_ldm,
                      int32_t* cand_prior, int32_t* cand_count,
                      float* dense_score, float* dense_box, float* dense_ldm,
                      fcp_stream_t stream);

int64_t fcp_retina_nms_workspace_bytes(int n, int cap);
int fcp_retina_nms_select(const float* cand_score, const float* cand_box,
                          const int32_t* cand_count, int n, int cap,
                          float nms_threshold, int strategy, void* workspace,
                          int32_t* keep_pos, int32_t* keep_count,
                          int32_t* sel_pos, int32_t* sel_count, fcp_stream_t stream);

int fcp_retina_gather_faces(const float* cand_ldm, const int32_t* sel_pos,
                            const int32_t* sel_count, int n, int cap,
                            const int32_t* paddings, int max_faces,
                            int32_t* face_offset, float* out_ldm, int32_t* out_img,
                            fcp_stream_t stream);


int fcp_estimate_transform(const float* src, const float* dst, int f, int k,
                           int allow_skew, double* mat, int32_t* ok, fcp_stream_t stream);

int fcp_estimate_transform_counted(const float* src, const float* dst, int f, int k,
                                   int allow_skew, const int32_t* face_count,
                                   double* mat, int32_t* ok, int64_t* valid_total,
                                   fcp_stream_t stream);

int fcp_warp_affine_u8(const uint8_t* images, int n, int h, int w,
                       const int32_t* img_idx, const double* mat, const int32_t* ok,
                       const int32_t* paddings, int f, int out_h, int out_w, int border,
                       uint8_t* out, fcp_stream_t stream);

int fcp_warp_affine_u8_float(const uint8_t* images, int n, int h, int w,
                             const int32_t* img_idx, const double* mat, const int32_t* ok,
                             const int32_t* paddings, int f, int out_h, int out_w, int border,
                             uint8_t* out, fcp_stream_t stream);

typedef struct fcp_warp_src {
  int64_t off;
  int32_t h, w;
} fcp_warp_src;

int fcp_warp_affine_u8_ragged(const uint8_t* blob, int64_t blob_bytes,
                              const fcp_warp_src* srcs_host, const fcp_warp_src* srcs_dev,
                              const double* mat, const int32_t* ok, int f, int out_h, int out_w,
                              int border, uint8_t* out, fcp_stream_t stream);
int fcp_warp_affine_u8_float_ragged(const uint8_t* blob, int64_t blob_bytes,
                                    const fcp_warp_src* srcs_host, const fcp_warp_src* srcs_dev,
                                    const double* mat, const int32_t* ok, int f, int out_h,
                                    int out_w, int border, uint8_t* out, fcp_stream_t stream);

int fcp_warp_affine_u8_interp(const uint8_t* images, int n, int h, int w,
                              const int32_t* img_idx, const double* mat, const int32_t* ok,
                              const int32_t* paddings, int f, int out_h, int out_w, int border,
                              int interp, uint8_t* out, fcp_stream_t stream);
int fcp_warp_affine_u8_interp_ragged(const uint8_t* blob, int64_t blob_bytes,
                                     const fcp_warp_src* srcs_host, const fcp_warp_src* srcs_dev,
                                     const double* mat, const int32_t* ok, int f, int out_h,
                                     int out_w, int border, int interp, uint8_t* out,
                                     fcp_stream_t stream);

int fcp_warp_interp_weights(int interp, int16_t* out);

int fcp_crop_sharpness_u8(const uint8_t* crops, int f, int h, int w, const int32_t* ok,
                          int64_t* sums, fcp_stream_t stream);

int64_t fcp_jpeg_workspace_bytes(int f, int h, int w, int channels);
int fcp_jpeg_encode_u8(const uint8_t* crops, int f, int h, int w, int channels, int quality, int subsampling,
                       uint8_t* out, int64_t out_stride, int64_t capacity, int32_t* lengths,
                       void* workspace, int64_t workspace_bytes, fcp_stream_t stream);

int64_t fcp_jpeg_workspace_bytes_ex(int f, int h, int w, int channels, int subsampling, int optimize);
int fcp_jpeg_encode_ex_u8(const uint8_t* crops, int f, int h, int w, int channels, int quality,
                          int subsampling, int optimize,
                          uint8_t* out, int64_t out_stride, int64_t capacity, int32_t* lengths,
                          uint8_t* tables, void* workspace, int64_t workspace_bytes, fcp_stream_t stream);

int fcp_jpeg_huffman_tables(const uint32_t* freq, int n, uint8_t* tables, uint32_t* codes, fcp_stream_t stream);

int64_t fcp_png_workspace_bytes(int f, int h, int w, int channels);
int fcp_png_encode_u8(const uint8_t* pixels, int f, int h, int w, int channels,
                      uint8_t* out, int64_t out_stride, int64_t capacity, int32_t* lengths,
                      void* workspace, int64_t workspace_bytes, fcp_stream_t stream);

int fcp_png_huffman_lengths(const uint32_t* freq, int n, uint8_t* lengths, uint32_t* codes, fcp_stream_t stream);

int fcp_matte_u8(const uint8_t* crops, const uint8_t* labels, int f, int h, int w, uint32_t class_bits, int feather,
                 int bg_r, int bg_g, int bg_b, uint8_t* out, uint8_t* alpha, fcp_stream_t stream);

int64_t fcp_matte_blur_workspace_bytes(int f, int h, int w);
int fcp_matte_blur_u8(const uint8_t* crops, const uint8_t* labels, int f, int h, int w, uint32_t class_bits, int feather,
                      const uint16_t* taps, int radius, uint8_t* out, uint8_t* alpha, void* workspace, int64_t workspace_bytes,
                      fcp_stream_t stream);

int64_t fcp_matte_refine_workspace_bytes(int f, int h, int w);
int fcp_matte_refine_u8(const uint8_t* crops, const uint8_t* labels, int f, int h, int w, uint32_t class_bits, int radius, int eps,
                        uint8_t* alpha_out, void* workspace, int64_t workspace_bytes, fcp_stream_t stream);

int fcp_matte_alpha_u8(const uint8_t* crops, const uint8_t* alpha, int f, int h, int w, int bg_r, int bg_g, int bg_b, uint8_t* out,
                       fcp_stream_t stream);
int fcp_matte_blur_alpha_u8(const uint8_t* crops, const uint8_t* labels, const uint8_t* alpha, int f, int h, int w,
                            uint32_t class_bits, const uint16_t* taps, int radius, uint8_t* out, void* workspace,
                            int64_t workspace_bytes, fcp_stream_t stream);

#define FCP_CUTOUT_RGBA 0
#define FCP_CUTOUT_FILL 1
int fcp_feather_alpha_u8(const uint8_t* labels, int f, int h, int w, uint32_t class_bits, int feather, uint8_t* alpha_out,
                         fcp_stream_t stream);
int64_t fcp_cutout_workspace_bytes(int f, int h, int w);
int fcp_cutout_u8(const uint8_t* crops, const uint8_t* alpha, int f, int h, int w, int mode, int bg_r, int bg_g, int bg_b,
                  const uint16_t* taps, int radius, uint8_t* out, void* workspace, int64_t workspace_bytes, fcp_stream_t stream);

int64_t fcp_subject_mask_workspace_bytes(int f, int h, int w);
int fcp_subject_mask_u8(const uint8_t* labels, int f, int h, int w, uint32_t class_bits, int keep_largest, int max_hole, uint8_t* out,
                        void* workspace, int64_t workspace_bytes, fcp_stream_t stream);

int fcp_mask_shift_u8(const uint8_t* labels, int f, int h, int w, uint32_t class_bits, int shift, uint8_t* out,
                      fcp_stream_t stream);

int fcp_clahe_u8(const uint8_t* crops, int f, int h, int w, int grid, double clip_limit, uint8_t* luts, uint8_t* out, fcp_stream_t stream);

int fcp_nlm_denoise_u8(const uint8_t* crops, int f, int h, int w, const uint16_t* lut, int lut_len, int shift, uint8_t* out,
                       fcp_stream_t stream);


int fcp_bise_preprocess_u8(const uint8_t* faces, int f, int h, int w, float* out,
                           int out_h, int out_w, const float* mean_host,
                           const float* std_host, fcp_stream_t stream);

int fcp_avgpool_nhwc_f32(const float* in, int n, int hw, int c, int ld, float* out,
                         fcp_stream_t stream);

int fcp_fc_f32(const float* in, const float* w, const float* scale, const float* shift,
               int n, int cin, int cout, int act, float* out, fcp_stream_t stream);

int fcp_scale_add_nhwc_f32(const float* x, int x_ld, const float* scale_nc,
                           const float* add_nc, const float* add_t, int add_t_ld,
                           int n, int hw, int c, float* out, int out_ld, fcp_stream_t stream);

int fcp_parse_tail(const float* logits, int f, int lh, int lw, int ld, int ncls,
                   int mid_h, int mid_w, int out_h, int out_w, uint8_t* labels,
                   int32_t* counts, fcp_stream_t stream);

int fcp_label_mask_u8(const uint8_t* labels, int64_t total, uint32_t class_bits,
                      uint8_t* mask, fcp_stream_t stream);

int fcp_bicubic_down4_u8(const float* x4, int h, int w, int ld, uint8_t* out_rgb,
                         fcp_stream_t stream);

typedef struct fcp_batch_item {
  int64_t src_off;
  int32_t sh, sw;
  int32_t dh, dw;
  int32_t top, left;
  int32_t interp;
  int32_t reserved;
} fcp_batch_item;

int fcp_build_batch_u8(const uint8_t* src_blob, int64_t blob_bytes,
                       const fcp_batch_item* items_host, const fcp_batch_item* items_dev,
                       int n, int out_h, int out_w, int border, uint8_t* out,
                       fcp_stream_t stream);

typedef struct fcp_area_level {
  int64_t src_off;
  int32_t sh, sw;
  int64_t dst_off;
  int32_t dh, dw;
} fcp_area_level;

int fcp_resize_area_ragged_u8(const uint8_t* src_blob, int64_t src_bytes,
                              const fcp_area_level* levels_host, const fcp_area_level* levels_dev,
                              int n, uint8_t* dst_blob, int64_t dst_bytes, fcp_stream_t stream);

#ifdef __cplusplus
}
#endif
#endif
```

Before: 1400 faces/s.

## Group the three SSH pyramid levels' convs into single multi-problem kernel launches

Adds grouped-launch variants of the DMA, halo, halo-wide and big f16x3 conv kernels. A block-range prefix table maps each workgroup to one of up to four independent conv problems. The RetinaFace SSH and head convs for the three FPN levels are now issued as one launch per stage instead of three. This is meant to cut launch overhead and to let the small, under-occupied coarse-level convs share the GPU with the large level. The risks are extra per-block member lookup, copying a larger kernel argument struct, and losing the persistent scheduling in the big-kernel grouped path.

Result: no change. 1405 faces/s (median of 6 runs) (+0.3%).

```diff
diff --git a/face-crop-plus_amd/_native.py b/face-crop-plus_amd/_native.py
--- a/face-crop-plus_amd/_native.py
+++ b/face-crop-plus_amd/_native.py
@@ -33,6 +33,7 @@
 
 CONV_FLAT_ADDR = 1
 CONV_BALANCE_TAIL = 2
+CONV_GROUP_MAX = 4
 CHAIN_OUT_EVEN_ONLY = 1
 
 
@@ -46,6 +47,7 @@
 _P, _I, _F, _L = C.c_void_p, C.c_int, C.c_float, C.c_int64
 SIGNATURES = {
     "fcp_conv2d_nhwc_f32": [C.POINTER(ConvDesc), _P],
+    "fcp_conv2d_group_f16x3": [C.POINTER(ConvDesc), _I, _P],
     "fcp_bottleneck_chain_f16x3": [C.POINTER(ChainDesc), _P],
     "fcp_u8_to_nhwc4_f32": [_P, _P, _L, C.POINTER(C.c_float), _F, _P],
     "fcp_f32nchw_to_nhwc4_f32": [_P, _P, _I, _I, _I, C.POINTER(C.c_float), _F, _P],
@@ -98,7 +100,8 @@
 }
 EXPORTS = ["fcp_abi_version", "fcp_last_error", "fcp_retina_nms_workspace_bytes", "fcp_jpeg_workspace_bytes",
            "fcp_jpeg_workspace_bytes_ex", "fcp_matte_blur_workspace_bytes", "fcp_matte_refine_workspace_bytes",
-           "fcp_subject_mask_workspace_bytes", "fcp_png_workspace_bytes", "fcp_cutout_workspace_bytes"] + list(SIGNATURES)
+           "fcp_subject_mask_workspace_bytes", "fcp_png_workspace_bytes", "fcp_cutout_workspace_bytes",
+           "fcp_conv_kernel_id"] + list(SIGNATURES)
 
 
 def lib():
@@ -130,6 +133,8 @@
     l.fcp_subject_mask_workspace_bytes.restype = C.c_int64
     l.fcp_cutout_workspace_bytes.argtypes = [C.c_int, C.c_int, C.c_int]
     l.fcp_cutout_workspace_bytes.restype = C.c_int64
+    l.fcp_conv_kernel_id.argtypes = [C.POINTER(ConvDesc)]
+    l.fcp_conv_kernel_id.restype = C.c_int
     for name, args in SIGNATURES.items():
         fn = getattr(l, name)
         fn.argtypes = args
diff --git a/face-crop-plus_amd/csrc/fcp_conv.hip b/face-crop-plus_amd/csrc/fcp_conv.hip
--- a/face-crop-plus_amd/csrc/fcp_conv.hip
+++ b/face-crop-plus_amd/csrc/fcp_conv.hip
@@ -167,7 +167,9 @@
 
 }
 
-extern "C" int fcp_conv2d_nhwc_f32(const fcp_conv_desc* d, fcp_stream_t stream) {
+enum ConvRoute { ROUTE_F32, ROUTE_F32_FLAT, ROUTE_F16X3, ROUTE_DMA, ROUTE_HALO, ROUTE_HALO_WIDE, ROUTE_BIG };
+
+static int conv_resolve(const fcp_conv_desc* d, ConvK& k, ConvRoute& route) {
   FCP_REQUIRE(d != nullptr, "conv: null descriptor");
   FCP_REQUIRE(d->in && d->w && d->out, "conv: null tensor pointer");
   FCP_REQUIRE(d->n > 0 && d->in_h > 0 && d->in_w > 0 && d->cout > 0, "conv: bad sizes");
@@ -212,7 +214,6 @@
   const long M = (long)d->n * d->out_h * d->out_w;
   FCP_REQUIRE(M < (1L << 31), "conv: too many output pixels");
 
-  ConvK k;
   k.in = d->in; k.w = reinterpret_cast<const float*>(d->w); k.bias = d->bias; k.wscale = d->wscale; k.out = d->out; k.res1 = d->res1; k.res2 = d->res2;
   k.n = d->n; k.in_h = d->in_h; k.in_w = d->in_w;
   k.ph = d->in_up2 ? d->in_h / 2 : d->in_h;
@@ -277,7 +278,6 @@
   }
   k.grid_m = fcp_cdiv(M, BM);
   k.grid_n = fcp_cdiv(d->cout, d->tile_n);
-  hipStream_t s = (hipStream_t)stream;
   const unsigned long in_bytes = (unsigned long)d->n * k.ph * k.pw * d->in_ld * 4ul;
   const unsigned long w_bytes = (unsigned long)(k.grid_n * d->tile_n) * k.wrow * 4ul;
   FCP_REQUIRE(!(d->flags & FCP_CONV_FLAT_ADDR) || d->precision == 0, "conv: FCP_CONV_FLAT_ADDR is a precision-0 (fp32 kernel) option");
@@ -296,17 +296,47 @@
                   "conv(halo): wscale / bias must be 16-byte aligned");
       k.in2_bytes = (unsigned)out_bytes;
       k.w_bytes = (unsigned)((unsigned long)fcp_cdiv(d->cout, 128) * 128ul * k.wrow * 4ul);
-      return halo_wide ? launch_f16x3_halo_wide(k, s) : launch_f16x3_halo(k, s);
+      route = halo_wide ? ROUTE_HALO_WIDE : ROUTE_HALO;
+      return 0;
     }
     if (big) {
       k.w_bytes = (unsigned)((unsigned long)fcp_cdiv(d->cout, 128) * 128ul * k.wrow * 4ul);
-      return launch_f16x3_big(k, d->tile_n, s);
-    }
-    if (k.in_fmt == 1 && !d->cin4) return launch_f16x3_dma(k, d->tile_n, s);
-    return launch_f16x3(k, d->tile_n, d->cin4 != 0, s);
+      route = ROUTE_BIG;
+      return 0;
+    }
+    route = (k.in_fmt == 1 && !d->cin4) ? ROUTE_DMA : ROUTE_F16X3;
+    return 0;
   }
   k.in_bytes = buf ? (unsigned)in_bytes : 0u;
   k.w_bytes = buf ? (unsigned)w_bytes : 0u;
+  route = buf ? ROUTE_F32 : ROUTE_F32_FLAT;
+  return 0;
+}
+
+static int conv_group_kernel(const fcp_conv_desc* d, const ConvK& k, ConvRoute route) {
+  switch (route) {
+    case ROUTE_DMA: return d->tile_n == 32 && (k.out_fmt | k.res1_fmt | k.res2_fmt) == 0 ? GROUP_DMA_32 : 0;
+    case ROUTE_HALO: return k.cout > 32 ? GROUP_HALO_2 : 0;
+    case ROUTE_HALO_WIDE: return k.cout > 64 ? GROUP_HALO_WIDE_4 : 0;
+    case ROUTE_BIG: return d->tile_n == 192 ? GROUP_BIG_192 : 0;
+    default: return 0;
+  }
+}
+
+extern "C" int fcp_conv2d_nhwc_f32(const fcp_conv_desc* d, fcp_stream_t stream) {
+  ConvK k;
+  ConvRoute route;
+  if (const int e = conv_resolve(d, k, route)) return e;
+  hipStream_t s = (hipStream_t)stream;
+  switch (route) {
+    case ROUTE_HALO: return launch_f16x3_halo(k, s);
+    case ROUTE_HALO_WIDE: return launch_f16x3_halo_wide(k, s);
+    case ROUTE_BIG: return launch_f16x3_big(k, d->tile_n, s);
+    case ROUTE_DMA: return launch_f16x3_dma(k, d->tile_n, s);
+    case ROUTE_F16X3: return launch_f16x3(k, d->tile_n, d->cin4 != 0, s);
+    default: break;
+  }
+  const bool buf = route == ROUTE_F32;
 #define FCP_DISPATCH(BN_)                                                             \
   do {                                                                                \
     if (d->cin4) return buf ? launch<BN_, true, true>(k, s) : launch<BN_, true, false>(k, s); \
@@ -319,3 +349,31 @@
   }
 #undef FCP_DISPATCH
 }
+
+extern "C" int fcp_conv_kernel_id(const fcp_conv_desc* d) {
+  ConvK k;
+  ConvRoute route;
+  if (const int e = conv_resolve(d, k, route)) return e;
+  return conv_group_kernel(d, k, route);
+}
+
+extern "C" int fcp_conv2d_group_f16x3(const fcp_conv_desc* descs, int count, fcp_stream_t stream) {
+  FCP_REQUIRE(descs != nullptr && count >= 1 && count <= FCP_CONV_GROUP_MAX, "conv group: 1 .. %d descriptors", FCP_CONV_GROUP_MAX);
+  ConvK ks[FCP_CONV_GROUP_MAX];
+  int id = 0;
+  for (int i = 0; i < count; ++i) {
+    ConvRoute route;
+    if (const int e = conv_resolve(&descs[i], ks[i], route)) return e;
+    const int mine = conv_group_kernel(&descs[i], ks[i], route);
+    FCP_REQUIRE(mine != 0, "conv group: member %d resolves to a kernel without a grouped form", i);
+    FCP_REQUIRE(i == 0 || mine == id, "conv group: member %d resolves to another kernel instantiation (%d) than member 0 (%d)", i, mine, id);
+    id = mine;
+  }
+  hipStream_t s = (hipStream_t)stream;
+  switch (id) {
+    case GROUP_DMA_32: return launch_f16x3_dma_group(ks, count, s);
+    case GROUP_HALO_2: return launch_f16x3_halo_group(ks, count, s);
+    case GROUP_HALO_WIDE_4: return launch_f16x3_halo_wide_group(ks, count, s);
+    default: return launch_f16x3_big_group(ks, count, s);
+  }
+}
diff --git a/face-crop-plus_amd/csrc/fcp_conv_common.h b/face-crop-plus_amd/csrc/fcp_conv_common.h
--- a/face-crop-plus_amd/csrc/fcp_conv_common.h
+++ b/face-crop-plus_amd/csrc/fcp_conv_common.h
@@ -597,10 +597,61 @@
   }
 }
 
+constexpr int GROUP_MAX = FCP_CONV_GROUP_MAX;
+
+struct ConvGroupK {
+  ConvK m[GROUP_MAX];
+  int first[GROUP_MAX + 1];
+};
+
+__device__ __forceinline__ int group_member(const ConvGroupK& g, int block) {
+  int i = 0;
+#pragma unroll
+  for (int j = 1; j < GROUP_MAX; ++j) i += block >= g.first[j] ? 1 : 0;
+  return i;
+}
+
+template <typename Arg>
+struct LaunchMember;
+template <>
+struct LaunchMember<ConvK> {
+  const ConvK& p;
+  int block, nwg;
+  __device__ __forceinline__ LaunchMember(const ConvK& a) : p(a), block(blockIdx.x), nwg(gridDim.x) {}
+};
+template <>
+struct LaunchMember<ConvGroupK> {
+  int i;
+  const ConvK p;
+  int block, nwg;
+  __device__ __forceinline__ LaunchMember(const ConvGroupK& g)
+      : i(group_member(g, blockIdx.x)), p(g.m[i]), block(blockIdx.x - g.first[i]), nwg(g.first[i + 1] - g.first[i]) {}
+};
+
+static inline unsigned group_prefix(ConvGroupK& g, const unsigned* blocks, int count) {
+  unsigned total = 0;
+  for (int i = 0; i <= GROUP_MAX; ++i) {
+    g.first[i] = (int)total;
+    if (i < count) total += blocks[i];
+  }
+  return total;
+}
+
 int launch_f16x3(const ConvK& k, int tile_n, bool cin4, hipStream_t s);
 int launch_f16x3_dma(const ConvK& k, int tile_n, hipStream_t s);
 int launch_f16x3_halo(const ConvK& k, hipStream_t s);
 int launch_f16x3_halo_wide(const ConvK& k, hipStream_t s);
 int launch_f16x3_big(const ConvK& k, int tile_n, hipStream_t s);
 
-}
+enum GroupKernel {
+  GROUP_DMA_32 = 1,
+  GROUP_HALO_2 = 2,
+  GROUP_HALO_WIDE_4 = 3,
+  GROUP_BIG_192 = 4,
+};
+int launch_f16x3_dma_group(const ConvK* ks, int count, hipStream_t s);
+int launch_f16x3_halo_group(const ConvK* ks, int count, hipStream_t s);
+int launch_f16x3_halo_wide_group(const ConvK* ks, int count, hipStream_t s);
+int launch_f16x3_big_group(const ConvK* ks, int count, hipStream_t s);
+
+}
diff --git a/face-crop-plus_amd/csrc/fcp_conv_f16x3_big.hip b/face-crop-plus_amd/csrc/fcp_conv_f16x3_big.hip
--- a/face-crop-plus_amd/csrc/fcp_conv_f16x3_big.hip
+++ b/face-crop-plus_amd/csrc/fcp_conv_f16x3_big.hip
@@ -12,7 +12,7 @@
 constexpr int STAGE = 1 << 16;
 
 template <int BN>
-__global__ void __launch_bounds__(NT, 1) conv_igemm_f16x3_big(const ConvK p) {
+__device__ __forceinline__ void conv_igemm_f16x3_big_body(const ConvK& p, int block) {
   constexpr int WAVES_N = BN == 256 ? 4 : 2;
   constexpr int WAVES_M = 8 / WAVES_N;
   constexpr int WTM = BMB / WAVES_M, WTN = BN / WAVES_N;
@@ -23,7 +23,7 @@
   char* lds = reinterpret_cast<char*>(smem);
 
   const int nb = p.big_tiles;
-  int vb = blockIdx.x;
+  int vb = block;
   int tile_n = 0, m_start = 0, m_end = 0;
   auto decode = [&](int bid) {
     const int rbase = (bid / p.round_size) * p.round_size;
@@ -212,9 +212,18 @@
 }
 
 template <int BN>
-int launch(ConvK k, hipStream_t s) {
-  const size_t lds = 2 * (size_t)STAGE;
-  FCP_LDS_OPT_IN((&conv_igemm_f16x3_big<BN>), lds);
+__global__ void __launch_bounds__(NT, 1) conv_igemm_f16x3_big(const ConvK p) {
+  conv_igemm_f16x3_big_body<BN>(p, blockIdx.x);
+}
+template <int BN>
+__global__ void __launch_bounds__(NT, 1) conv_igemm_f16x3_big_group(const ConvGroupK g) {
+  const int i = group_member(g, blockIdx.x);
+  const ConvK p = g.m[i];
+  conv_igemm_f16x3_big_body<BN>(p, blockIdx.x - g.first[i]);
+}
+
+template <int BN>
+void schedule(ConvK& k) {
   k.grid_n = fcp_cdiv(k.cout, BN);
   int cus = k.cu_budget > 0 ? k.cu_budget : fcp_cu_count();
   cus = cus < 8 ? 8 : (cus & ~7);
@@ -240,6 +249,15 @@
     }
   }
   k.big_tiles = k.grid_m * k.grid_n;
+}
+
+constexpr size_t LDS_BYTES = 2 * (size_t)STAGE;
+
+template <int BN>
+int launch(ConvK k, hipStream_t s) {
+  const size_t lds = LDS_BYTES;
+  FCP_LDS_OPT_IN((&conv_igemm_f16x3_big<BN>), lds);
+  schedule<BN>(k);
   static const int persist_env = getenv("FCP_BIG_PERSIST") ? atoi(getenv("FCP_BIG_PERSIST")) : -1;
   k.big_persist = persist_env < 0 ? (k.cu_budget == 0) : (persist_env != 0);
   hipLaunchKernelGGL((conv_igemm_f16x3_big<BN>), dim3(k.big_persist && k.big_tiles > k.round_size ? k.round_size : k.big_tiles), dim3(NT), lds, s, k);
@@ -255,4 +273,21 @@
   return tile_n == 256 ? launch<256>(k, s) : tile_n == 192 ? launch<192>(k, s) : launch<128>(k, s);
 }
 
-}
+int launch_f16x3_big_group(const ConvK* ks, int count, hipStream_t s) {
+  ConvGroupK g = {};
+  unsigned blocks[GROUP_MAX] = {};
+  for (int i = 0; i < count; ++i) {
+    g.m[i] = ks[i];
+    schedule<192>(g.m[i]);
+    g.m[i].big_persist = 0;
+    blocks[i] = (unsigned)g.m[i].big_tiles;
+  }
+  const unsigned total = group_prefix(g, blocks, count);
+  const size_t lds = LDS_BYTES;
+  FCP_LDS_OPT_IN((&conv_igemm_f16x3_big_group<192>), lds);
+  hipLaunchKernelGGL((conv_igemm_f16x3_big_group<192>), dim3(total), dim3(NT), lds, s, g);
+  FCP_LAUNCH_OK();
+  return 0;
+}
+
+}
diff --git a/face-crop-plus_amd/csrc/fcp_conv_f16x3_dma.hip b/face-crop-plus_amd/csrc/fcp_conv_f16x3_dma.hip
--- a/face-crop-plus_amd/csrc/fcp_conv_f16x3_dma.hip
+++ b/face-crop-plus_amd/csrc/fcp_conv_f16x3_dma.hip
@@ -7,7 +7,7 @@
 constexpr int NST = 2;
 
 template <int BN, bool EP8>
-__global__ void __launch_bounds__(256, (BN == 128 ? 2 : 3)) conv_igemm_f16x3_dma(const ConvK p) {
+__device__ __forceinline__ void conv_igemm_f16x3_dma_body(const ConvK& p, int block, int nwg) {
   constexpr int WAVES_N = (BN == 32) ? 1 : 2;
   constexpr int WAVES_M = 4 / WAVES_N;
   constexpr int WTM = BM / WAVES_M;
@@ -21,7 +21,7 @@
   extern __shared__ __attribute__((aligned(16))) float smem[];
   char* lds = reinterpret_cast<char*>(smem);
 
-  const int logical = xcd_tile_order(gridDim.x, blockIdx.x);
+  const int logical = xcd_tile_order(nwg, block);
   const int tile_n = logical % p.grid_n;
   const int tile_m = logical / p.grid_n;
 
@@ -129,10 +129,26 @@
 }
 
 template <int BN, bool EP8>
+__global__ void __launch_bounds__(256, (BN == 128 ? 2 : 3)) conv_igemm_f16x3_dma(const ConvK p) {
+  conv_igemm_f16x3_dma_body<BN, EP8>(p, blockIdx.x, gridDim.x);
+}
+template <int BN, bool EP8>
+__global__ void __launch_bounds__(256, (BN == 128 ? 2 : 3)) conv_igemm_f16x3_dma_group(const ConvGroupK g) {
+  const int i = group_member(g, blockIdx.x);
+  const ConvK p = g.m[i];
+  conv_igemm_f16x3_dma_body<BN, EP8>(p, blockIdx.x - g.first[i], g.first[i + 1] - g.first[i]);
+}
+
+template <int BN, bool EP8>
+size_t lds_bytes() {
+  const size_t lds = (size_t)NST * (BM + BN) * 128;
+  const size_t epi = EP8 ? 0 : (size_t)BM * BN * 4;
+  return lds < epi ? epi : lds;
+}
+
+template <int BN, bool EP8>
 int launch_ep(const ConvK& k, hipStream_t s) {
-  size_t lds = (size_t)NST * (BM + BN) * 128;
-  const size_t epi = EP8 ? 0 : (size_t)BM * BN * 4;
-  if (lds < epi) lds = epi;
+  const size_t lds = lds_bytes<BN, EP8>();
   FCP_LDS_OPT_IN((&conv_igemm_f16x3_dma<BN, EP8>), lds);
   hipLaunchKernelGGL((conv_igemm_f16x3_dma<BN, EP8>), dim3(k.grid_m * k.grid_n), dim3(256), lds, s, k);
   FCP_LAUNCH_OK();
@@ -156,4 +172,19 @@
   }
 }
 
+int launch_f16x3_dma_group(const ConvK* ks, int count, hipStream_t s) {
+  ConvGroupK g = {};
+  unsigned blocks[GROUP_MAX] = {};
+  for (int i = 0; i < count; ++i) {
+    g.m[i] = ks[i];
+    blocks[i] = (unsigned)(ks[i].grid_m * ks[i].grid_n);
+  }
+  const unsigned total = group_prefix(g, blocks, count);
+  const size_t lds = lds_bytes<32, false>();
+  FCP_LDS_OPT_IN((&conv_igemm_f16x3_dma_group<32, false>), lds);
+  hipLaunchKernelGGL((conv_igemm_f16x3_dma_group<32, false>), dim3(total), dim3(256), lds, s, g);
+  FCP_LAUNCH_OK();
+  return 0;
 }
+
+}
diff --git a/face-crop-plus_amd/csrc/fcp_conv_f16x3_halo.hip b/face-crop-plus_amd/csrc/fcp_conv_f16x3_halo.hip
--- a/face-crop-plus_amd/csrc/fcp_conv_f16x3_halo.hip
+++ b/face-crop-plus_amd/csrc/fcp_conv_f16x3_halo.hip
@@ -60,13 +60,15 @@
   }
 }
 
-template <int TN>
-__global__ void __launch_bounds__(512, 1) conv3x3_halo_f16x3(const ConvK p) {
+template <int TN, typename Arg>
+__global__ void __launch_bounds__(512, 1) conv3x3_halo_f16x3(const Arg arg) {
+  const LaunchMember<Arg> me(arg);
+  const ConvK& p = me.p;
   extern __shared__ __attribute__((aligned(16))) float smem[];
   char* lds = reinterpret_cast<char*>(smem);
   const unsigned lds0 = (unsigned)(size_t)(__attribute__((address_space(3))) char*)lds;
 
-  const HaloTiles ts(p, gridDim.x, blockIdx.x);
+  const HaloTiles ts(p, me.nwg, me.block);
 
   const int lane = threadIdx.x & 63;
   const int wave8 = __builtin_amdgcn_readfirstlane(threadIdx.x >> 6);
@@ -337,8 +339,10 @@
 }
 
 
-template <int TN, bool RES, int BT, int RS>
-__global__ void __launch_bounds__(512, 1) conv3x3_halo_wide_f16x3(const ConvK p) {
+template <int TN, bool RES, int BT, int RS, typename Arg>
+__global__ void __launch_bounds__(512, 1) conv3x3_halo_wide_f16x3(const Arg arg) {
+  const LaunchMember<Arg> me(arg);
+  const ConvK& p = me.p;
   constexpr int TAPB = TN * 32 * ROWB;
   constexpr int PRE = RS - BT;
   constexpr bool SLACK2 = (RS - BT - 1) / BT >= 2;
@@ -347,7 +351,7 @@
   char* lds = reinterpret_cast<char*>(smem);
   const unsigned lds0 = (unsigned)(size_t)(__attribute__((address_space(3))) char*)lds;
 
-  const HaloTiles ts(p, gridDim.x, blockIdx.x);
+  const HaloTiles ts(p, me.nwg, me.block);
 
   const int lane = threadIdx.x & 63;
   const int wave8 = __builtin_amdgcn_readfirstlane(threadIdx.x >> 6);
@@ -667,11 +671,11 @@
   unsigned grid = 0;
   if (const int e = halo_grid(k, &grid)) return e;
   if (k.cout <= 32) {
-    FCP_LDS_OPT_IN(&conv3x3_halo_f16x3<1>, lds);
-    hipLaunchKernelGGL(conv3x3_halo_f16x3<1>, dim3(grid), dim3(512), lds, s, k);
+    FCP_LDS_OPT_IN((&conv3x3_halo_f16x3<1, ConvK>), lds);
+    hipLaunchKernelGGL((conv3x3_halo_f16x3<1, ConvK>), dim3(grid), dim3(512), lds, s, k);
   } else {
-    FCP_LDS_OPT_IN(&conv3x3_halo_f16x3<2>, lds);
-    hipLaunchKernelGGL(conv3x3_halo_f16x3<2>, dim3(grid), dim3(512), lds, s, k);
+    FCP_LDS_OPT_IN((&conv3x3_halo_f16x3<2, ConvK>), lds);
+    hipLaunchKernelGGL((conv3x3_halo_f16x3<2, ConvK>), dim3(grid), dim3(512), lds, s, k);
   }
   FCP_LAUNCH_OK();
   return 0;
@@ -687,14 +691,50 @@
   FCP_REQUIRE(k.ctiles >= 2 && k.ctiles % 2 == 0 && k.cout <= 128, "conv(halo, wide): cin must be a multiple of 64, cout <= 128");
   FCP_REQUIRE(tn == 2 || (k.res1 == nullptr && k.res2 == nullptr), "conv(halo, wide): no residual inputs with more than 64 filters");
   if (tn == 2) {
-    FCP_LDS_OPT_IN((&conv3x3_halo_wide_f16x3<2, true, WIDE2_BT, 8>), lds);
-    hipLaunchKernelGGL((conv3x3_halo_wide_f16x3<2, true, WIDE2_BT, 8>), dim3(grid), dim3(512), lds, s, k);
+    FCP_LDS_OPT_IN((&conv3x3_halo_wide_f16x3<2, true, WIDE2_BT, 8, ConvK>), lds);
+    hipLaunchKernelGGL((conv3x3_halo_wide_f16x3<2, true, WIDE2_BT, 8, ConvK>), dim3(grid), dim3(512), lds, s, k);
   } else {
-    FCP_LDS_OPT_IN((&conv3x3_halo_wide_f16x3<4, false, 1, 4>), lds);
-    hipLaunchKernelGGL((conv3x3_halo_wide_f16x3<4, false, 1, 4>), dim3(grid), dim3(512), lds, s, k);
+    FCP_LDS_OPT_IN((&conv3x3_halo_wide_f16x3<4, false, 1, 4, ConvK>), lds);
+    hipLaunchKernelGGL((conv3x3_halo_wide_f16x3<4, false, 1, 4, ConvK>), dim3(grid), dim3(512), lds, s, k);
   }
   FCP_LAUNCH_OK();
   return 0;
 }
 
-}
+static int halo_group(ConvGroupK& g, const ConvK* ks, int count, unsigned* total) {
+  unsigned blocks[GROUP_MAX] = {};
+  for (int i = 0; i < count; ++i) {
+    g.m[i] = ks[i];
+    if (const int e = halo_grid(ks[i], &blocks[i])) return e;
+  }
+  *total = group_prefix(g, blocks, count);
+  return 0;
+}
+
+int launch_f16x3_halo_group(const ConvK* ks, int count, hipStream_t s) {
+  ConvGroupK g = {};
+  unsigned total = 0;
+  for (int i = 0; i < count; ++i) FCP_REQUIRE(ks[i].cout > 32 && ks[i].cout <= 64, "conv group(halo): members need 33 .. 64 filters");
+  if (const int e = halo_group(g, ks, count, &total)) return e;
+  const size_t lds = (size_t)LDS_TOTAL;
+  FCP_LDS_OPT_IN((&conv3x3_halo_f16x3<2, ConvGroupK>), lds);
+  hipLaunchKernelGGL((conv3x3_halo_f16x3<2, ConvGroupK>), dim3(total), dim3(512), lds, s, g);
+  FCP_LAUNCH_OK();
+  return 0;
+}
+
+int launch_f16x3_halo_wide_group(const ConvK* ks, int count, hipStream_t s) {
+  ConvGroupK g = {};
+  unsigned total = 0;
+  for (int i = 0; i < count; ++i)
+    FCP_REQUIRE(ks[i].ctiles >= 2 && ks[i].ctiles % 2 == 0 && ks[i].cout > 64 && ks[i].cout <= 128 && ks[i].res1 == nullptr && ks[i].res2 == nullptr,
+                "conv group(halo, wide): members need cin %% 64 == 0, 65 .. 128 filters and no residual inputs");
+  if (const int e = halo_group(g, ks, count, &total)) return e;
+  const size_t lds = (size_t)(2 * A_BYTES + 4 * 4 * 32 * ROWB);
+  FCP_LDS_OPT_IN((&conv3x3_halo_wide_f16x3<4, false, 1, 4, ConvGroupK>), lds);
+  hipLaunchKernelGGL((conv3x3_halo_wide_f16x3<4, false, 1, 4, ConvGroupK>), dim3(total), dim3(512), lds, s, g);
+  FCP_LAUNCH_OK();
+  return 0;
+}
+
+}
diff --git a/face-crop-plus_amd/engine.py b/face-crop-plus_amd/engine.py
--- a/face-crop-plus_amd/engine.py
+++ b/face-crop-plus_amd/engine.py
@@ -1,6 +1,7 @@
 from __future__ import annotations
 
 import contextlib
+import functools
 import ctypes as C
 import os
 import threading
@@ -560,7 +561,10 @@
     if mon is not None:
         for i, t in enumerate(outs):
             if t is not None and t.c % 8 == 0:
-                mon.see(mon_label if i == 0 else f"{mon_label} [output {i}]", t)
+                if isinstance(mon_label, tuple):
+                    mon.see(mon_label[i], t)
+                else:
+                    mon.see(mon_label if i == 0 else f"{mon_label} [output {i}]", t)
     return outs
 
 
@@ -597,12 +601,16 @@
     return d
 
 
-def conv(pc: PackedConv, x: Act, out: Act | None = None, *, act_slope: float = 1.0,
-         alpha: float = 1.0, res1: Act | None = None, res1_pre: bool = True,
-         res2: Act | None = None, alpha2: float = 1.0, in_up2: bool = False,
-         tile_n: int | None = None, out_fmt: int = 0, tile_m: int | None = None,
-         x2: Act | None = None, x2_stride: int = 1, flat: bool = False, balance_tail: bool = False,
-         band: tuple[int, int] = (0, 0)) -> Act:
+class _ConvCall:
+    __slots__ = ("out", "desc", "go", "describe", "relaunch", "ins", "keep")
+
+
+def _conv_call(pc: PackedConv, x: Act, out: Act | None = None, *, act_slope: float = 1.0,
+               alpha: float = 1.0, res1: Act | None = None, res1_pre: bool = True,
+               res2: Act | None = None, alpha2: float = 1.0, in_up2: bool = False,
+               tile_n: int | None = None, out_fmt: int = 0, tile_m: int | None = None,
+               x2: Act | None = None, x2_stride: int = 1, flat: bool = False, balance_tail: bool = False,
+               band: tuple[int, int] = (0, 0)) -> _ConvCall:
     assert x.c + (x2.c if x2 is not None else 0) == pc.cin, f"conv expects {pc.cin} input channels, got {x.c}"
     in_h, in_w = (x.h * 2, x.w * 2) if in_up2 else (x.h, x.w)
     oh = (in_h - band[0] - band[1] + 2 * pc.pad - pc.kh) // pc.stride + 1
@@ -660,7 +668,63 @@
     def relaunch(o):
         o = _alias_safe_out(o, x, x2, res1, res2)
         return "fcp_conv2d_nhwc_f32", (C.byref(desc(o)),), (pc, x, x2, res1, res2, o)
-    return _accounted(go, describe, relaunch)[0]
+    c = _ConvCall()
+    c.out, c.desc, c.go, c.describe, c.relaunch = out, desc, go, describe, relaunch
+    c.ins, c.keep = (x, x2, res1, res2), (pc, x, x2, res1, res2)
+    return c
+
+
+@functools.wraps(_conv_call)
+def conv(*args, **kw) -> Act:
+    c = _conv_call(*args, **kw)
+    return _accounted(c.go, c.describe, c.relaunch)[0]
+
+
+conv.__name__ = conv.__qualname__ = "conv"
+conv.__doc__ = "Launch one fused convolution and return its output view: ``_conv_call`` (which documents the arguments), launched."
+_own_conv = conv
+
+
+def conv_group(calls) -> list:
+    if conv is not _own_conv:
+        return [conv(**kw) for kw in calls]
+    cs = [_conv_call(**kw) for kw in calls]
+    buckets = []
+    for c in cs:
+        kid = 0 if T.INSISTED else N.lib().fcp_conv_kernel_id(C.byref(c.desc(c.out)))
+        b = next((b for b in buckets if kid > 0 and b[0] == kid and len(b[1]) < N.CONV_GROUP_MAX), None)
+        if b is None:
+            buckets.append([kid if kid > 0 else None, [c]])
+        else:
+            b[1].append(c)
+    for _, members in buckets:
+        if len(members) == 1:
+            c = members[0]
+            _accounted(c.go, c.describe, c.relaunch)
+        else:
+            _conv_group_launch(members)
+    return [c.out for c in cs]
+
+
+def _conv_group_launch(members):
+    k = len(members)
+
+    def args(outs):
+        return (N.ConvDesc * k)(*[c.desc(o) for c, o in zip(members, outs)]), k
+
+    def go():
+        _c_launch("fcp_conv2d_group_f16x3", *args([c.out for c in members]))
+        return tuple(c.out for c in members)
+
+    def describe():
+        rows = [c.describe() for c in members]
+        return ("group[" + " | ".join(r[0] for r in rows) + "]", tuple(r[1] for r in rows),
+                sum(r[2] for r in rows), sum(r[3] for r in rows))
+
+    def relaunch(*outs):
+        outs = [_alias_safe_out(o, *c.ins) for c, o in zip(members, outs)]
+        return "fcp_conv2d_group_f16x3", args(outs), ([c.keep for c in members], outs)
+    return _accounted(go, describe, relaunch)
 
 
 def tile_candidates(cout: int, halo_ok: bool, wide_ok: bool, big_ok: bool):
diff --git a/face-crop-plus_amd/retinaface.py b/face-crop-plus_amd/retinaface.py
--- a/face-crop-plus_amd/retinaface.py
+++ b/face-crop-plus_amd/retinaface.py
@@ -27,6 +27,7 @@
         self._p = None
         self.precision = 0
         self.fused_chain = True
+        self.grouped_ssh = True
         self.streams = int(os.environ.get("FCP_DET_STREAMS", "2"))
         self.min_images_per_stream = 6
         self._tls = threading.local()
@@ -199,6 +200,13 @@
         o1 = E.conv(p["fpn.output1"], feats[0], act_slope=0.0, res1=o2, res1_pre=False, out_fmt=f)
         o1 = E.conv(p["fpn.merge1"], o1, act_slope=0.0, out_fmt=f)
         heads = []
+        if self.grouped_ssh:
+            lv = [(k, ft, E.Act.empty(ft.n, ft.h, ft.w, 384, ft.buf.device, f)) for k, ft in zip((1, 2, 3), (o1, o2, o3))]
+            E.conv_group([dict(pc=p[f"ssh{k}.ab"], x=ft, out=s.slice(0, 192), act_slope=0.0) for k, ft, s in lv])
+            E.conv_group([dict(pc=p[f"ssh{k}.cd"], x=s.slice(0, 64), out=s.slice(256, 128), act_slope=0.0) for k, ft, s in lv])
+            E.conv_group([dict(pc=p[f"ssh{k}.e"], x=s.slice(320, 64), out=s.slice(192, 64), act_slope=0.0) for k, ft, s in lv])
+            return E.conv_group([dict(pc=p[f"head{k}"], x=s.slice(64, 256),
+                                      out=None if heads_out is None else heads_out[k - 1]) for k, ft, s in lv])
         for k, ft in zip((1, 2, 3), (o1, o2, o3)):
             s = E.Act.empty(ft.n, ft.h, ft.w, 384, ft.buf.device, f)
             E.conv(p[f"ssh{k}.ab"], ft, s.slice(0, 192), act_slope=0.0)
diff --git a/face-crop-plus_amd/torch_ops.py b/face-crop-plus_amd/torch_ops.py
--- a/face-crop-plus_amd/torch_ops.py
+++ b/face-crop-plus_amd/torch_ops.py
@@ -23,6 +23,7 @@
 
 
 ENABLED = _default_enabled()
+INSISTED = ENABLED and os.environ.get("FCP_BOUNDARY", "auto").lower() == "torch"
 
 
 def load():
diff --git a/include/fcp_hip.h b/include/fcp_hip.h
--- a/include/fcp_hip.h
+++ b/include/fcp_hip.h
@@ -46,6 +46,10 @@
 
 int fcp_conv2d_nhwc_f32(const fcp_conv_desc* desc, fcp_stream_t stream);
 
+#define FCP_CONV_GROUP_MAX 4
+int fcp_conv2d_group_f16x3(const fcp_conv_desc* descs, int count, fcp_stream_t stream);
+int fcp_conv_kernel_id(const fcp_conv_desc* desc);
+
 typedef struct fcp_chain_desc {
   const float* t1;
   const void* w2;  const float* ws2;  const float* b2;
```
